# cboin1996/avddpg

Measured on AMD Instinct MI355X. Metric: env-steps/sec + DDPG updates/sec, 4096x5-vehicle platoons, higher is better.
Workload: dtype f32-class (fp16 hi+lo operand pairs on the 16-bit matrix cores, f32 accumulate)

## Files before the change

### avddpg_amd/_hip.py

```python
import ctypes as C
import os

_HERE = os.path.dirname(os.path.abspath(__file__))
LIB_PATH = os.path.join(_HERE, "lib", "libavddpg_hip.so")
if os.environ.get("AVDDPG_HIP_LIB"):
    LIB_PATH = os.path.abspath(os.environ["AVDDPG_HIP_LIB"])
HEADER_PATH = os.path.join(os.path.dirname(_HERE), "include", "avddpg_hip.h")
AVD_MAX_L = 16


class AvdError(RuntimeError):
    pass


class EnvConsts(C.Structure):
    _fields_ = [("L", C.c_int32), ("model_a", C.c_int32), ("can_terminate", C.c_int32), ("uniform_reset", C.c_int32),
                ("max_ep", C.c_float), ("max_ev", C.c_float), ("abs_action_high", C.c_float),
                ("two_max_a", C.c_float), ("T", C.c_float),
                ("ca", C.c_float), ("cb", C.c_float), ("cc", C.c_float), ("cd", C.c_float),
                ("re_scalar", C.c_float), ("terminal_reward", C.c_float),
                ("stand_still", C.c_float), ("timegap", C.c_float),
                ("reset_ep_max", C.c_float), ("reset_max_ev", C.c_float), ("reset_max_a", C.c_float),
                ("reset_ep_eval", C.c_float), ("reset_ev_eval", C.c_float), ("reset_a_eval", C.c_float),
                ("leader_reset_a", C.c_float),
                ("A", (C.c_float * 16) * AVD_MAX_L), ("B", (C.c_float * 4) * AVD_MAX_L),
                ("C", (C.c_float * 4) * AVD_MAX_L)]


_LAYOUT_FIELDS = ["S", "A", "H1", "H2", "Ha", "B",
                  "aW1", "ab1", "ag1", "abe1", "aW2", "ab2", "ag2", "abe2", "aW3", "ab3", "actor_size",
                  "cWs", "cbs", "cgs", "cbes", "cWa", "cba", "cga", "cbea", "cW2", "cb2", "cg3", "cbe3", "cW3", "cb3",
                  "theta_size",
                  "amm1", "amv1", "amm2", "amv2", "cmms", "cmvs", "cmma", "cmva", "cmm3", "cmv3", "stats_size"]


class MlpLayout(C.Structure):
    _fields_ = [(n, C.c_int32) for n in _LAYOUT_FIELDS]


_P = C.c_void_p
_i, _f, _d, _u64, _i64 = C.c_int, C.c_float, C.c_double, C.c_uint64, C.c_int64
_LP = C.POINTER(MlpLayout)

_PROTOS = {
    "avd_mlp_layout_init": [_LP, _i, _i, _i, _i, _i, _i],
    "avd_env_step_f32": [_P, _i, _i, _P, _P, _P, _P, _P, _P, _P, _P, _P, _P, _P, _P],
    "avd_env_reset_f32": [_P, _i, _i, _P, _P, _P, _P, _P, _i, _u64, _u64, _P, _P],
    "avd_episode_end_f32": [_P, _i, _i, _i, _P, _P, _P, _P, _P, _P, _i, _P, _P, _P, _P, _i, _u64, _u64, _P],
    "avd_ou_step_f32": [_i, _P, _P, _f, _f, _f, _f, _u64, _u64, _P],
    "avd_policy_f32": [_i, _P, _P, _f, _f, _P, _P],
    "avd_normal_f32": [_i, _P, _f, _u64, _u64, _P],
    "avd_uniform_f32": [_i, _P, _f, _u64, _u64, _P],
    "avd_step_fused_f32": [_P, _i, _i, _i, _P, _P, _P, _P, _P, _P, _P, _P, _P, _P, _P, _P, _P, _f, _f, _f, _f, _f, _f, _f, _i, _u64, _u64,
                           _u64, _P, _i, _i64, _P, _P],
    "avd_replay_sample_f32": [_i, _i, _i, _i, _i, _P, _i, _u64, _u64, _P, _P, _P, _P, _P, _P],
    "avd_actor_forward_set_f32": [_LP, _i, _i, _P, _P, _P, _i, _f, _P, _P, _P],
    "avd_replay_add_f32": [_i, _i, _i, _i, _P, _i64, _P, _P, _i, _P, _P, _P],
    "avd_replay_indices": [_i, _i, _i, _u64, _u64, _P, _P],
    "avd_replay_gather_f32": [_i, _i, _i, _i, _i, _P, _P, _P, _P, _P, _P, _P],
    "avd_actor_forward_f32": [_LP, _i, _i, _P, _P, _P, _i, _f, _P, _P],
    "avd_actor_forward_cond_f32": [_LP, _i, _i, _P, _P, _P, _i, _f, _P, _P, _P],
    "avd_critic_forward_f32": [_LP, _i, _i, _P, _P, _P, _i, _P, _P, _P],
    "avd_learn_f32": [_LP, _i, _i, _P, _P, _P, _P, _P, _P, _P, _P, _f, _f, _P, _P, _P],
    "avd_learn_update_f32": [_LP, _i, _P, _P, _P, _P, _P, _P, _P, _P, _P, _P, _P, _P, _f, _f, _f, _f, _d, _P, _P, _P],
    "avd_learn_update_act_f32": [_LP, _i, _P, _P, _P, _P, _P, _P, _P, _P, _P, _P, _P, _P, _f, _f, _f, _f, _d, _P, _P, _P, _i, _P, _P],
    "avd_learn_update_plan": [_LP, _i, C.POINTER(C.c_int), C.POINTER(C.c_int), C.POINTER(C.c_int)],
    "avd_adam_polyak_f32": [_LP, _i, _P, _P, _P, _P, _P, _P, _P, _P, _f, _f, _d, _P],
    "avd_adam_polyak_guarded_f32": [_LP, _i, _P, _P, _P, _P, _P, _P, _P, _P, _f, _f, _d, _P, _P],
    "avd_polyak_f32": [_i64, _P, _P, _d, _P],
    "avd_fed_sum_f32": [_i, _i, _i, _i, _i, _P, _P, _P, _P, _P],
    "avd_fed_finalize_f32": [_i, _i, _P, _f, _P, _P],
    "avd_fed_scatter_f32": [_i, _i, _i, _i, _i, _i, _P, _P, _P],
    "avd_adam_polyak_intra_f32": [_LP, _i, _i, _i, _P, _P, _P, _P, _P, _P, _P, _P, _P, _f, _f, _d, _P],
    "avd_fed_history_push_f32": [_i, _i, _i, _P, _P, _P, _i, _P, _i, _i, _P, _P, _P],
    "avd_fed_weights_f32": [_i, _i, _i, _P, _P, _i, _P, _P, _P, _P],
    "avd_learn_shared_workspace": [_LP, _i, _i, C.POINTER(C.c_size_t)],
    "avd_learn_shared_bf16": [_LP, _i, _i, _P, _P, _P, _P, _P, _P, _P, _P, _P, _f, _f, _P, _P, _P, C.c_size_t, _P],
    "avd_learn_set_fused_workspace": [_LP, _i, _i, C.POINTER(C.c_size_t)],
    "avd_learn_set_fused_bf16": [_LP, _i, _i, _P, _P, _P, _P, _P, _P, _P, _P, _P, _f, _f, _P, _P, _P, C.c_size_t, _P],
    "avd_learn_set_split_workspace": [_LP, _i, _i, C.POINTER(C.c_size_t)],
    "avd_learn_set_split_mfma_count": [_LP, _i, _i, C.POINTER(C.c_ulonglong)],
    "avd_learn_set_split_critic": [_LP, _i, _i, _P, _P, _P, _P, _P, _P, _P, _P, _P, _f, _f, _P, _P, _P, C.c_size_t, _P],
    "avd_learn_set_split_actor": [_LP, _i, _i, _P, _P, _P, _f, _P, _P, C.c_size_t, _P],
    "avd_learn_set_split_bf16x3": [_LP, _i, _i, _P, _P, _P, _P, _P, _P, _P, _P, _P, _f, _f, _P, _P, _P, C.c_size_t, _P],
    "avd_learn_set_split_f16x3": [_LP, _i, _i, _P, _P, _P, _P, _P, _P, _P, _P, _P, _f, _f, _P, _P, _P, C.c_size_t, _P],
    "avd_actor_forward_shared_workspace": [_LP, _i, _i, C.POINTER(C.c_size_t)],
    "avd_actor_forward_shared_bf16": [_LP, _i, _i, _P, _P, _P, _f, _P, _P, C.c_size_t, _P],
    "avd_gemm_bt_bf16": [_i, _i, _i, _P, C.c_long, _P, C.c_long, _P, C.c_long, _P],
}

_lib = None
DIAG_LIB_PATH = os.path.join(_HERE, "lib", "libavddpg_hip_diag.so")


def _load(path):
    if not os.path.exists(path):
        raise AvdError(f"{path} not found: build the HIP extension first (__graft_entry__.build()); "
                       "avddpg_amd has no CPU fallback")
    l = C.CDLL(path)
    missing = []
    for name, args in _PROTOS.items():
        fn = getattr(l, name, None)
        if fn is None:
            missing.append(name)
            continue
        fn.argtypes = args
        fn.restype = C.c_int
    if missing and not os.environ.get("AVDDPG_HIP_LIB"):
        raise AvdError(f"{path} does not export {', '.join(missing)}: rebuild it (make -C avddpg_amd/csrc)")
    l.avd_last_error.restype = C.c_char_p
    l.avd_last_error.argtypes = []
    l.avd_version.restype, l.avd_version.argtypes = C.c_int, []
    if getattr(l, "avd_diagnostics_enabled", None) is None:
        l.avd_diagnostics_enabled = lambda: 0
    else:
        l.avd_diagnostics_enabled.restype, l.avd_diagnostics_enabled.argtypes = C.c_int, []
    return l


def lib():
    global _lib
    if _lib is None:
        _lib = _load(LIB_PATH)
    return _lib


class diag_library:
    _cached = None
    _stack = []

    def __enter__(self):
        global _lib, LIB_PATH
        if diag_library._cached is None:
            diag_library._cached = _load(DIAG_LIB_PATH)
            if not diag_library._cached.avd_diagnostics_enabled():
                raise AvdError(f"{DIAG_LIB_PATH} is not a diagnostic build")
        diag_library._stack.append((lib(), LIB_PATH))
        _lib, LIB_PATH = diag_library._cached, DIAG_LIB_PATH
        return _lib

    def __exit__(self, *exc):
        global _lib, LIB_PATH
        _lib, LIB_PATH = diag_library._stack.pop()
        return False


def call(name, *args):
    fn = getattr(lib(), name, None)
    if fn is None:
        raise AvdError(f"{name} is not exported by the loaded library (an older build?)")
    rc = fn(*args)
    if rc != 0:
        raise AvdError(f"{name} failed ({rc}): {lib().avd_last_error().decode()}")


def ptr(t):
    if t is None:
        return None
    if not t.is_contiguous():
        raise AvdError("non-contiguous tensor passed to the C ABI")
    return C.c_void_p(t.data_ptr())


def stream_handle():
    import torch
    return C.c_void_p(torch.cuda.current_stream().cuda_stream)


def make_layout(S, A, H1, H2, Ha, B):
    lay = MlpLayout()
    call("avd_mlp_layout_init", C.byref(lay), S, A, H1, H2, Ha, B)
    return lay
```

### avddpg_amd/csrc/fset.hip

```cpp
#include "fset_common.h"

namespace avd {
namespace fset {

__device__ __forceinline__ bf16x8 make_xf(float x0, float x1, float x2, float x3, int h) {
    const bf16 a0 = (bf16)x0, a1 = (bf16)x1, a2 = (bf16)x2, a3 = (bf16)x3;
    const bf16 l0 = (bf16)(x0 - (float)a0), l1 = (bf16)(x1 - (float)a1), l2 = (bf16)(x2 - (float)a2), l3 = (bf16)(x3 - (float)a3);
    const bf16 one = (bf16)1.f, zero = (bf16)0.f;
    bf16x8 v;
    v[0] = a0, v[1] = a1, v[2] = a2, v[3] = a3;
    v[4] = h ? one : l0, v[5] = h ? one : l1, v[6] = h ? zero : l2, v[7] = h ? zero : l3;
    return v;
}
__device__ __forceinline__ bf16x8 make_wf(float w0, float w1, float w2, float w3, float b, int h) {
    const bf16 a0 = (bf16)w0, a1 = (bf16)w1, a2 = (bf16)w2, a3 = (bf16)w3, bh = (bf16)b;
    const bf16 l0 = (bf16)(w0 - (float)a0), l1 = (bf16)(w1 - (float)a1), l2 = (bf16)(w2 - (float)a2), l3 = (bf16)(w3 - (float)a3);
    const bf16 bl = (bf16)(b - (float)bh), zero = (bf16)0.f;
    bf16x8 v;
    v[0] = h ? l0 : a0, v[1] = h ? l1 : a1, v[2] = h ? l2 : a2, v[3] = h ? l3 : a3;
    v[4] = h ? bh : a0, v[5] = h ? bl : a1, v[6] = h ? zero : a2, v[7] = h ? zero : a3;
    return v;
}

struct NetP {
// ... 382 lines not shown
    NetP net;
    int n_agents, n_sets;
    const bf16* xf;
    const float* act;
    const bf16* dz;
    float* partG;
};
template <int S, class NET>
__global__ __launch_bounds__(NT) void dw_kernel(const DwArgs p) {
    constexpr int KG = NET::KG, NGT = NET::NGT, NFW = (NGT + 1) / 2, LDZ = 160;
    __shared__ __attribute__((aligned(16))) bf16 dzimg[2][TILE * LDZ];
    const int tid = threadIdx.x, w = tid >> 6, lane = tid & 63, r = lane & 31, h = lane >> 5, wn = w & 3, fg = w >> 2;
    const int set = blockIdx.x % p.n_sets, j0 = blockIdx.x / p.n_sets, J = gridDim.x / p.n_sets, P = p.n_agents / p.n_sets;
    const float* th = p.net.th + (long)set * p.net.th_stride;
    bf16x8 wf[NFW];
    f32x16 G[NFW];
    const f32x16 zero16 = {};
#pragma unroll
    for (int i = 0; i < NFW; ++i) wf[i] = layer1_wf<S, NET>(p.net, th, fg * NFW + i, r, h, true), G[i] = zero16;
    const bool act_tiles = NET::critic && fg == 1;

    const int srow = tid >> 3, sch = tid & 7;
    uint4 d0 = {}, d1 = {};
    auto fetch = [&](int agent) {
        const uint4* src = (const uint4*)(p.dz + ((long)agent * TILE + srow) * H2 + 16 * sch);
        d0 = src[0], d1 = src[1];
    };
    auto stage = [&](int buf) {
        uint4* dst = (uint4*)(dzimg[buf] + srow * LDZ + 16 * sch);
        dst[0] = d0, dst[1] = d1;
    };
    bf16x8 nx0 = {}, nx1 = {};
    float na0 = 0.f, na1 = 0.f;
    auto fetch_x = [&](int agent) {
        const bf16x8* xa = (const bf16x8*)p.xf + (long)agent * TILE * 2;
        nx0 = xa[2 * r + h], nx1 = xa[2 * (32 + r) + h];
        if (act_tiles) na0 = p.act[(long)agent * TILE + r], na1 = p.act[(long)agent * TILE + 32 + r];
    };
    if (j0 < P) fetch(j0 * p.n_sets + set), fetch_x(j0 * p.n_sets + set), stage(0);
    __syncthreads();
    const int g4 = lane >> 4, q = (lane & 15) >> 2, pp = lane & 3;
    int buf = 0;
    for (int pi = j0; pi < P; pi += J, buf ^= 1) {
        const bool more = pi + J < P;
        const bf16x8 xs0 = nx0, xs1 = nx1;
        const bf16x8 xa0 = make_xf(na0, 0.f, 0.f, 0.f, h), xa1 = make_xf(na1, 0.f, 0.f, 0.f, h);
        if (more) fetch((pi + J) * p.n_sets + set), fetch_x((pi + J) * p.n_sets + set);
        bf16x8 bfr[2][2];
#pragma unroll
        for (int rh = 0; rh < 2; ++rh)
#pragma unroll
            for (int s = 0; s < 2; ++s)
#pragma unroll
                for (int hf = 0; hf < 2; ++hf) {
                    const int R0 = 32 * rh + 16 * s + 8 * hf + 4 * (g4 >> 1);
                    const bf16x4 t = __builtin_amdgcn_ds_read_tr16_b64_v4bf16(
                        (__attribute__((address_space(3))) bf16x4*)(dzimg[buf] + (R0 + q) * LDZ + 32 * wn + 16 * (g4 & 1) + 4 * pp));
#pragma unroll
                    for (int j = 0; j < 4; ++j) bfr[rh][s][4 * hf + j] = t[j];
                }
#pragma unroll
        for (int i = 0; i < NFW; ++i) {
            if (fg * NFW + i >= NGT) continue;
            const bool at = act_tiles && i >= 3;
#pragma unroll
            for (int rh = 0; rh < 2; ++rh) {
                const bf16x8 xf = rh ? (at ? xa1 : xs1) : (at ? xa0 : xs0);
                const f32x16 p1 = mfma(xf, wf[i], zero16);
#pragma unroll
                for (int s = 0; s < 2; ++s) {
                    uint4 xu;
                    xu.x = relu_bf16x2(p1[8 * s], p1[8 * s + 1]), xu.y = relu_bf16x2(p1[8 * s + 2], p1[8 * s + 3]);
                    xu.z = relu_bf16x2(p1[8 * s + 4], p1[8 * s + 5]), xu.w = relu_bf16x2(p1[8 * s + 6], p1[8 * s + 7]);
                    G[i] = mfma(__builtin_bit_cast(bf16x8, xu), bfr[rh][s], G[i]);
                }
            }
        }
        if (more) stage(buf ^ 1);
        __syncthreads();
    }
#pragma unroll
    for (int i = 0; i < NFW; ++i) {
        if (fg * NFW + i >= NGT) continue;
        float* dst = p.partG + ((long)blockIdx.x * KG + 32 * (fg * NFW + i)) * H2 + 32 * wn + r;
#pragma unroll
        for (int k = 0; k < 16; ++k) dst[(long)acc_row(k, h) * H2] = G[i][k];
    }
}

struct DxArgs {
    NetP net;
    int n_agents, n_sets;
    const bf16* xf;
    const float* x;
    const bf16* dz;
    float* partU;
    float* partV;
};
template <int S, class NET>
__global__ __launch_bounds__(NT) void dx_kernel(const DxArgs p) {
    constexpr int KP = NET::KP, NF = 2, LDZ = 136;
    __shared__ __attribute__((aligned(16))) bf16 dzimg[2][TILE * LDZ];
    __shared__ __attribute__((aligned(16))) bf16 xt[8][2][32 * 32];
    const int tid = threadIdx.x, w = tid >> 6, lane = tid & 63, r = lane & 31, h = lane >> 5, rh = w & 1, fg = w >> 1;
    const int set = blockIdx.x % p.n_sets, j0 = blockIdx.x / p.n_sets, J = gridDim.x / p.n_sets, P = p.n_agents / p.n_sets;
    const float* th = p.net.th + (long)set * p.net.th_stride;
    const f32x16 zero16 = {};
    bf16x8 w2[NF][8], wf[NF];
    f32x16 V[NF];
    float U0[NF], U1[NF];
#pragma unroll
    for (int i = 0; i < NF; ++i) {
        const int ft = fg + 4 * i;
        const bf16* src = p.net.W2R + ((long)set * KP + 32 * ft + r) * H2 + 8 * h;
#pragma unroll
        for (int s = 0; s < 8; ++s) w2[i][s] = *(const bf16x8*)(src + 16 * s);
        wf[i] = layer1_wf<S, NET>(p.net, th, ft, r, h);
        V[i] = zero16, U0[i] = 0.f, U1[i] = 0.f;
    }
    for (int i = lane; i < 2 * 32 * 32; i += 64) {
        const int k = (i >> 5) & 31;
        xt[w][0][i] = (bf16)(k == 8 ? 1.f : 0.f);
    }
    const int srow = tid >> 3, sch = tid & 7;
    uint4 d0 = {}, d1 = {};
    auto fetch = [&](int agent) {
        const uint4* src = (const uint4*)(p.dz + ((long)agent * TILE + srow) * H2 + 16 * sch);
        d0 = src[0], d1 = src[1];
    };
    auto stage = [&](int buf) {
        uint4* dst = (uint4*)(dzimg[buf] + srow * LDZ + 16 * sch);
        dst[0] = d0, dst[1] = d1;
    };
    bf16x8 xfn = {};
    auto fetch_x = [&](int agent) { xfn = ((const bf16x8*)p.xf)[((long)agent * TILE + 32 * rh + r) * 2 + h]; };
    auto stage_x = [&](int buf) {
        if (h == 0) {
#pragma unroll
            for (int k = 0; k < 8; ++k) xt[w][buf][k * 32 + r] = xfn[k];
        }
    };
    __syncthreads();
    if (j0 < P) fetch(j0 * p.n_sets + set), fetch_x(j0 * p.n_sets + set), stage(0), stage_x(0);
    __syncthreads();
    int buf = 0;
    for (int pi = j0; pi < P; pi += J, buf ^= 1) {
        const bool more = pi + J < P;
        const bf16x8 xf = xfn;
        if (more) fetch((pi + J) * p.n_sets + set), fetch_x((pi + J) * p.n_sets + set);
        bf16x8 dzf[8];
        const bf16* arow = dzimg[buf] + (32 * rh + r) * LDZ + 8 * h;
#pragma unroll
        for (int s = 0; s < 8; ++s) dzf[s] = *(const bf16x8*)(arow + 16 * s);
        bf16x8 xb[2];
#pragma unroll
        for (int s = 0; s < 2; ++s) {
            const bf16x4 lo = *(const bf16x4*)(&xt[w][buf][r * 32 + 16 * s + 4 * h]);
            const bf16x4 hi = *(const bf16x4*)(&xt[w][buf][r * 32 + 16 * s + 8 + 4 * h]);
#pragma unroll
            for (int j = 0; j < 4; ++j) xb[s][j] = lo[j], xb[s][4 + j] = hi[j];
        }
#pragma unroll
        for (int i = 0; i < NF; ++i) {
            f32x16 dc = zero16;
#pragma unroll
            for (int s = 0; s < 8; ++s) dc = mfma(dzf[s], w2[i][s], dc);
            const f32x16 p1 = mfma(xf, wf[i], zero16);
            float u0 = 0.f, u1 = 0.f;
            bf16x8 va[2];
#pragma unroll
            for (int k = 0; k < 16; ++k) {
                const float pr = relu(p1[k]);
                u0 += dc[k];
                u1 = fmaf(dc[k], pr, u1);
                va[k >> 3][k & 7] = (bf16)(pr > 0.f ? dc[k] : 0.f);
            }
            U0[i] += u0, U1[i] += u1;
            V[i] = mfma(va[0], xb[0], V[i]);
            V[i] = mfma(va[1], xb[1], V[i]);
        }
        if (more) stage(buf ^ 1), stage_x(buf ^ 1);
        __syncthreads();
    }
#pragma unroll
    for (int i = 0; i < NF; ++i) {
        const int ft = fg + 4 * i;
        float* pu = p.partU + ((((long)blockIdx.x * 2 + rh) * 2 + h) * KP + 32 * ft + r) * 2;
        pu[0] = U0[i], pu[1] = U1[i];
        if (r < 16) {
            float* pv = p.partV + (((long)blockIdx.x * 2 + rh) * KP + 32 * ft) * 16 + r;
#pragma unroll
            for (int k = 0; k < 16; ++k) pv[(long)acc_row(k, h) * 16] = V[i][k];
        }
    }
}

template <int S>
__global__ __launch_bounds__(NT) void dxa_kernel(const DxArgs p) {
    typedef Critic NET;
    constexpr int KP = NET::KP;
    __shared__ __attribute__((aligned(16))) bf16 xt[8][2][32 * 32];
    __shared__ float comb[4][64][2 + 16];
    const int tid = threadIdx.x, w = tid >> 6, lane = tid & 63, r = lane & 31, h = lane >> 5, rh = w & 1, ftl = (w >> 1) & 1, par = w >> 2;
    const int set = blockIdx.x % p.n_sets, j0 = blockIdx.x / p.n_sets, J = gridDim.x / p.n_sets, P = p.n_agents / p.n_sets;
    const float* th = p.net.th + (long)set * p.net.th_stride;
    const f32x16 zero16 = {};
    const int ft = 8 + ftl;
    bf16x8 w2[8];
    {
        const bf16* src = p.net.W2R + ((long)set * KP + 32 * ft + r) * H2 + 8 * h;
#pragma unroll
        for (int s = 0; s < 8; ++s) w2[s] = *(const bf16x8*)(src + 16 * s);
    }
    const bf16x8 wf = layer1_wf<S, NET>(p.net, th, ft, r, h);
    f32x16 V = zero16;
    float U0 = 0.f, U1 = 0.f;
    for (int i = lane; i < 2 * 32 * 32; i += 64) {
        const int k = (i >> 5) & 31;
        xt[w][0][i] = (bf16)(k == 8 ? 1.f : 0.f);
    }
    __syncthreads();
    const int ntile = j0 < P ? (P - j0 + J - 1) / J : 0;
    bf16x8 dzn[8];
    float an = 0.f;
    auto fetch = [&](int k) {
        const long ri = (long)((j0 + k * J) * p.n_sets + set) * TILE + 32 * rh + r;
        const bf16* src = p.dz + ri * H2 + 8 * h;
#pragma unroll
        for (int s = 0; s < 8; ++s) dzn[s] = *(const bf16x8*)(src + 16 * s);
        an = p.x[ri];
    };
    if (par < ntile) fetch(par);
    int buf = 0;
    for (int k = par; k < ntile; k += 2, buf ^= 1) {
        bf16x8 dzf[8];
#pragma unroll
        for (int s = 0; s < 8; ++s) dzf[s] = dzn[s];
        const bf16x8 xf = make_xf(an, 0.f, 0.f, 0.f, h);
        if (k + 2 < ntile) fetch(k + 2);
        if (h == 0) {
            xt[w][buf][r] = xf[0];
            xt[w][buf][4 * 32 + r] = xf[4];
        }
        __builtin_amdgcn_fence(__ATOMIC_RELEASE, "wavefront");
        __builtin_amdgcn_wave_barrier();
        bf16x8 xb[2];
#pragma unroll
        for (int s = 0; s < 2; ++s) {
            const bf16x4 lo = *(const bf16x4*)(&xt[w][buf][r * 32 + 16 * s + 4 * h]);
            const bf16x4 hi = *(const bf16x4*)(&xt[w][buf][r * 32 + 16 * s + 8 + 4 * h]);
#pragma unroll
            for (int j = 0; j < 4; ++j) xb[s][j] = lo[j], xb[s][4 + j] = hi[j];
        }
        f32x16 dc = zero16;
#pragma unroll
        for (int s = 0; s < 8; ++s) dc = mfma(dzf[s], w2[s], dc);
        const f32x16 p1 = mfma(xf, wf, zero16);
        float u0 = 0.f, u1 = 0.f;
        bf16x8 va[2];
#pragma unroll
        for (int i = 0; i < 16; ++i) {
            const float pr = relu(p1[i]);
            u0 += dc[i];
            u1 = fmaf(dc[i], pr, u1);
            va[i >> 3][i & 7] = (bf16)(pr > 0.f ? dc[i] : 0.f);
        }
        U0 += u0, U1 += u1;
        V = mfma(va[0], xb[0], V);
        V = mfma(va[1], xb[1], V);
    }
    const int pw = w & 3;
    if (par == 1) {
        comb[pw][lane][0] = U0, comb[pw][lane][1] = U1;
#pragma unroll
        for (int i = 0; i < 16; ++i) comb[pw][lane][2 + i] = V[i];
    }
    __syncthreads();
    if (par == 0) {
        U0 += comb[pw][lane][0], U1 += comb[pw][lane][1];
        float* pu = p.partU + ((((long)blockIdx.x * 2 + rh) * 2 + h) * KP + 32 * ft + r) * 2;
        pu[0] = U0, pu[1] = U1;
        if (r < 16) {
            float* pv = p.partV + (((long)blockIdx.x * 2 + rh) * KP + 32 * ft) * 16 + r;
#pragma unroll
            for (int i = 0; i < 16; ++i) pv[(long)acc_row(i, h) * 16] = V[i] + comb[pw][lane][2 + i];
        }
    }
}

__global__ __launch_bounds__(512) void finalize_small_kernel(const FinArgs a) {
    const int set = blockIdx.x, net = a.net_lo + blockIdx.y, tid = threadIdx.x, jl = tid & 31;
    const int item = a.item_base + blockIdx.z * 16 + (tid >> 5);
    const bool critic = net;
    const avd_mlp_layout& L = a.L;
    const float* th = a.theta + (long)set * L.theta_size + (critic ? L.actor_size : 0);
    const float* st = a.stats + (long)set * L.stats_size;
    float* g = a.grads + (long)set * L.theta_size + (critic ? L.actor_size : 0);
    const int K = critic ? Critic::K : Actor::K, KP = critic ? Critic::KP : Actor::KP;
    auto allsum = [&](float v) {
#pragma unroll
        for (int o = 1; o < 32; o <<= 1) v += __shfl_xor(v, o);
        return v;
    };
    if (item < H2) {
        const int n = item;
        const int og2 = critic ? L.cg3 : L.ag2, obe2 = critic ? L.cbe3 : L.abe2, omm2 = critic ? L.cmm3 : L.amm2, omv2 = critic ? L.cmv3 : L.amv2;
        const int oW3 = critic ? L.cW3 : L.aW3, ob3 = critic ? L.cb3 : L.ab3, ob2 = critic ? L.cb2 : L.ab2;
        const int KG = critic ? Critic::KG : Actor::KG;
        float T1 = 0.f, S2 = 0.f, D = 0.f, Lc = 0.f, La = 0.f;
        const bool t1g = a.t1_from_g[net] != 0;
        for (int j = jl; j < a.J; j += 32) {
            const long wg = (long)j * a.n_sets + set;
            for (int w = 0; w < 8; ++w) {
                if (!t1g) T1 += a.partH[net][(wg * 8 + w) * H2 + n];
                D += a.partHs[net][(wg * 8 + w) * 2];
                if (critic && n == 0) Lc += a.partHs[1][(wg * 8 + w) * 2 + 1], La += a.partLa[(wg * 8 + w) * 2 + 1];
            }
            S2 += a.partG[net][(wg * KG + K) * H2 + n];
        }
        T1 = allsum(T1), S2 = allsum(S2), D = allsum(D);
        if (t1g && jl == 0) a.s2raw[((long)net * a.n_sets + set) * H2 + n] = S2;
        if (a.c3[net]) S2 *= a.c3[net][(long)set * VEC + H2 + n];
        if (critic && n == 0) Lc = allsum(Lc), La = allsum(La);
        if (a.bad && *a.bad) T1 = S2 = D = Lc = La = __uint_as_float(0x7fc00000u);
        if (jl == 0) {
            const float rs2 = 1.0f / sqrtf(st[omv2 + n] + BN_EPS), inv2 = rs2 * th[og2 + n], mm2 = st[omm2 + n];
            const float sh2 = th[obe2 + n] - mm2 * inv2, w3 = th[oW3 + n];
            if (!t1g) {
                g[oW3 + n] = inv2 * T1 + sh2 * D;
                g[og2 + n] = w3 * rs2 * (T1 - mm2 * D);
            }
            g[obe2 + n] = w3 * D;
            g[ob2 + n] = S2;
            if (n == 0) g[ob3] = D;
            if (critic && n == 0 && a.losses) a.losses[2 * set] = Lc * a.inv_n, a.losses[2 * set + 1] = -La * a.inv_n;
        }
        return;
    }
    const int f = item - H2;
    if (f >= K) return;
    float U0 = 0.f, U1 = 0.f, V[9];
#pragma unroll
    for (int k = 0; k < 9; ++k) V[k] = 0.f;
    const bool have_u = a.partU[net] != nullptr;
    for (int j = jl; j < a.J; j += 32) {
        const long wg = (long)j * a.n_sets + set;
        for (int rh = 0; rh < a.nrh; ++rh) {
            if (have_u)
                for (int h = 0; h < 2; ++h) {
                    const float* pu = a.partU[net] + ((((wg * a.nrh + rh) * 2 + h) * KP) + f) * 2;
                    U0 += pu[0], U1 += pu[1];
                }
            const float* pv = a.partV[net] + ((wg * a.nrh + rh) * KP + f) * 16;
#pragma unroll
            for (int k = 0; k < 9; ++k) V[k] += pv[k];
        }
    }
    U0 = allsum(U0), U1 = allsum(U1);
#pragma unroll
    for (int k = 0; k < 9; ++k) V[k] = allsum(V[k]);
    if (!have_u) {
        const int oW2 = critic ? L.cW2 : L.aW2, ob2 = critic ? L.cb2 : L.ab2;
        float u0 = 0.f;
        for (int n = jl; n < H2; n += 32) u0 = fmaf(th[oW2 + (long)f * H2 + n], g[ob2 + n], u0);
        U0 = allsum(u0);
        int oW, ob, ff = f, ld = H1, sin = a.S;
        if (!critic) oW = L.aW1, ob = L.ab1;
        else if (f < H1) oW = L.cWs, ob = L.cbs;
        else oW = L.cWa, ob = L.cba, ff = f - H1, ld = HA, sin = 1;
        U1 = th[ob + ff] * V[8];
        for (int k = 0; k < sin; ++k) U1 = fmaf(th[oW + k * ld + ff], V[k] + V[4 + k], U1);
    }
    if (a.bad && *a.bad) U0 = U1 = V[0] = V[4] = V[8] = __uint_as_float(0x7fc00000u);
    if (jl == 0) {
        int og, obe, omm, omv, oW, ob, ff = f, ld = H1, sin = a.S;
        if (!critic) og = L.ag1, obe = L.abe1, omm = L.amm1, omv = L.amv1, oW = L.aW1, ob = L.ab1;
        else if (f < H1) og = L.cgs, obe = L.cbes, omm = L.cmms, omv = L.cmvs, oW = L.cWs, ob = L.cbs;
        else og = L.cga, obe = L.cbea, omm = L.cmma, omv = L.cmva, oW = L.cWa, ob = L.cba, ff = f - H1, ld = HA, sin = 1;
        const float rs1 = 1.0f / sqrtf(st[omv + ff] + BN_EPS), inv1 = rs1 * th[og + ff], mm1 = st[omm + ff];
        g[obe + ff] = U0;
        g[og + ff] = rs1 * (U1 - mm1 * U0);
        g[ob + ff] = inv1 * V[8];
        for (int k = 0; k < sin; ++k) g[oW + k * ld + ff] = inv1 * (V[k] + V[4 + k]);
    }
}
__global__ __launch_bounds__(128) void finalize_w2_kernel(const FinArgs a) {
    const int f = blockIdx.x, set = blockIdx.y, net = a.net_lo + blockIdx.z, n = threadIdx.x;
    const bool critic = net;
    const int K = critic ? Critic::K : Actor::K, KG = critic ? Critic::KG : Actor::KG;
    if (f >= K) return;
    const avd_mlp_layout& L = a.L;
    const float* th = a.theta + (long)set * L.theta_size + (critic ? L.actor_size : 0);
    const float* st = a.stats + (long)set * L.stats_size;
    float* g = a.grads + (long)set * L.theta_size + (critic ? L.actor_size : 0);
    int og, obe, omm, omv, ff = f;
    if (!critic) og = L.ag1, obe = L.abe1, omm = L.amm1, omv = L.amv1;
    else if (f < H1) og = L.cgs, obe = L.cbes, omm = L.cmms, omv = L.cmvs;
    else og = L.cga, obe = L.cbea, omm = L.cmma, omv = L.cmva, ff = f - H1;
    const float inv1 = (1.0f / sqrtf(st[omv + ff] + BN_EPS)) * th[og + ff], sh1 = th[obe + ff] - st[omm + ff] * inv1;
    float G = 0.f;
    const float* pg = a.partG[net] + ((long)set * KG + f) * H2 + n;
    const long stride = (long)a.n_sets * KG * H2;
    int j = 0;
    for (; j + 8 <= a.J; j += 8) {
        float v[8];
#pragma unroll
        for (int u = 0; u < 8; ++u) v[u] = pg[(j + u) * stride];
#pragma unroll
        for (int u = 0; u < 8; ++u) G += v[u];
    }
    for (; j < a.J; ++j) G += pg[j * stride];
    const int oW2 = critic ? L.cW2 : L.aW2, ob2 = critic ? L.cb2 : L.ab2;
    if (a.t1_from_g[net]) a.t1p[(((long)net * a.n_sets + set) * Critic::K + f) * H2 + n] = inv1 * th[oW2 + (long)f * H2 + n] * G;
    if (a.c3[net]) G *= a.c3[net][(long)set * VEC + H2 + n];
    if (a.bad && *a.bad) G = __uint_as_float(0x7fc00000u);
    g[oW2 + (long)f * H2 + n] = inv1 * G + sh1 * g[ob2 + n];
}
__global__ __launch_bounds__(128) void finalize_t1_kernel(const FinArgs a) {
    const int set = blockIdx.x, net = a.net_lo + blockIdx.y, n = threadIdx.x;
    if (!a.t1_from_g[net]) return;
    const bool critic = net;
    const avd_mlp_layout& L = a.L;
    const float* th = a.theta + (long)set * L.theta_size + (critic ? L.actor_size : 0);
    const float* st = a.stats + (long)set * L.stats_size;
    float* g = a.grads + (long)set * L.theta_size + (critic ? L.actor_size : 0);
    const int K = critic ? Critic::K : Actor::K;
    const int og2 = critic ? L.cg3 : L.ag2, obe2 = critic ? L.cbe3 : L.abe2, omm2 = critic ? L.cmm3 : L.amm2, omv2 = critic ? L.cmv3 : L.amv2;
    const int oW3 = critic ? L.cW3 : L.aW3, ob3 = critic ? L.cb3 : L.ab3;
    const float* tp = a.t1p + ((long)net * a.n_sets + set) * Critic::K * H2 + n;
    float T1 = 0.f;
    int f = 0;
    for (; f + 8 <= K; f += 8) {
        float v[8];
#pragma unroll
        for (int u = 0; u < 8; ++u) v[u] = tp[(long)(f + u) * H2];
#pragma unroll
        for (int u = 0; u < 8; ++u) T1 += v[u];
    }
    for (; f < K; ++f) T1 += tp[(long)f * H2];
    T1 = fmaf(a.c3[net][(long)set * VEC + n], a.s2raw[((long)net * a.n_sets + set) * H2 + n], T1);
    const float D = g[ob3];
    if (a.bad && *a.bad) T1 = __uint_as_float(0x7fc00000u);
    const float rs2 = 1.0f / sqrtf(st[omv2 + n] + BN_EPS), inv2 = rs2 * th[og2 + n], mm2 = st[omm2 + n];
    const float sh2 = th[obe2 + n] - mm2 * inv2, w3 = th[oW3 + n];
    g[oW3 + n] = inv2 * T1 + sh2 * D;
    g[og2 + n] = w3 * rs2 * (T1 - mm2 * D);
}

void launch_finalize(const FinArgs& fa0, hipStream_t st, int net_lo, int n_nets) {
    FinArgs fa = fa0;
    fa.net_lo = net_lo, fa.item_base = 0;
    const int K = (net_lo + n_nets > 1) ? Critic::K : Actor::K;
    if (fa.partU[net_lo]) {
        hipLaunchKernelGGL(finalize_small_kernel, dim3(fa.n_sets, n_nets, (H2 + K + 15) / 16), dim3(512), 0, st, fa);
    } else {
        hipLaunchKernelGGL(finalize_small_kernel, dim3(fa.n_sets, n_nets, H2 / 16), dim3(512), 0, st, fa);
        fa.item_base = H2;
        hipLaunchKernelGGL(finalize_small_kernel, dim3(fa.n_sets, n_nets, (K + 15) / 16), dim3(512), 0, st, fa);
    }
    hipLaunchKernelGGL(finalize_w2_kernel, dim3(K, fa.n_sets, n_nets), dim3(H2), 0, st, fa);
    bool any = false;
    for (int net = net_lo; net < net_lo + n_nets; ++net) any = any || fa.t1_from_g[net];
    if (any) hipLaunchKernelGGL(finalize_t1_kernel, dim3(fa.n_sets, n_nets), dim3(H2), 0, st, fa);
}

struct Plan {
    int grid, J;
    size_t W2T[4], W2R[2], vec[4], a2, y, mu, dmu, dz, xfs, xfs2, partH[2], partHs[3], partU[2], partV[2], partG[2], bad, total;
};
int cu_count() {
    static int cache[64] = {0};
    int dev = 0;
    if (hipGetDevice(&dev) != hipSuccess || dev < 0) return 256;
    if (dev < 64 && cache[dev]) return cache[dev];
    hipDeviceProp_t prop;
    if (hipGetDeviceProperties(&prop, dev) != hipSuccess) return 256;
    const int n = prop.multiProcessorCount > 0 ? prop.multiProcessorCount : 256;
    if (dev < 64) cache[dev] = n;
    return n;
}
static Plan make_plan(int n_agents, int n_sets) {
    Plan pl;
    const int P = n_agents / n_sets;
    int J = cu_count() / n_sets;
    if (J < 1) J = 1;
    if (J > P) J = P;
    pl.J = J, pl.grid = J * n_sets;
    size_t o = 0;
    auto take = [&](size_t bytes) {
        const size_t at = o;
        o += (bytes + 255) / 256 * 256;
        return at;
    };
    for (int i = 0; i < 4; ++i) {
        const int KP = (i & 1) ? Critic::KP : Actor::KP, KW = (i & 1) ? Critic::KW : Actor::KW;
        pl.W2T[i] = take(sizeof(bf16) * (size_t)n_sets * H2 * KW);
        pl.vec[i] = take(sizeof(float) * (size_t)n_sets * VEC);
        if (i < 2) pl.W2R[i] = take(sizeof(bf16) * (size_t)n_sets * KP * H2);
    }
    const size_t rows = (size_t)n_agents * TILE;
    pl.a2 = take(4 * rows), pl.y = take(4 * rows), pl.mu = take(4 * rows), pl.dmu = take(4 * rows);
    pl.dz = take(sizeof(bf16) * rows * H2);
    pl.xfs = take(sizeof(bf16) * rows * 16), pl.xfs2 = take(sizeof(bf16) * rows * 16);
    for (int i = 0; i < 2; ++i) {
        const int KP = i ? Critic::KP : Actor::KP, KG = i ? Critic::KG : Actor::KG;
        pl.partH[i] = take(4 * (size_t)pl.grid * 8 * H2);
        pl.partU[i] = take(4 * (size_t)pl.grid * 2 * 2 * KP * 2);
        pl.partV[i] = take(4 * (size_t)pl.grid * 2 * KP * 16);
        pl.partG[i] = take(4 * (size_t)pl.grid * KG * H2);
    }
    for (int i = 0; i < 3; ++i) pl.partHs[i] = take(4 * (size_t)pl.grid * 8 * 2);
    pl.bad = take(sizeof(int));
    pl.total = o;
    return pl;
}
static int check_fset(const avd_mlp_layout* L, int n_agents, int n_sets, const char* who) {
    AVD_REQUIRE(L, "%s: null layout", who);
    if (L->H1 != H1 || L->H2 != H2 || L->Ha != HA || L->A != 1 || (L->S != 3 && L->S != 4) || L->B != TILE) {
        set_error("%s: serves the reference widths only (layer1 256, layer2 128, action layer 48, A = 1, S in {3, 4}, B = 64); "
                  "got H1=%d H2=%d Ha=%d A=%d S=%d B=%d (avd_learn_shared_bf16 takes other widths)",
                  who, L->H1, L->H2, L->Ha, L->A, L->S, L->B);
        return AVD_E_UNSUPPORTED;
    }
    AVD_REQUIRE(n_sets > 0 && n_sets <= 64 && n_agents > 0 && n_agents % n_sets == 0, "%s: n_agents=%d n_sets=%d", who, n_agents,
                n_sets);
    return AVD_OK;
}

template <int S>
static int run(const avd_mlp_layout& L, int n_agents, int n_sets, const float* theta, const float* stats, const float* theta_t,
               const float* stats_t, const float* s, const float* a, const float* r, const float* s2, const float* aw, float gamma,
               float high, float* grads, float* losses, unsigned char* ws, const Plan& pl, hipStream_t st) {
    PrepArgs pa;
    pa.L = L, pa.theta = theta, pa.stats = stats, pa.theta_t = theta_t, pa.stats_t = stats_t;
    NetP net[4];
    for (int i = 0; i < 4; ++i) {
        const bool critic = i & 1, target = i >= 2;
        pa.W2T[i] = (bf16*)(ws + pl.W2T[i]), pa.vec[i] = (float*)(ws + pl.vec[i]);
        pa.W2R[i] = i < 2 ? (bf16*)(ws + pl.W2R[i]) : nullptr;
        NetP& n = net[i];
        n.th = (target ? theta_t : theta) + (critic ? L.actor_size : 0), n.st = target ? stats_t : stats;
        n.th_stride = L.theta_size, n.st_stride = L.stats_size;
        n.oW1 = critic ? L.cWs : L.aW1, n.ob1 = critic ? L.cbs : L.ab1;
        n.oWa = critic ? L.cWa : 0, n.oba = critic ? L.cba : 0, n.oga = critic ? L.cga : 0, n.omva = critic ? L.cmva : 0;
        n.W2T = pa.W2T[i], n.W2R = pa.W2R[i], n.vec = pa.vec[i];
    }
    pa.bad = (int*)(ws + pl.bad);
    (void)hipMemsetAsync(ws + pl.bad, 0, sizeof(int), st);
    hipLaunchKernelGGL(prep_kernel, dim3(H2, 4, n_sets), dim3(320), 0, st, pa);
    const long nrows = (long)n_agents * TILE;
    bf16 *xfs = (bf16*)(ws + pl.xfs), *xfs2 = (bf16*)(ws + pl.xfs2);
    int* bad = (int*)(ws + pl.bad);
    hipLaunchKernelGGL(pack_x_kernel<S>, dim3((unsigned)((2 * nrows + 255) / 256)), dim3(256), 0, st, s, a, nrows, xfs, bad);
    hipLaunchKernelGGL(pack_x_kernel<S>, dim3((unsigned)((2 * nrows + 255) / 256)), dim3(256), 0, st, s2, r, nrows, xfs2, bad);
    const int P = n_agents / n_sets;
    const float inv_n = 1.0f / ((float)P * TILE);
    float *a2 = (float*)(ws + pl.a2), *y = (float*)(ws + pl.y), *mu = (float*)(ws + pl.mu), *dmu = (float*)(ws + pl.dmu);
    bf16* dz = (bf16*)(ws + pl.dz);
    auto F = [&](size_t off) { return (float*)(ws + off); };
    const dim3 grid(pl.grid), block(NT);
    HeadArgs h;
    h.n_agents = n_agents, h.n_sets = n_sets, h.gamma = gamma, h.high = high, h.inv_n = inv_n, h.aw = aw, h.dz = dz, h.dmu = dmu;
    auto head = [&](auto kern, int mode, int ni, const bf16* x, const float* act, const float* rr, const float* yin, float* out,
                    float* part, float* part_s) {
        h.net = net[ni], h.xf = x, h.act = act, h.r = rr, h.yin = yin, h.out = out, h.part = part, h.part_s = part_s;
        hipLaunchKernelGGL(kern, grid, dim3(64 * head_waves(mode)), 0, st, h);
    };
    DwArgs dw;
    dw.n_agents = n_agents, dw.n_sets = n_sets, dw.dz = dz;
    DxArgs dx;
    dx.n_agents = n_agents, dx.n_sets = n_sets, dx.dz = dz;
    head(head_kernel<S, Actor, OUT_TANH>, OUT_TANH, 2, xfs2, nullptr, nullptr, nullptr, a2, nullptr, nullptr);
    head(head_kernel<S, Critic, OUT_TD>, OUT_TD, 3, xfs2, a2, r, nullptr, y, nullptr, nullptr);
    head(head_kernel<S, Actor, OUT_TANH>, OUT_TANH, 0, xfs, nullptr, nullptr, nullptr, mu, nullptr, nullptr);
    head(head_kernel<S, Critic, HEAD_CRITIC>, HEAD_CRITIC, 1, xfs, a, nullptr, y, nullptr, F(pl.partH[1]), F(pl.partHs[1]));
    dw.net = net[1], dw.xf = xfs, dw.act = a, dw.partG = F(pl.partG[1]);
    hipLaunchKernelGGL((dw_kernel<S, Critic>), grid, block, 0, st, dw);
    dx.net = net[1], dx.partU = F(pl.partU[1]), dx.partV = F(pl.partV[1]);
    dx.xf = xfs, dx.x = nullptr;
    hipLaunchKernelGGL((dx_kernel<S, Critic>), grid, block, 0, st, dx);
    dx.x = a;
    hipLaunchKernelGGL((dxa_kernel<S>), grid, block, 0, st, dx);
    head(head_kernel<S, Critic, HEAD_CONST>, HEAD_CONST, 1, xfs, mu, nullptr, nullptr, nullptr, nullptr, F(pl.partHs[2]));
    head(head_kernel<S, Actor, HEAD_ACTOR>, HEAD_ACTOR, 0, xfs, nullptr, nullptr, dmu, nullptr, F(pl.partH[0]), F(pl.partHs[0]));
    dw.net = net[0], dw.xf = xfs, dw.act = nullptr, dw.partG = F(pl.partG[0]);
    hipLaunchKernelGGL((dw_kernel<S, Actor>), grid, block, 0, st, dw);
    dx.net = net[0], dx.partU = F(pl.partU[0]), dx.partV = F(pl.partV[0]), dx.x = nullptr;
    hipLaunchKernelGGL((dx_kernel<S, Actor>), grid, block, 0, st, dx);
    FinArgs fa;
    fa.L = L, fa.n_sets = n_sets, fa.J = pl.J, fa.S = S, fa.theta = theta, fa.stats = stats, fa.grads = grads, fa.losses = losses;
    fa.inv_n = inv_n, fa.partLa = F(pl.partHs[2]);
    for (int i = 0; i < 2; ++i)
        fa.partH[i] = F(pl.partH[i]), fa.partHs[i] = F(pl.partHs[i]), fa.partU[i] = F(pl.partU[i]), fa.partV[i] = F(pl.partV[i]),
        fa.partG[i] = F(pl.partG[i]);
    fa.nrh = 2, fa.c3[0] = fa.c3[1] = nullptr, fa.bad = (const int*)(ws + pl.bad);
    fa.t1_from_g[0] = fa.t1_from_g[1] = 0, fa.t1p = nullptr, fa.s2raw = nullptr;
    launch_finalize(fa, st);
    return check_launch("avd_learn_set_fused_bf16");
}

}
}

using namespace avd;

extern "C" int avd_learn_set_fused_workspace(const avd_mlp_layout* lay, int n_agents, int n_sets, size_t* bytes) {
    int rc = fset::check_fset(lay, n_agents, n_sets, "avd_learn_set_fused_workspace");
    if (rc) return rc;
    AVD_REQUIRE(bytes, "avd_learn_set_fused_workspace: null pointer");
    *bytes = fset::make_plan(n_agents, n_sets).total;
    return AVD_OK;
}

extern "C" int avd_learn_set_fused_bf16(const avd_mlp_layout* lay, int n_agents, int n_sets, const float* theta, const float* stats,
                                        const float* theta_t, const float* stats_t, const float* s, const float* a, const float* r,
                                        const float* s2, const float* agent_weight, float gamma, float high, float* grads,
                                        float* losses, void* workspace, size_t workspace_bytes, void* stream) {
    int rc = fset::check_fset(lay, n_agents, n_sets, "avd_learn_set_fused_bf16");
    if (rc) return rc;
    AVD_REQUIRE(theta && stats && theta_t && stats_t && s && a && r && s2 && grads && workspace,
                "avd_learn_set_fused_bf16: null pointer");
    const fset::Plan pl = fset::make_plan(n_agents, n_sets);
    AVD_REQUIRE(workspace_bytes >= pl.total, "avd_learn_set_fused_bf16: workspace %zu B < %zu B", workspace_bytes, pl.total);
    if (hipMemsetAsync(grads, 0, sizeof(float) * (size_t)n_sets * lay->theta_size, (hipStream_t)stream) != hipSuccess)
        return check_launch("avd_learn_set_fused_bf16: hipMemsetAsync(grads)");
    if (lay->S == 4)
        return fset::run<4>(*lay, n_agents, n_sets, theta, stats, theta_t, stats_t, s, a, r, s2, agent_weight, gamma, high, grads,
                            losses, (unsigned char*)workspace, pl, (hipStream_t)stream);
    return fset::run<3>(*lay, n_agents, n_sets, theta, stats, theta_t, stats_t, s, a, r, s2, agent_weight, gamma, high, grads, losses,
                        (unsigned char*)workspace, pl, (hipStream_t)stream);
}
```

### avddpg_amd/csrc/fsplit.hip

```cpp
#include <type_traits>

#include "fset_common.h"

namespace avd {
namespace fsplit {
using namespace fset;

struct ActorS {
    static constexpr int K = 256, KP = 256, NFT = 8, NKS = 16, LD = 264, NGT = 9, KG = 288;
    static constexpr bool critic = false;
};
struct CriticS {
    static constexpr int K = 304, KP = 320, NFT = 10, NKS = 19, LD = 312, NGT = 10, KG = 320;
    static constexpr bool critic = true;
};
constexpr int NGT_MAX = 10;

template <int I, int N, class F>
__device__ __forceinline__ void static_for(F&& f) {
    if constexpr (I < N) {
        f(std::integral_constant<int, I>{});
        static_for<I + 1, N>(f);
    }
}

typedef _Float16 f16;
typedef _Float16 f16x2 __attribute__((ext_vector_type(2)));
typedef _Float16 f16x8 __attribute__((ext_vector_type(8)));
constexpr float S1 = 64.f;
constexpr float F16_OVERFLOW = 65520.f;
#if defined(FSPLIT_ABL_CONST)
#define FSPLIT_ABL(x) FSPLIT_ABL_CONST
#elif defined(AVD_DIAG)
#define FSPLIT_ABL(x) (x)
#else
#define FSPLIT_ABL(x) 0
#endif
__device__ __forceinline__ void split2h(float a, float b, unsigned& hi, unsigned& lo) {
    const f32x2 f = {a, b};
    const f16x2 h = __builtin_convertvector(f, f16x2);
    hi = __builtin_bit_cast(unsigned, h);
    f32x2 l;
#ifdef __HIP_DEVICE_COMPILE__
    asm("v_fma_mix_f32 %0, -%1, 1.0, %2 op_sel:[0,0,0] op_sel_hi:[1,0,0]" : "=v"(l[0]) : "v"(hi), "v"(a));
    asm("v_fma_mix_f32 %0, -%1, 1.0, %2 op_sel:[1,0,0] op_sel_hi:[1,0,0]" : "=v"(l[1]) : "v"(hi), "v"(b));
#else
    l[0] = a - (float)h[0], l[1] = b - (float)h[1];
#endif
    lo = __builtin_bit_cast(unsigned, __builtin_convertvector(l, f16x2));
}
__device__ __forceinline__ void split1h(float x, f16& hi, f16& lo) {
    hi = (f16)x;
    lo = (f16)(x - (float)hi);
}
template <class V>
__device__ __forceinline__ void pin16(V& x) {
#pragma unroll
    for (int q = 0; q < 2; ++q) {
        float a = x[8 * q], b = x[8 * q + 1], c = x[8 * q + 2], d = x[8 * q + 3], e = x[8 * q + 4], f = x[8 * q + 5], g = x[8 * q + 6], h = x[8 * q + 7];
        asm volatile("" : "+v"(a), "+v"(b), "+v"(c), "+v"(d), "+v"(e), "+v"(f), "+v"(g), "+v"(h));
        x[8 * q] = a, x[8 * q + 1] = b, x[8 * q + 2] = c, x[8 * q + 3] = d, x[8 * q + 4] = e, x[8 * q + 5] = f, x[8 * q + 6] = g, x[8 * q + 7] = h;
    }
}
__device__ __forceinline__ f16x8 fragh(unsigned a, unsigned b, unsigned c, unsigned d) {
    uint4 o;
    o.x = a, o.y = b, o.z = c, o.w = d;
    return __builtin_bit_cast(f16x8, o);
}
__device__ __forceinline__ f32x16 mfmah(f16x8 a, f16x8 b, f32x16 c) {
    return __builtin_amdgcn_mfma_f32_32x32x16_f16(a, b, c, 0, 0, 0);
}
__device__ __forceinline__ f16x8 make_xh(float x0, float x1, float x2, float x3, int h) {
    f16 a0, a1, a2, a3, l0, l1, l2, l3;
    split1h(x0, a0, l0), split1h(x1, a1, l1), split1h(x2, a2, l2), split1h(x3, a3, l3);
    const f16 one = (f16)1.f, zero = (f16)0.f;
    f16x8 v;
    v[0] = a0, v[1] = a1, v[2] = a2, v[3] = a3;
    v[4] = h ? one : l0, v[5] = h ? one : l1, v[6] = h ? zero : l2, v[7] = h ? zero : l3;
    return v;
}
__device__ __forceinline__ f16x8 make_wh(float w0, float w1, float w2, float w3, float b, float sc, int h) {
    f16 a0, a1, a2, a3, l0, l1, l2, l3, bh, bl;
    split1h(sc * w0, a0, l0), split1h(sc * w1, a1, l1), split1h(sc * w2, a2, l2), split1h(sc * w3, a3, l3), split1h(sc * b, bh, bl);
    const f16 zero = (f16)0.f;
    f16x8 v;
    v[0] = h ? l0 : a0, v[1] = h ? l1 : a1, v[2] = h ? l2 : a2, v[3] = h ? l3 : a3;
    v[4] = h ? bh : a0, v[5] = h ? bl : a1, v[6] = h ? bh : a2, v[7] = h ? zero : a3;
    return v;
}
__device__ __forceinline__ f16x8 make_xg(float x0, float x1, float x2, float x3, float g, int h) {
    f16 a0, a1, a2, a3, l0, l1, l2, l3, gh, gl;
    split1h(x0, a0, l0), split1h(x1, a1, l1), split1h(x2, a2, l2), split1h(x3, a3, l3), split1h(g, gh, gl);
    const f16 zero = (f16)0.f;
    f16x8 v;
    v[0] = a0, v[1] = a1, v[2] = a2, v[3] = a3;
    v[4] = h ? gh : l0, v[5] = h ? gh : l1, v[6] = h ? gl : l2, v[7] = h ? zero : l3;
    return v;
}

template <int S>
__device__ __forceinline__ void load_x(const float* xa, long row, float (&x)[4]) {
    if (S == 4) {
        const float4 v = *(const float4*)(xa + 4 * row);
        x[0] = v.x, x[1] = v.y, x[2] = v.z, x[3] = v.w;
    } else {
#pragma unroll
        for (int k = 0; k < 4; ++k) x[k] = k < S ? xa[S * row + k] : 0.f;
    }
}

__host__ __device__ constexpr int wpos(int f) { return (f & ~12) | ((f & 4) << 1) | ((f & 8) >> 1); }

struct NetP {
    const float* th;
    long th_stride;
    const f16* Whi;
    const f16* Wlo;
    const f16* Wchi;
    const f16* Wclo;
    const f16x8* wf1h;
    const float* vec;
    const unsigned* wap;
};

struct PackArgs {
    const float* x[2];
    const float* extra[2];
    f16x8* outh[2];
    long rows;
    int* bad;
};
template <int S>
__global__ __launch_bounds__(256) void pack_x_kernel(const PackArgs a) {
    const int which = blockIdx.y;
    const float* x = a.x[which];
    const float* extra = a.extra[which];
    const bool extra_is_action = which == 0;
    const long i = (long)blockIdx.x * 256 + threadIdx.x;
    if (i >= 2 * a.rows) return;
    float v[4];
    load_x<S>(x, i >> 1, v);
    bool nf = not_finite(v[0]) || not_finite(v[1]) || not_finite(v[2]) || not_finite(v[3]);
    nf = nf || fmaxf(fmaxf(fabsf(v[0]), fabsf(v[1])), fmaxf(fabsf(v[2]), fabsf(v[3]))) >= F16_OVERFLOW;
    if (!(i & 1)) {
        const float e = extra[i >> 1];
        nf = nf || not_finite(e) || (extra_is_action && fabsf(e) >= F16_OVERFLOW);
    }
    if (nf) atomicOr(a.bad, 1);
    a.outh[which][i] = make_xh(v[0], v[1], v[2], v[3], (int)(i & 1));
}

struct PrepArgs {
    avd_mlp_layout L;
    int S;
    const float *theta, *stats, *theta_t, *stats_t;
    f16 *Whi[4], *Wlo[4];
    f16 *Wchi[4], *Wclo[4];
    f16x8* wf1h[4];
    float* vec[4];
    unsigned* wap;
    unsigned* smax;
    int* bad;
};
constexpr int SCALE_SLICES = 16;
__device__ __forceinline__ float pow2_for(float mx) {
    int e = 0;
    if (mx > 0.f && !not_finite(mx)) (void)frexpf(mx, &e);
    int k = 13 - e;
    k = k < -14 ? -14 : (k > 30 ? 30 : k);
    return ldexpf(1.f, k);
}
__global__ __launch_bounds__(256) void scale_kernel(const PrepArgs a) {
    __shared__ float red[256], red2[256], c3a[H2], inva[CriticS::K];
    const int net = blockIdx.x, set = blockIdx.y, slice = blockIdx.z, tid = threadIdx.x;
    const bool critic = net & 1, target = net >= 2;
    const avd_mlp_layout& L = a.L;
    const float* th = (target ? a.theta_t : a.theta) + (long)set * L.theta_size + (critic ? L.actor_size : 0);
    const float* st = (target ? a.stats_t : a.stats) + (long)set * L.stats_size;
    const int K = critic ? CriticS::K : ActorS::K, oW2 = critic ? L.cW2 : L.aW2;
    const int og2 = critic ? L.cg3 : L.ag2, omv2 = critic ? L.cmv3 : L.amv2, oW3 = critic ? L.cW3 : L.aW3;
    if (tid < H2) c3a[tid] = fabsf((1.0f / sqrtf(st[omv2 + tid] + BN_EPS)) * th[og2 + tid] * th[oW3 + tid]);
    for (int f = tid; f < K; f += 256) {
        int og, omv, ff = f;
        if (!critic) og = L.ag1, omv = L.amv1;
        else if (f < H1) og = L.cgs, omv = L.cmvs;
        else og = L.cga, omv = L.cmva, ff = f - H1;
        inva[f] = fabsf((1.0f / sqrtf(st[omv + ff] + BN_EPS)) * th[og + ff]);
    }
    __syncthreads();
    const int total = K * H2, per = (total + SCALE_SLICES - 1) / SCALE_SLICES, lo = slice * per, hi = min(total, lo + per);
    float m = 0.f, m2 = 0.f;
    for (int i = lo + tid; i < hi; i += 256) {
        const float w = fabsf(th[oW2 + i]);
        m = fmaxf(m, inva[i / H2] * w);
        m2 = fmaxf(m2, c3a[i % H2] * w);
    }
    red[tid] = m, red2[tid] = m2;
    __syncthreads();
    for (int o = 128; o > 0; o >>= 1) {
        if (tid < o) red[tid] = fmaxf(red[tid], red[tid + o]), red2[tid] = fmaxf(red2[tid], red2[tid + o]);
        __syncthreads();
    }
    if (tid == 0) {
        unsigned* dst = a.smax + ((long)net * gridDim.y + set) * 2;
        atomicMax(dst, __float_as_uint(red[0]));
        atomicMax(dst + 1, __float_as_uint(red2[0]));
    }
}
__global__ __launch_bounds__(320) void prep_kernel(const PrepArgs a) {
    __shared__ float red[320];
    const int n = blockIdx.x, net = blockIdx.y, set = blockIdx.z, f = threadIdx.x;
    const bool critic = net & 1, target = net >= 2;
    const avd_mlp_layout& L = a.L;
    const float* th = (target ? a.theta_t : a.theta) + (long)set * L.theta_size + (critic ? L.actor_size : 0);
    const float* st = (target ? a.stats_t : a.stats) + (long)set * L.stats_size;
    const int K = critic ? CriticS::K : ActorS::K, KP = critic ? CriticS::KP : ActorS::KP;
    const int oW2 = critic ? L.cW2 : L.aW2, ob2 = critic ? L.cb2 : L.ab2, oW3 = critic ? L.cW3 : L.aW3, ob3 = critic ? L.cb3 : L.ab3;
    const int og2 = critic ? L.cg3 : L.ag2, obe2 = critic ? L.cbe3 : L.abe2, omm2 = critic ? L.cmm3 : L.amm2, omv2 = critic ? L.cmv3 : L.amv2;
    const float inv2n = (1.0f / sqrtf(st[omv2 + n] + BN_EPS)) * th[og2 + n], c3n = inv2n * th[oW3 + n];
    const unsigned* smax = a.smax + ((long)net * gridDim.z + set) * 2;
    const float SW = pow2_for(__uint_as_float(smax[0])), SWC = pow2_for(__uint_as_float(smax[1]));
    float shw = 0.f;
    if (f < KP) {
        float w = 0.f, inv = 0.f;
        if (f < K) {
            int og, obe, omm, omv, ff = f;
            if (!critic) og = L.ag1, obe = L.abe1, omm = L.amm1, omv = L.amv1;
            else if (f < H1) og = L.cgs, obe = L.cbes, omm = L.cmms, omv = L.cmvs;
            else og = L.cga, obe = L.cbea, omm = L.cmma, omv = L.cmva, ff = f - H1;
            inv = (1.0f / sqrtf(st[omv + ff] + BN_EPS)) * th[og + ff];
            const float sh = th[obe + ff] - st[omm + ff] * inv;
            w = th[oW2 + (long)f * H2 + n];
            shw = sh * w;
            if (not_finite(w) || not_finite(inv) || not_finite(sh)) atomicOr(a.bad, 1);
            f16 hi, lo;
            const float ws = SW * (inv * w);
            if (fabsf(ws) >= F16_OVERFLOW) atomicOr(a.bad, 1);
            split1h(ws, hi, lo);
            const long at = ((long)set * H2 + n) * K + wpos(f);
            a.Whi[net][at] = hi, a.Wlo[net][at] = lo;
        }
        if (!target) {
            f16 hi, lo;
            const float wc = SWC * (c3n * w);
            if (fabsf(wc) >= F16_OVERFLOW) atomicOr(a.bad, 1);
            split1h(wc, hi, lo);
            const long at = ((long)set * KP + f) * H2 + n;
            a.Wchi[net][at] = hi, a.Wclo[net][at] = lo;
        }
    }
    red[f] = shw;
    __syncthreads();
    if (f < 64) red[f] += red[f + 256];
    __syncthreads();
    for (int o = 128; o > 0; o >>= 1) {
        if (f < o) red[f] += red[f + o];
        __syncthreads();
    }
    float* vec = a.vec[net] + (long)set * VEC;
    if (f == 0) {
        if (n == 0) vec[2 * H2 + 1] = SW, vec[2 * H2 + 2] = SWC;
        vec[n] = th[ob2 + n] + red[0];
        vec[H2 + n] = c3n;
        if (not_finite(vec[n]) || not_finite(c3n) || not_finite(th[ob3])) atomicOr(a.bad, 1);
    }
    if (n == 0) {
        __syncthreads();
        float v = 0.f;
        if (f < H2) {
            const float inv2 = (1.0f / sqrtf(st[omv2 + f] + BN_EPS)) * th[og2 + f];
            v = (th[obe2 + f] - st[omm2 + f] * inv2) * th[oW3 + f];
        }
        red[f] = v;
        __syncthreads();
        for (int o = 64; o > 0; o >>= 1) {
            if (f < o) red[f] += red[f + o];
            __syncthreads();
        }
        if (f == 0) vec[2 * H2] = th[ob3] + red[0];
    }
}
__global__ __launch_bounds__(64) void prep1_kernel(const PrepArgs a) {
    const int ft = blockIdx.x, net = blockIdx.y, set = blockIdx.z, lane = threadIdx.x, r = lane & 31, h = lane >> 5;
    const bool critic = net & 1, target = net >= 2;
    const avd_mlp_layout& L = a.L;
    const float* th = (target ? a.theta_t : a.theta) + (long)set * L.theta_size + (critic ? L.actor_size : 0);
    const int K = critic ? CriticS::K : ActorS::K;
    const int f = 32 * ft + r;
    float w[4] = {0.f, 0.f, 0.f, 0.f}, b = 0.f;
    if (f == K) {
        b = 1.f;
    } else if (f < K) {
        if (critic && ft >= 8) {
            w[0] = th[L.cWa + (f - H1)], b = th[L.cba + (f - H1)];
        } else {
            const float* W = th + (critic ? L.cWs : L.aW1);
#pragma unroll
            for (int k = 0; k < 4; ++k) w[k] = k < a.S ? W[k * H1 + f] : 0.f;
            b = th[(critic ? L.cbs : L.ab1) + f];
        }
        if (not_finite(w[0]) || not_finite(w[1]) || not_finite(w[2]) || not_finite(w[3]) || not_finite(b)) atomicOr(a.bad, 1);
        if (S1 * fmaxf(fmaxf(fabsf(w[0]), fabsf(w[1])), fmaxf(fmaxf(fabsf(w[2]), fabsf(w[3])), fabsf(b))) >= F16_OVERFLOW) atomicOr(a.bad, 1);
    }
    a.wf1h[net][((long)set * NGT_MAX + ft) * 64 + lane] = make_wh(w[0], w[1], w[2], w[3], b, S1, h);
    if (net == 1 && ft == 0 && lane < 48) {
        const int hl = lane / 24, hh = (lane / 12) & 1, ks = (lane / 4) % 3, m = lane & 3;
        unsigned v = 0;
#pragma unroll
        for (int e = 0; e < 2; ++e) {
            const int jj = 2 * m + e, fa = 16 * ks + 8 * (jj >> 2) + 4 * hh + (jj & 3);
            f16 hi, lo;
            split1h(S1 * th[L.cWa + fa], hi, lo);
            v |= (unsigned)__builtin_bit_cast(unsigned short, hl ? lo : hi) << (16 * e);
        }
        a.wap[(long)set * 48 + lane] = v;
    }
}

enum HeadMode { OUT_TANH = 0, OUT_TD = 1, HEAD_BOTH = 5, OUT_TANH_SAVE = 6 };
struct HeadArgs {
    unsigned long long* stamp;
    NetP net;
    int n_agents, n_sets;
    const f16x8* xf;
    const float* act;
    const float* act2;
    const float* r;
    const float* yin;
    const float* aw;
    float* out;
    f16* sm;
    float* g3;
    float* dmu;
    float* part_s;
    float* part_s2;
    float* part_m;
    float* tz;
    float gamma, high, inv_n;
    int* bad;
    int abl;
};
#ifndef HEAD_FAST
#define HEAD_FAST 5
#define HEAD_SLOW 3
#endif

template <int S, class NET, int MODE>
__global__ __launch_bounds__(NT) void head_kernel(const HeadArgs p) {
    constexpr int K = NET::K, NKS = NET::NKS, NFT = NET::NFT, LD = NET::LD;
    constexpr int NTH = NT;
    constexpr bool BOTH = (MODE == HEAD_BOTH);
    static_assert(!BOTH || NET::critic, "HEAD_BOTH is a critic mode");
    __shared__ __attribute__((aligned(16))) f16 wimg[2][H2 * LD];
    __shared__ __attribute__((aligned(16))) float b2s[H2];
    __shared__ __attribute__((aligned(16))) float c3s[H2];
    __shared__ __attribute__((aligned(16))) unsigned waps[BOTH ? 48 : 4];
    const int tid = threadIdx.x, w = tid >> 6, lane = tid & 63, r = lane & 31, h = lane >> 5, q = w >> 1, rh = w & 1;
    const int set = blockIdx.x % p.n_sets, j0 = blockIdx.x / p.n_sets, J = gridDim.x / p.n_sets, P = p.n_agents / p.n_sets;
    for (int i = tid; i < 2 * H2 * (K / 8); i += NTH) {
        const int hl = i / (H2 * (K / 8)), rem = i - hl * (H2 * (K / 8)), n = rem / (K / 8), c = rem - n * (K / 8);
        const f16* src = (hl ? p.net.Wlo : p.net.Whi) + ((long)set * H2 + n) * K + 8 * c;
        *(uint4*)(&wimg[hl][n * LD + 8 * c]) = *(const uint4*)src;
    }
    const float* vec = p.net.vec + (long)set * VEC;
    const float SW = vec[2 * H2 + 1], sc = SW * S1, isc = 1.f / sc;
    if (tid < H2) b2s[tid] = vec[tid] * sc, c3s[tid] = vec[H2 + tid] * isc;
    if (BOTH && tid < 48) waps[tid] = p.net.wap[(long)set * 48 + tid];
    const float d3 = vec[2 * H2];
    const f16x8* wf1 = p.net.wf1h + (long)set * NGT_MAX * 64 + lane;
    const f32x16 zero16 = {};
#ifdef AVD_STAMP
    unsigned long long hacc[4] = {0, 0, 0, 0}, hlast = __builtin_amdgcn_s_memtime();
    const unsigned long long hstart = hlast;
#define HSTAMP(i) { const unsigned long long t_ = __builtin_amdgcn_s_memtime(); hacc[i] += t_ - hlast; hlast = t_; }
#else
#define HSTAMP(i)
#endif
    float Dacc = 0.f, Lacc = 0.f, Dacc2 = 0.f, Lacc2 = 0.f, gmax = 0.f;
    unsigned watch = 0;
    auto look = [&](float x) {
        unsigned u = __float_as_uint(x);
        asm volatile("" : "+v"(u));
        u &= 0x7fffffffu;
        watch = watch > u ? watch : u;
    };
    __syncthreads();

    const int ntile = j0 < P ? (P - j0 + J - 1) / J : 0;
    const int row = 32 * rh + r;
    f16x8 nx = {};
    float na = 0.f, nb = 0.f, ny = 0.f, nw = 1.f;
    auto fetch_in = [&](int k) {
        const int agent = (j0 + k * J) * p.n_sets + set;
        const long ri = (long)agent * TILE + row;
        nx = p.xf[2 * ri + h];
        if (NET::critic) na = p.act[ri];
        if (BOTH) nb = p.act2[ri];
        if (MODE == OUT_TD) ny = p.r[ri];
        if (BOTH) ny = p.yin[ri];
        if (BOTH && p.aw) nw = p.aw[agent];
    };
    const f16* whi0 = &wimg[0][r * LD + 8 * h];
    const f16* wlo0 = &wimg[1][r * LD + 8 * h];
    constexpr int NSEQ = BOTH ? 8 : NFT;
    HSTAMP(3);
    constexpr int FAST = HEAD_FAST, SLOW = HEAD_SLOW, PERIOD = 2 * (FAST + SLOW);
    const int qs = __builtin_amdgcn_readfirstlane(q);
    const int cnt = qs < 2 ? FAST : SLOW, start = qs < 2 ? qs * FAST : 2 * FAST + (qs - 2) * SLOW;
    int k = start, pos = 0;
    auto next_tile = [&](int kk, int pp) { return pp + 1 == cnt ? kk + PERIOD - cnt + 1 : kk + 1; };
    if (k < ntile) fetch_in(k);
    for (int ui = 0; k < ntile; ++ui, k = next_tile(k, pos), pos = pos + 1 == cnt ? 0 : pos + 1) {
        const int agent = (j0 + k * J) * p.n_sets + set;
        const long ri = (long)agent * TILE + row;
        const f16x8 xs = nx, xa = make_xh(na, 0.f, 0.f, 0.f, h), xb = BOTH ? make_xh(nb, 0.f, 0.f, 0.f, h) : xa;
        const float ty = ny, tw = nw;
        if (next_tile(k, pos) < ntile) fetch_in(next_tile(k, pos));
        f32x16 acc[4];
#pragma unroll
        for (int t = 0; t < 4; ++t)
#pragma unroll
            for (int g = 0; g < 4; ++g) {
                const float4 b = *(const float4*)(b2s + 32 * t + 8 * g + 4 * h);
                acc[t][4 * g] = b.x, acc[t][4 * g + 1] = b.y, acc[t][4 * g + 2] = b.z, acc[t][4 * g + 3] = b.w;
            }
        unsigned ph[8], pl[8];
        auto split16 = [&](const f32x16& p1) {
            if (FSPLIT_ABL(p.abl) & 4) {
#pragma unroll
                for (int m = 0; m < 8; ++m) ph[m] = __float_as_uint(p1[2 * m]), pl[m] = __float_as_uint(p1[2 * m + 1]);
                return;
            }
#pragma unroll
            for (int m = 0; m < 8; ++m) split2h(relu(p1[2 * m]), relu(p1[2 * m + 1]), ph[m], pl[m]);
        };
        auto zdot_t = [&](f32x16& a, int t) {
            float zp = 0.f;
#pragma unroll
            for (int g = 0; g < 4; ++g) {
                const float4 c = *(const float4*)(c3s + 32 * t + 8 * g + 4 * h);
                const float cc[4] = {c.x, c.y, c.z, c.w};
#pragma unroll
                for (int j = 0; j < 4; ++j) {
                    a[4 * g + j] = relu(a[4 * g + j]);
                    zp = fmaf(a[4 * g + j], cc[j], zp);
                }
            }
            return zp;
        };
        auto zdot_nd = [&](const f32x16& a, int t) {
            float zp = 0.f;
#pragma unroll
            for (int g = 0; g < 4; ++g) {
                const float4 c = *(const float4*)(c3s + 32 * t + 8 * g + 4 * h);
                const float cc[4] = {c.x, c.y, c.z, c.w};
#pragma unroll
                for (int j = 0; j < 4; ++j) zp = fmaf(relu(a[4 * g + j]), cc[j], zp);
            }
            return zp;
        };
        auto mask_t = [&](const f32x16& a, int t, unsigned s16, f16* dst) {
            unsigned pk[4][2];
#pragma unroll
            for (int g = 0; g < 4; ++g)
#pragma unroll
                for (int e = 0; e < 2; ++e) {
                    const int i = 4 * g + 2 * e;
                    pk[g][e] = (a[i] > 0.f ? s16 : 0u) | (a[i + 1] > 0.f ? s16 << 16 : 0u);
                }
#pragma unroll
            for (int gg = 0; gg < 2; ++gg) {
                const auto s0 = __builtin_amdgcn_permlane32_swap(pk[2 * gg][0], pk[2 * gg + 1][0], false, false);
                const auto s1 = __builtin_amdgcn_permlane32_swap(pk[2 * gg][1], pk[2 * gg + 1][1], false, false);
                uint4 o;
                o.x = s0[0], o.y = s1[0], o.z = s0[1], o.w = s1[1];
                *(uint4*)(dst + 32 * t + 16 * gg) = o;
            }
        };
        auto out_z = [&](f32x16 (&ac)[4]) {
            float zp = 0.f;
#pragma unroll
            for (int t = 0; t < 4; ++t) zp += zdot_t(ac[t], t);
            zp += __shfl_xor(zp, 32);
            return d3 + zp;
        };
        split16(mfmah(wf1[0], xs, zero16));
        f16x8 wfn = wf1[64];
        f16x8 wg[2][2][2];
        auto read_group = [&](int g, f16x8 (&dst)[2][2]) {
            const int ks = g >> 1, th = g & 1;
#pragma unroll
            for (int tt = 0; tt < 2; ++tt) {
                dst[tt][0] = *(const f16x8*)(whi0 + 32 * (2 * th + tt) * LD + 16 * ks);
                dst[tt][1] = *(const f16x8*)(wlo0 + 32 * (2 * th + tt) * LD + 16 * ks);
            }
        };
        read_group(0, wg[0]);
        auto tile = [&](auto si_c, f32x16 (&ac)[4]) {
            constexpr int si = decltype(si_c)::value;
            constexpr int ft = si;
            f32x16 p1n = zero16;
            if constexpr (si + 1 < NSEQ) {
                p1n = mfmah(wfn, (NET::critic && si + 1 >= 8) ? xa : xs, zero16);
                if constexpr (si + 2 < NSEQ) wfn = wf1[64 * (si + 2)];
            }
#pragma unroll
            for (int s = 0; s < 2; ++s) {
                const int ks = 2 * ft + s;
                if (ks >= NKS) continue;
                const f16x8 bhi = fragh(ph[4 * s], ph[4 * s + 1], ph[4 * s + 2], ph[4 * s + 3]);
                const f16x8 blo = fragh(pl[4 * s], pl[4 * s + 1], pl[4 * s + 2], pl[4 * s + 3]);
#pragma unroll
                for (int th = 0; th < 2; ++th) {
                    const int g = 2 * ks + th;
                    if (g + 1 < 2 * (BOTH ? 16 : NKS)) read_group(g + 1, wg[(g + 1) & 1]);
#pragma unroll
                    for (int tt = 0; tt < 2; ++tt) {
                        const int t = 2 * th + tt;
                        const f16x8 whi = wg[g & 1][tt][0], wlo = wg[g & 1][tt][1];
                        ac[t] = mfmah(whi, bhi, ac[t]);
                        ac[t] = mfmah(wlo, bhi, ac[t]);
                        ac[t] = mfmah(whi, blo, ac[t]);
                    }
                }
            }
            if constexpr (si + 1 < NSEQ) split16(p1n);
            __builtin_amdgcn_sched_group_barrier(0x008, 1, 0);
#pragma unroll
            for (int gi = 0; gi < 4; ++gi) {
                __builtin_amdgcn_sched_group_barrier(0x100, 4, 0);
#pragma unroll
                for (int i = 0; i < 6; ++i) {
                    __builtin_amdgcn_sched_group_barrier(0x008, 1, 0);
                    __builtin_amdgcn_sched_group_barrier(0x002, 3, 0);
                }
            }
            __builtin_amdgcn_sched_barrier(0);
        };
        HSTAMP(0);
        static_for<0, NSEQ>([&](auto si_c) { tile(si_c, acc); });
        HSTAMP(1);
        if constexpr (BOTH) {
            f16x8 fh[3], fl[3];
            auto act_sweep = [&](f32x16 (&c)[4]) {
                f16x8 wq[2][2][2];
                read_group(2 * 16, wq[0]);
#pragma unroll
                for (int g = 0; g < 6; ++g) {
                    if (g + 1 < 6) read_group(2 * 16 + g + 1, wq[(g + 1) & 1]);
#pragma unroll
                    for (int tt = 0; tt < 2; ++tt) {
                        const int t = 2 * (g & 1) + tt;
                        const f16x8 whi = wq[g & 1][tt][0], wlo = wq[g & 1][tt][1];
                        c[t] = mfmah(whi, fh[g >> 1], c[t]);
                        c[t] = mfmah(wlo, fh[g >> 1], c[t]);
                        c[t] = mfmah(whi, fl[g >> 1], c[t]);
                    }
                }
            };
#pragma unroll
            for (int tl = 0; tl < 2; ++tl) {
                const f32x16 p1 = mfmah(wf1[64 * (8 + tl)], xa, zero16);
                split16(p1);
#pragma unroll
                for (int ss = 0; ss < 2 - tl; ++ss) {
                    fh[2 * tl + ss] = fragh(ph[4 * ss], ph[4 * ss + 1], ph[4 * ss + 2], ph[4 * ss + 3]);
                    fl[2 * tl + ss] = fragh(pl[4 * ss], pl[4 * ss + 1], pl[4 * ss + 2], pl[4 * ss + 3]);
                }
            }
            act_sweep(acc);
            look(acc[0][0]);
            {
                float zp = 0.f;
#pragma unroll
                for (int t = 0; t < 4; ++t) zp += zdot_nd(acc[t], t);
                zp += __shfl_xor(zp, 32);
                const float diff = d3 + zp - ty, g3a = 2.f * diff * p.inv_n * tw;
                if (h == 0) p.g3[ri] = g3a, Dacc += g3a, Lacc += diff * diff;
                gmax = fmaxf(gmax, fabsf(g3a));
#pragma unroll
                for (int t = 0; t < 4; ++t) {
                    mask_t(acc[t], t, g3a < 0.f ? 0xbc00u : 0x3c00u, p.sm + ri * H2 + 8 * h);
                }
            }
            __builtin_amdgcn_sched_barrier(0);
            f16x8 mh[3], ml[3];
#pragma unroll
            for (int tl = 0; tl < 2; ++tl) {
                const f32x16 pa = mfmah(wf1[64 * (8 + tl)], xa, zero16), pm = mfmah(wf1[64 * (8 + tl)], xb, zero16);
                unsigned dh[8], dl[8], mk[8];
#pragma unroll
                for (int m = 0; m < 4 * (2 - tl); ++m) {
                    split2h(relu(pm[2 * m]) - relu(pa[2 * m]), relu(pm[2 * m + 1]) - relu(pa[2 * m + 1]), dh[m], dl[m]);
                    mk[m] = (pm[2 * m] > 0.f ? 0xffffu : 0u) | (pm[2 * m + 1] > 0.f ? 0xffff0000u : 0u);
                }
#pragma unroll
                for (int ss = 0; ss < 2 - tl; ++ss) {
                    const int kk = 2 * tl + ss;
                    fh[kk] = fragh(dh[4 * ss], dh[4 * ss + 1], dh[4 * ss + 2], dh[4 * ss + 3]);
                    fl[kk] = fragh(dl[4 * ss], dl[4 * ss + 1], dl[4 * ss + 2], dl[4 * ss + 3]);
                    const uint4 ch = *(const uint4*)(waps + (0 * 2 + h) * 12 + 4 * kk), cl = *(const uint4*)(waps + (1 * 2 + h) * 12 + 4 * kk);
                    mh[kk] = fragh(ch.x & mk[4 * ss], ch.y & mk[4 * ss + 1], ch.z & mk[4 * ss + 2], ch.w & mk[4 * ss + 3]);
                    ml[kk] = fragh(cl.x & mk[4 * ss], cl.y & mk[4 * ss + 1], cl.z & mk[4 * ss + 2], cl.w & mk[4 * ss + 3]);
                }
            }
            act_sweep(acc);
            look(acc[0][0]);
            float zq = 0.f;
            unsigned pos[2] = {0u, 0u};
#pragma unroll
            for (int t = 0; t < 4; ++t) {
                zq += zdot_nd(acc[t], t);
#pragma unroll
                for (int i = 0; i < 16; ++i) pos[t >> 1] |= acc[t][i] > 0.f ? 1u << (16 * (t & 1) + i) : 0u;
            }
            zq += __shfl_xor(zq, 32);
            asm volatile("" : "+v"(pos[0]), "+v"(pos[1]));
#pragma unroll
            for (int kk = 0; kk < 3; ++kk) fh[kk] = mh[kk], fl[kk] = ml[kk];
#pragma unroll
            for (int t = 0; t < 4; ++t) acc[t] = zero16;
// ... 292 lines not shown
    if (p.stamp && blockIdx.x == 16 && lane == 0)
        for (int i = 0; i < 4; ++i) p.stamp[w * 8 + i] = tacc[i];
#endif
    const float dsc = 1.f / (gsc * S1);
    float* comb = (float*)&smimg[0][0];
    const int cidx = NET::critic ? 2 * (w >> 2) + (w & 1) : (w & 3);
    if (xrh == 1) {
#pragma unroll
        for (int c = 0; c < XC; ++c)
#pragma unroll
            for (int k = 0; k < 16; ++k) comb[((cidx * XC + c) * 16 + k) * 64 + lane] = G1[c][k];
    }
    __syncthreads();
#pragma unroll
    for (int c = 0; c < 4; ++c) {
        float* dst = p.partG + ((long)blockIdx.x * KG + 32 * w) * H2 + 32 * c + r;
#pragma unroll
        for (int k = 0; k < 16; ++k) dst[(long)acc_row(k, h) * H2] = G0[c][k] * dsc;
    }
    if (xrh == 0) {
#pragma unroll
        for (int c = 0; c < XC; ++c) {
            float* dst = p.partG + ((long)blockIdx.x * KG + 32 * xt) * H2 + 32 * (xc0 + c) + r;
#pragma unroll
            for (int k = 0; k < 16; ++k) dst[(long)acc_row(k, h) * H2] = (G1[c][k] + comb[((cidx * XC + c) * 16 + k) * 64 + lane]) * dsc;
        }
    }
}

struct DxArgs {
    NetP net;
    int n_agents, n_sets;
    const f16x8* xfh;
    const float* act;
    int L_cWa, L_cba;
    const float* g3;
    const float* part_m;
    const f16* sm;
    int unsigned_mask;
    float* partV;
    int abl;
    unsigned long long* stamp;
};
template <int S, class NET>
__global__ __launch_bounds__(NT) void dx_kernel(const DxArgs p) {
    constexpr int KP = NET::KP, LDZ = 136;
    constexpr float VSH = 1.f / 32.f;
    __shared__ __attribute__((aligned(16))) f16 smimg[2][TILE * LDZ];
    __shared__ __attribute__((aligned(16))) f16 xt[2][2][32 * 32];
    __shared__ __attribute__((aligned(16))) float g3s[2][TILE];
    __shared__ float gred[8];
    const int tid = threadIdx.x, w = __builtin_amdgcn_readfirstlane(tid >> 6), lane = tid & 63, r = lane & 31, h = lane >> 5, ft = w;
    const int set = blockIdx.x % p.n_sets, j0 = blockIdx.x / p.n_sets, J = gridDim.x / p.n_sets, P = p.n_agents / p.n_sets;
    const f32x16 zero16 = {};
    const float gsc = set_gscale(p.part_m, set, p.n_sets, J, gred);
    f16x8 wch[8], wcl[8];
    {
        const long at = ((long)set * KP + 32 * ft + r) * H2 + 8 * h;
#pragma unroll
        for (int s = 0; s < 8; ++s) wch[s] = *(const f16x8*)(p.net.Wchi + at + 16 * s), wcl[s] = *(const f16x8*)(p.net.Wclo + at + 16 * s);
    }
    const float swc = __uint_as_float(__builtin_amdgcn_readfirstlane(__float_as_uint(p.net.vec[(long)set * VEC + 2 * H2 + 2])));
    const float gv = gsc * VSH, vs = gsc * swc * VSH;
    const f16x8 wf = p.net.wf1h[((long)set * NGT_MAX + ft) * 64 + lane];
    f32x16 V = zero16;
    for (int i = tid; i < 2 * 2 * 32 * 32; i += NT) {
        const int k = (i >> 5) & 31;
        (&xt[0][0][0])[i] = (f16)(k == 8 ? 1.f : 0.f);
    }
    const int srow = tid >> 3, sch = tid & 7;
    uint4 d0 = {}, d1 = {};
    float gn = 0.f;
    auto fetch = [&](int agent) {
        if (FSPLIT_ABL(p.abl) & 1) agent = j0 * p.n_sets + set;
        const uint4* src = (const uint4*)(p.sm + ((long)agent * TILE + srow) * H2 + 16 * sch);
        d0 = src[0], d1 = src[1];
        if (tid < TILE) gn = p.g3[(long)agent * TILE + tid];
    };
    auto stage = [&](int buf) {
        uint4* dst = (uint4*)(smimg[buf] + srow * LDZ + 16 * sch);
        dst[0] = d0, dst[1] = d1;
        if (tid < TILE) g3s[buf][tid] = (p.unsigned_mask ? gn : fabsf(gn)) * gv;
    };
    f16x8 xfn0 = {}, xfn1 = {};
    auto fetch_x = [&](int agent) {
        xfn0 = p.xfh[((long)agent * TILE + r) * 2 + h];
        xfn1 = p.xfh[((long)agent * TILE + 32 + r) * 2 + h];
    };
    auto stage_x = [&](int buf) {
        if (w < 2 && h == 0) {
            f16x8 src = xfn0;
            if (w == 1) src = xfn1;
            asm volatile("" : "+v"(src));
#pragma unroll
            for (int k = 0; k < 8; ++k) xt[buf][w][k * 32 + r] = src[k];
        }
    };
    __syncthreads();
    if (j0 < P) fetch(j0 * p.n_sets + set), fetch_x(j0 * p.n_sets + set), stage(0), stage_x(0);
    __syncthreads();
#ifdef AVD_STAMP
    unsigned long long dacc[4] = {0, 0, 0, 0}, dlast = __builtin_amdgcn_s_memtime();
#define DXSTAMP(i) { const unsigned long long t_ = __builtin_amdgcn_s_memtime(); dacc[i] += t_ - dlast; dlast = t_; }
#else
#define DXSTAMP(i)
#endif
    int buf = 0;
    for (int pi = j0; pi < P; pi += J, buf ^= 1) {
        const bool more = pi + J < P;
        const f16x8 xf[2] = {xfn0, xfn1};
        if (more) fetch((pi + J) * p.n_sets + set), fetch_x((pi + J) * p.n_sets + set);
        DXSTAMP(0);
        auto read_a = [&](int e, f16x8 (&smf)[8]) {
            const f16* arow = smimg[buf] + (32 * e + r) * LDZ + 8 * h;
#pragma unroll
            for (int s = 0; s < 8; ++s) smf[s] = *(const f16x8*)(arow + 16 * s);
        };
        typedef _Float16 f16x4 __attribute__((ext_vector_type(4)));
        auto read_img = [&](const f16* img, f16x8 (&xb)[2]) {
#pragma unroll
            for (int s = 0; s < 2; ++s) {
                const f16x4 lo = *(const f16x4*)(img + r * 32 + 16 * s + 4 * h);
                const f16x4 hi = *(const f16x4*)(img + r * 32 + 16 * s + 8 + 4 * h);
#pragma unroll
                for (int j = 0; j < 4; ++j) xb[s][j] = lo[j], xb[s][4 + j] = hi[j];
            }
        };
        auto backward = [&](int e, const f32x16& dc, const f32x16& p1, unsigned (&vh)[8], unsigned (&vl)[8]) {
            if (FSPLIT_ABL(p.abl) & 4) {
#pragma unroll
                for (int m = 0; m < 8; ++m) vh[m] = __float_as_uint(dc[2 * m]) ^ __float_as_uint(p1[2 * m]), vl[m] = __float_as_uint(dc[2 * m + 1]);
                return;
            }
#pragma unroll
            for (int g = 0; g < 4; ++g) {
                const float4 gq = *(const float4*)(&g3s[buf][32 * e + 8 * g + 4 * h]);
                const float gg[4] = {gq.x, gq.y, gq.z, gq.w};
                float dm[4];
#pragma unroll
                for (int j = 0; j < 4; ++j) {
                    const int k = 4 * g + j;
                    dm[j] = p1[k] > 0.f ? dc[k] * gg[j] : 0.f;
                }
                split2h(dm[0], dm[1], vh[2 * g], vl[2 * g]);
                split2h(dm[2], dm[3], vh[2 * g + 1], vl[2 * g + 1]);
            }
        };
        f16x8 smf[8], xb0[2], xb1[2];
        unsigned vh0[8], vl0[8], vh1[8], vl1[8];
        read_a(0, smf);
        f32x16 dc0 = zero16;
#pragma unroll
        for (int s = 0; s < 8; ++s) dc0 = mfmah(smf[s], wch[s], dc0), dc0 = mfmah(smf[s], wcl[s], dc0);
        const f32x16 p10 = mfmah(xf[0], wf, zero16);
        __builtin_amdgcn_sched_barrier(0);
        read_a(1, smf);
        read_img(xt[buf][0], xb0);
        f32x16 dc1 = zero16;
#pragma unroll
        for (int s = 0; s < 8; ++s) dc1 = mfmah(smf[s], wch[s], dc1), dc1 = mfmah(smf[s], wcl[s], dc1);
        const f32x16 p11 = mfmah(xf[1], wf, zero16);
        backward(0, dc0, p10, vh0, vl0);
        __builtin_amdgcn_sched_group_barrier(0x100, 12, 0);
#pragma unroll
        for (int i = 0; i < 17; ++i) {
            __builtin_amdgcn_sched_group_barrier(0x008, 1, 0);
            __builtin_amdgcn_sched_group_barrier(0x002, 5, 0);
            __builtin_amdgcn_sched_group_barrier(0x100, 1, 0);
        }
        __builtin_amdgcn_sched_barrier(0);
        read_img(xt[buf][1], xb1);
#pragma unroll
        for (int s = 0; s < 2; ++s) {
            V = mfmah(fragh(vh0[4 * s], vh0[4 * s + 1], vh0[4 * s + 2], vh0[4 * s + 3]), xb0[s], V);
            V = mfmah(fragh(vl0[4 * s], vl0[4 * s + 1], vl0[4 * s + 2], vl0[4 * s + 3]), xb0[s], V);
        }
        backward(1, dc1, p11, vh1, vl1);
#pragma unroll
        for (int s = 0; s < 2; ++s) {
            V = mfmah(fragh(vh1[4 * s], vh1[4 * s + 1], vh1[4 * s + 2], vh1[4 * s + 3]), xb1[s], V);
            V = mfmah(fragh(vl1[4 * s], vl1[4 * s + 1], vl1[4 * s + 2], vl1[4 * s + 3]), xb1[s], V);
        }
        DXSTAMP(1);
        if (more) stage(buf ^ 1), stage_x(buf ^ 1);
        DXSTAMP(2);
        if (!(FSPLIT_ABL(p.abl) & 2)) __syncthreads();
        DXSTAMP(3);
    }
#ifdef AVD_STAMP
    if (p.stamp && blockIdx.x == 16 && lane == 0)
        for (int i = 0; i < 4; ++i) p.stamp[w * 8 + i] = dacc[i];
#endif
    const float ivs = 1.f / vs;
    if (r < 16) {
        float* pv = p.partV + ((long)blockIdx.x * KP + 32 * ft) * 16 + r;
#pragma unroll
        for (int k = 0; k < 16; ++k) pv[(long)acc_row(k, h) * 16] = V[k] * ivs;
    }
}

template <int S>
__global__ __launch_bounds__(NT) void dxa_kernel(const DxArgs p) {
    typedef CriticS NET;
    constexpr int KP = NET::KP;
    constexpr float VSH = 1.f / 32.f;
    constexpr int LDZ = 136;
    __shared__ __attribute__((aligned(16))) f16 simg[8][32 * LDZ];
    __shared__ __attribute__((aligned(16))) float ga[8][2][2][32];
    __shared__ float comb[8][64][2];
    __shared__ float gred[8];
    const int tid = threadIdx.x, w = __builtin_amdgcn_readfirstlane(tid >> 6), lane = tid & 63, r = lane & 31, h = lane >> 5;
    const int rh = w & 1, ftl = (w >> 1) & 1, par = w >> 2;
    const int set = blockIdx.x % p.n_sets, j0 = blockIdx.x / p.n_sets, J = gridDim.x / p.n_sets, P = p.n_agents / p.n_sets;
    const f32x16 zero16 = {};
    const int ft = 8 + ftl, f = 32 * ftl + r;
    const float gsc = set_gscale(p.part_m, set, p.n_sets, J, gred);
    f16x8 wch[8], wcl[8];
    {
        const long at = ((long)set * KP + 32 * ft + r) * H2 + 8 * h;
#pragma unroll
        for (int s = 0; s < 8; ++s) wch[s] = *(const f16x8*)(p.net.Wchi + at + 16 * s), wcl[s] = *(const f16x8*)(p.net.Wclo + at + 16 * s);
    }
    const float swc = __uint_as_float(__builtin_amdgcn_readfirstlane(__float_as_uint(p.net.vec[(long)set * VEC + 2 * H2 + 2])));
    const float gv = gsc * VSH, vs = gsc * swc * VSH;
    const float* th = p.net.th + (long)set * p.net.th_stride;
    const float wa = f < HA ? th[p.L_cWa + f] : 0.f, ba = f < HA ? th[p.L_cba + f] : 0.f;
    float Sa = 0.f, Sb = 0.f;
    const int ntile = j0 < P ? (P - j0 + J - 1) / J : 0;
    uint4 A0 = {}, A1 = {}, A2 = {}, A3 = {}, A4 = {}, A5 = {}, A6 = {}, A7 = {}, B0 = {}, B1 = {}, B2 = {}, B3 = {}, B4 = {}, B5 = {}, B6 = {}, B7 = {};
    float gA = 0.f, aA = 0.f, gB = 0.f, aB = 0.f;
#define DXA_FETCH(k_, X, g_, a_)                                                                                    \
    {                                                                                                               \
        const long r0_ = (long)((j0 + (k_) * J) * p.n_sets + set) * TILE + 32 * rh;                                 \
        const uint4* src_ = (const uint4*)(p.sm + r0_ * H2) + lane;  \
        X##0 = src_[0], X##1 = src_[64], X##2 = src_[128], X##3 = src_[192], X##4 = src_[256], X##5 = src_[320], X##6 = src_[384], X##7 = src_[448]; \
        g_ = p.g3[r0_ + r], a_ = p.act[r0_ + r];                                                                    \
    }
#define DXA_PUT(buf_, X, g_, a_)                                                                                    \
    {                                                                                                               \
        if (h == 0) ga[w][buf_][0][r] = fabsf(g_) * gv, ga[w][buf_][1][r] = a_;                                     \
        f16* dst_ = simg[w] + (lane >> 4) * LDZ + 8 * (lane & 15);                                                   \
        *(uint4*)(dst_) = X##0, *(uint4*)(dst_ + 4 * LDZ) = X##1, *(uint4*)(dst_ + 8 * LDZ) = X##2, *(uint4*)(dst_ + 12 * LDZ) = X##3; \
        *(uint4*)(dst_ + 16 * LDZ) = X##4, *(uint4*)(dst_ + 20 * LDZ) = X##5, *(uint4*)(dst_ + 24 * LDZ) = X##6, *(uint4*)(dst_ + 28 * LDZ) = X##7; \
        __builtin_amdgcn_fence(__ATOMIC_RELEASE, "wavefront");                                                      \
        __builtin_amdgcn_wave_barrier();                                                                            \
    }
    auto unit = [&](int buf) {
        f32x16 dc = zero16;
        const f16* arow = simg[w] + r * LDZ + 8 * h;
#pragma unroll
        for (int s = 0; s < 8; ++s) {
            const f16x8 af = *(const f16x8*)(arow + 16 * s);
            dc = mfmah(af, wch[s], dc), dc = mfmah(af, wcl[s], dc);
        }
        float sa = 0.f, sb = 0.f;
#pragma unroll
        for (int q = 0; q < 4; ++q) {
            const float4 gq = *(const float4*)(&ga[w][buf][0][8 * q + 4 * h]), aq = *(const float4*)(&ga[w][buf][1][8 * q + 4 * h]);
            const float gg[4] = {gq.x, gq.y, gq.z, gq.w}, av[4] = {aq.x, aq.y, aq.z, aq.w};
#pragma unroll
            for (int j = 0; j < 4; ++j) {
                const float m = fmaf(av[j], wa, ba) > 0.f ? dc[4 * q + j] * gg[j] : 0.f;
                sa = fmaf(m, av[j], sa);
                sb += m;
            }
        }
        Sa += sa, Sb += sb;
        __builtin_amdgcn_fence(__ATOMIC_ACQ_REL, "wavefront");
        __builtin_amdgcn_wave_barrier();
    };
    if (par < ntile) DXA_FETCH(par, A, gA, aA);
    if (par + 2 < ntile) DXA_FETCH(par + 2, B, gB, aB);
    for (int k = par; k < ntile; k += 4) {
        DXA_PUT(0, A, gA, aA);
        if (k + 4 < ntile) DXA_FETCH(k + 4, A, gA, aA);
        unit(0);
        if (k + 2 < ntile) {
            DXA_PUT(1, B, gB, aB);
            if (k + 6 < ntile) DXA_FETCH(k + 6, B, gB, aB);
            unit(1);
        }
    }
#undef DXA_FETCH
#undef DXA_PUT
    comb[w][lane][0] = Sa, comb[w][lane][1] = Sb;
    __syncthreads();
    if (rh == 0 && par == 0 && h == 0) {
        const int ws[4] = {w, w + 1, w + 4, w + 5};
        float t[2] = {0.f, 0.f};
#pragma unroll
        for (int i = 0; i < 4; ++i)
#pragma unroll
            for (int c = 0; c < 2; ++c) t[c] += comb[ws[i]][r][c] + comb[ws[i]][32 + r][c];
        const float ivs = 1.f / vs;
        float* pv = p.partV + ((long)blockIdx.x * KP + 32 * ft + r) * 16;
#pragma unroll
        for (int c = 0; c < 9; ++c) pv[c] = c == 0 ? t[0] * ivs : (c == 8 ? t[1] * ivs : 0.f);
    }
}

struct Plan {
    int grid, J;
    size_t Whi[4], Wlo[4], Wchi[2], Wclo[2], wf1h[4], vec[4], wap, a2, y, mu, dmu, g3, sm, sma, tz, t1p, s2raw, xfs, xfs2, partHs[3], partM[2],
        partV[2], partG[2], bad, total;
};
static Plan make_plan(int n_agents, int n_sets) {
    Plan pl;
    const int P = n_agents / n_sets;
    int J = cu_count() / n_sets;
    if (const char* e = AVD_DIAG_ENV("FSPLIT_J")) J = atoi(e);
    if (J < 1) J = 1;
    if (J > P) J = P;
    pl.J = J, pl.grid = J * n_sets;
    size_t o = 0;
    auto take = [&](size_t bytes) {
        const size_t at = o;
        o += (bytes + 255) / 256 * 256;
        return at;
    };
    for (int i = 0; i < 4; ++i) {
        const int K = (i & 1) ? CriticS::K : ActorS::K, KP = (i & 1) ? CriticS::KP : ActorS::KP;
        pl.Whi[i] = take(sizeof(f16) * (size_t)n_sets * H2 * K), pl.Wlo[i] = take(sizeof(f16) * (size_t)n_sets * H2 * K);
        pl.vec[i] = take(sizeof(float) * (size_t)n_sets * VEC);
        pl.wf1h[i] = take(16 * (size_t)n_sets * NGT_MAX * 64);
        if (i < 2) pl.Wchi[i] = take(sizeof(f16) * (size_t)n_sets * KP * H2), pl.Wclo[i] = take(sizeof(f16) * (size_t)n_sets * KP * H2);
    }
    pl.wap = take(4 * (size_t)n_sets * 48);
    const size_t rows = (size_t)n_agents * TILE;
    pl.a2 = take(4 * rows), pl.y = take(4 * rows), pl.mu = take(4 * rows), pl.dmu = take(4 * rows), pl.g3 = take(4 * rows);
    pl.sm = take(sizeof(f16) * rows * H2);
    pl.sma = take(sizeof(f16) * rows * H2);
    pl.tz = take(4 * rows);
    pl.t1p = take(2 * 4 * (size_t)n_sets * CriticS::K * H2), pl.s2raw = take(2 * 4 * (size_t)n_sets * H2);
    pl.xfs = take(32 * rows), pl.xfs2 = take(32 * rows);
    for (int i = 0; i < 2; ++i) {
        const int KP = i ? CriticS::KP : ActorS::KP, KG = i ? CriticS::KG : ActorS::KG;
        pl.partM[i] = take(4 * (size_t)pl.grid * 8);
        pl.partV[i] = take(4 * (size_t)pl.grid * KP * 16);
        pl.partG[i] = take(4 * (size_t)pl.grid * KG * H2);
    }
    for (int i = 0; i < 3; ++i) pl.partHs[i] = take(4 * (size_t)pl.grid * 8 * 2);
    pl.bad = take(sizeof(int) + sizeof(unsigned) * 4 * (size_t)n_sets * 2);
    pl.total = o;
    return pl;
}
static int check_shape(const avd_mlp_layout* L, int n_agents, int n_sets, const char* who) {
    AVD_REQUIRE(L, "%s: null layout", who);
    if (L->H1 != H1 || L->H2 != H2 || L->Ha != HA || L->A != 1 || (L->S != 3 && L->S != 4) || L->B != TILE) {
        set_error("%s: serves the reference widths only (layer1 256, layer2 128, action layer 48, A = 1, S in {3, 4}, B = 64); "
                  "got H1=%d H2=%d Ha=%d A=%d S=%d B=%d (avd_learn_shared_bf16 takes other widths)",
                  who, L->H1, L->H2, L->Ha, L->A, L->S, L->B);
        return AVD_E_UNSUPPORTED;
    }
    AVD_REQUIRE(n_sets > 0 && n_sets <= 64 && n_agents > 0 && n_agents % n_sets == 0, "%s: n_agents=%d n_sets=%d", who, n_agents,
                n_sets);
    return AVD_OK;
}

enum Phase { PH_CRITIC = 1, PH_ACTOR = 2, PH_BOTH = 3 };
template <int S>
static int run(int phases, const avd_mlp_layout& L, int n_agents, int n_sets, const float* theta, const float* stats, const float* theta_t,
               const float* stats_t, const float* s, const float* a, const float* r, const float* s2, const float* aw, float gamma,
               float high, float* grads, float* losses, unsigned char* ws, const Plan& pl, hipStream_t st) {
    PrepArgs pa;
    pa.L = L, pa.S = S, pa.theta = theta, pa.stats = stats, pa.theta_t = theta_t, pa.stats_t = stats_t;
    pa.wap = (unsigned*)(ws + pl.wap), pa.bad = (int*)(ws + pl.bad), pa.smax = (unsigned*)(ws + pl.bad + sizeof(int));
    NetP net[4];
    for (int i = 0; i < 4; ++i) {
        const bool critic = i & 1, target = i >= 2;
        pa.Whi[i] = (f16*)(ws + pl.Whi[i]), pa.Wlo[i] = (f16*)(ws + pl.Wlo[i]), pa.vec[i] = (float*)(ws + pl.vec[i]);
        pa.wf1h[i] = (f16x8*)(ws + pl.wf1h[i]);
        pa.Wchi[i] = i < 2 ? (f16*)(ws + pl.Wchi[i]) : nullptr, pa.Wclo[i] = i < 2 ? (f16*)(ws + pl.Wclo[i]) : nullptr;
        NetP& n = net[i];
        n.th = (target ? theta_t : theta) + (critic ? L.actor_size : 0), n.th_stride = L.theta_size;
        n.Whi = pa.Whi[i], n.Wlo = pa.Wlo[i], n.Wchi = pa.Wchi[i], n.Wclo = pa.Wclo[i], n.wf1h = pa.wf1h[i], n.vec = pa.vec[i];
        n.wap = pa.wap;
    }
    const int P = n_agents / n_sets;
    const float inv_n = 1.0f / ((float)P * TILE);
    const long nrows = (long)n_agents * TILE;
    f16x8 *xfs = (f16x8*)(ws + pl.xfs), *xfs2 = (f16x8*)(ws + pl.xfs2);
    int* bad = (int*)(ws + pl.bad);
    float *a2 = (float*)(ws + pl.a2), *y = (float*)(ws + pl.y), *mu = (float*)(ws + pl.mu), *dmu = (float*)(ws + pl.dmu);
    float* g3 = (float*)(ws + pl.g3);
    f16 *sm = (f16*)(ws + pl.sm), *sma = (f16*)(ws + pl.sma);
    auto F = [&](size_t off) { return (float*)(ws + off); };
    const dim3 grid(pl.grid), block(NT);
    HeadArgs h;
    h.n_agents = n_agents, h.n_sets = n_sets, h.gamma = gamma, h.high = high, h.inv_n = inv_n, h.aw = aw, h.sm = sm, h.g3 = g3, h.dmu = dmu;
    h.act2 = nullptr, h.part_s2 = nullptr, h.stamp = nullptr, h.bad = bad, h.part_m = nullptr, h.tz = F(pl.tz), h.abl = 0;
    if (const char* e = AVD_DIAG_ENV("FSPLIT_ABL")) h.abl = atoi(e);
    auto head = [&](auto kern, int ni, const f16x8* x, const float* act, const float* rr, const float* yin, float* out, float* part_s) {
        h.net = net[ni], h.xf = x, h.act = act, h.r = rr, h.yin = yin, h.out = out, h.part_s = part_s;
        hipLaunchKernelGGL(kern, grid, block, 0, st, h);
    };
    DwArgs dw;
    dw.n_agents = n_agents, dw.n_sets = n_sets, dw.sm = sm, dw.g3 = g3, dw.x = s, dw.stamp = nullptr, dw.abl = 0;
    if (const char* e = AVD_DIAG_ENV("FSPLIT_ABL")) dw.abl = atoi(e);
#ifdef AVD_STAMP
    static unsigned long long* d_stamp = nullptr;
    if (!d_stamp) (void)hipMalloc(&d_stamp, 128 * 8);
    dw.stamp = d_stamp;
#endif
    DxArgs dx;
    dx.n_agents = n_agents, dx.n_sets = n_sets, dx.sm = sm, dx.g3 = g3, dx.xfh = xfs, dx.stamp = nullptr, dx.L_cWa = dx.L_cba = 0, dx.unsigned_mask = 0;
    dx.abl = dw.abl;
#ifdef AVD_STAMP
    dx.stamp = d_stamp;
#endif
    FinArgs fa;
    fa.L = L, fa.n_sets = n_sets, fa.J = pl.J, fa.S = S, fa.nrh = 1, fa.theta = theta, fa.stats = stats, fa.grads = grads, fa.losses = losses;
    fa.inv_n = inv_n, fa.partLa = F(pl.partHs[2]), fa.bad = bad;
    for (int i = 0; i < 2; ++i)
        fa.partH[i] = nullptr, fa.partHs[i] = F(pl.partHs[i]), fa.partU[i] = nullptr, fa.partV[i] = F(pl.partV[i]),
        fa.partG[i] = F(pl.partG[i]), fa.c3[i] = F(pl.vec[i]);
    fa.t1_from_g[0] = fa.t1_from_g[1] = 1, fa.t1p = F(pl.t1p), fa.s2raw = F(pl.s2raw);
    if (phases & PH_CRITIC) {
        if (hipMemsetAsync(ws + pl.bad, 0, sizeof(int) + sizeof(unsigned) * 4 * (size_t)n_sets * 2, st) != hipSuccess)
            return check_launch("avd_learn_set_split: memset");
        hipLaunchKernelGGL(scale_kernel, dim3(4, n_sets, SCALE_SLICES), dim3(256), 0, st, pa);
        hipLaunchKernelGGL(prep_kernel, dim3(H2, 4, n_sets), dim3(320), 0, st, pa);
        hipLaunchKernelGGL(prep1_kernel, dim3(NGT_MAX, 4, n_sets), dim3(64), 0, st, pa);
        PackArgs pk;
        pk.x[0] = s, pk.extra[0] = a, pk.outh[0] = xfs, pk.x[1] = s2, pk.extra[1] = r, pk.outh[1] = xfs2, pk.rows = nrows, pk.bad = bad;
        hipLaunchKernelGGL(pack_x_kernel<S>, dim3((unsigned)((2 * nrows + 255) / 256), 2), dim3(256), 0, st, pk);
        head(head_kernel<S, ActorS, OUT_TANH>, 2, xfs2, nullptr, nullptr, nullptr, a2, nullptr);
        head(head_kernel<S, CriticS, OUT_TD>, 3, xfs2, a2, r, nullptr, y, nullptr);
        h.sm = sma;
        head(head_kernel<S, ActorS, OUT_TANH_SAVE>, 0, xfs, nullptr, nullptr, nullptr, mu, nullptr);
        h.sm = sm;
        h.act2 = mu, h.part_s2 = F(pl.partHs[2]), h.part_m = F(pl.partM[1]);
        head(head_kernel<S, CriticS, HEAD_BOTH>, 1, xfs, a, nullptr, y, nullptr, F(pl.partHs[1]));
        dw.net = net[1], dw.act = a, dw.partG = F(pl.partG[1]), dw.part_m = F(pl.partM[1]);
        hipLaunchKernelGGL((dw_kernel<S, CriticS>), grid, block, 0, st, dw);
        dx.net = net[1], dx.partV = F(pl.partV[1]), dx.act = a, dx.part_m = F(pl.partM[1]);
        hipLaunchKernelGGL((dx_kernel<S, CriticS>), grid, block, 0, st, dx);
        dx.L_cWa = L.cWa, dx.L_cba = L.cba;
        hipLaunchKernelGGL((dxa_kernel<S>), grid, block, 0, st, dx);
        if (phases == PH_CRITIC) launch_finalize(fa, st, 1, 1);
    }
    if (phases & PH_ACTOR) {
        SeedArgs sd;
        sd.n_agents = n_agents, sd.n_sets = n_sets, sd.dmu = dmu, sd.tz = F(pl.tz), sd.high = high, sd.g3 = g3, sd.part_m = F(pl.partM[0]),
        sd.part_s = F(pl.partHs[0]);
        hipLaunchKernelGGL(actor_seed_kernel, grid, block, 0, st, sd);
        dw.sm = sma, dx.sm = sma;
        dw.net = net[0], dw.act = nullptr, dw.partG = F(pl.partG[0]), dw.part_m = F(pl.partM[0]);
        hipLaunchKernelGGL((dw_kernel<S, ActorS>), grid, block, 0, st, dw);
        dx.net = net[0], dx.partV = F(pl.partV[0]), dx.act = nullptr, dx.part_m = F(pl.partM[0]), dx.L_cWa = dx.L_cba = 0, dx.unsigned_mask = 1;
        hipLaunchKernelGGL((dx_kernel<S, ActorS>), grid, block, 0, st, dx);
        if (phases == PH_ACTOR) launch_finalize(fa, st, 0, 1);
        else launch_finalize(fa, st, 0, 2);
    }
    return check_launch("avd_learn_set_split");
}

}
}

using namespace avd;

namespace avd { namespace fsplit {
constexpr long MFMA_PER_TILE = 2 * (200 + 238 + 200 + 314)
                               + 8 * (2 + 32 + 1 + 2 * 2 * 2)
                               + 8 * (2 + 32 + 1 + 2 * 1 * 2)
                               + 2 * 8 * (32 + 2 + 8)
                               + 4 * 16;
static_assert(MFMA_PER_TILE == 3296, "update DESIGN.md 3.4 and the count above together");
}}
extern "C" int avd_learn_set_split_mfma_count(const avd_mlp_layout* lay, int n_agents, int n_sets, unsigned long long* mfma_32x32x16) {
    int rc = fsplit::check_shape(lay, n_agents, n_sets, "avd_learn_set_split_mfma_count");
    if (rc) return rc;
    AVD_REQUIRE(mfma_32x32x16, "avd_learn_set_split_mfma_count: null pointer");
    *mfma_32x32x16 = (unsigned long long)fsplit::MFMA_PER_TILE * (unsigned long long)n_agents;
    return AVD_OK;
}

extern "C" int avd_learn_set_split_workspace(const avd_mlp_layout* lay, int n_agents, int n_sets, size_t* bytes) {
    int rc = fsplit::check_shape(lay, n_agents, n_sets, "avd_learn_set_split_workspace");
    if (rc) return rc;
    AVD_REQUIRE(bytes, "avd_learn_set_split_workspace: null pointer");
    *bytes = fsplit::make_plan(n_agents, n_sets).total;
    return AVD_OK;
}

static int split_entry(int phases, const char* who, const avd_mlp_layout* lay, int n_agents, int n_sets, const float* theta, const float* stats,
                       const float* theta_t, const float* stats_t, const float* s, const float* a, const float* r, const float* s2,
                       const float* agent_weight, float gamma, float high, float* grads, float* losses, void* workspace,
                       size_t workspace_bytes, void* stream) {
    int rc = fsplit::check_shape(lay, n_agents, n_sets, who);
    if (rc) return rc;
    const bool cr = phases & fsplit::PH_CRITIC;
    AVD_REQUIRE(theta && stats && s && grads && workspace && (!cr || (theta_t && stats_t && a && r && s2)), "%s: null pointer", who);
    const fsplit::Plan pl = fsplit::make_plan(n_agents, n_sets);
    AVD_REQUIRE(workspace_bytes >= pl.total, "%s: workspace %zu B < %zu B", who, workspace_bytes, pl.total);
    if (cr && hipMemsetAsync(grads, 0, sizeof(float) * (size_t)n_sets * lay->theta_size, (hipStream_t)stream) != hipSuccess)
        return check_launch("avd_learn_set_split: hipMemsetAsync(grads)");
    if (lay->S == 4)
        return fsplit::run<4>(phases, *lay, n_agents, n_sets, theta, stats, theta_t, stats_t, s, a, r, s2, agent_weight, gamma, high, grads,
                              losses, (unsigned char*)workspace, pl, (hipStream_t)stream);
    return fsplit::run<3>(phases, *lay, n_agents, n_sets, theta, stats, theta_t, stats_t, s, a, r, s2, agent_weight, gamma, high, grads, losses,
                          (unsigned char*)workspace, pl, (hipStream_t)stream);
}

extern "C" int avd_learn_set_split_f16x3(const avd_mlp_layout* lay, int n_agents, int n_sets, const float* theta, const float* stats,
                                          const float* theta_t, const float* stats_t, const float* s, const float* a, const float* r,
                                          const float* s2, const float* agent_weight, float gamma, float high, float* grads,
                                          float* losses, void* workspace, size_t workspace_bytes, void* stream) {
    return split_entry(fsplit::PH_BOTH, "avd_learn_set_split_f16x3", lay, n_agents, n_sets, theta, stats, theta_t, stats_t, s, a, r, s2,
                       agent_weight, gamma, high, grads, losses, workspace, workspace_bytes, stream);
}

extern "C" int avd_learn_set_split_bf16x3(const avd_mlp_layout* lay, int n_agents, int n_sets, const float* theta, const float* stats,
                                          const float* theta_t, const float* stats_t, const float* s, const float* a, const float* r,
                                          const float* s2, const float* agent_weight, float gamma, float high, float* grads,
                                          float* losses, void* workspace, size_t workspace_bytes, void* stream) {
    return avd_learn_set_split_f16x3(lay, n_agents, n_sets, theta, stats, theta_t, stats_t, s, a, r, s2, agent_weight, gamma, high, grads,
                                     losses, workspace, workspace_bytes, stream);
}

extern "C" int avd_learn_set_split_critic(const avd_mlp_layout* lay, int n_agents, int n_sets, const float* theta, const float* stats,
                                          const float* theta_t, const float* stats_t, const float* s, const float* a, const float* r,
                                          const float* s2, const float* agent_weight, float gamma, float high, float* grads,
                                          float* losses, void* workspace, size_t workspace_bytes, void* stream) {
    return split_entry(fsplit::PH_CRITIC, "avd_learn_set_split_critic", lay, n_agents, n_sets, theta, stats, theta_t, stats_t, s, a, r, s2,
                       agent_weight, gamma, high, grads, losses, workspace, workspace_bytes, stream);
}

extern "C" int avd_learn_set_split_actor(const avd_mlp_layout* lay, int n_agents, int n_sets, const float* theta, const float* stats,
                                         const float* s, float high, float* grads, void* workspace, size_t workspace_bytes, void* stream) {
    return split_entry(fsplit::PH_ACTOR, "avd_learn_set_split_actor", lay, n_agents, n_sets, theta, stats, nullptr, nullptr, s, nullptr, nullptr,
                       nullptr, nullptr, 0.f, high, grads, nullptr, workspace, workspace_bytes, stream);
}
```

### avddpg_amd/csrc/optim.hip

```cpp
#include <stdlib.h>

#include "common.h"

namespace avd {

constexpr float ADAM_B1 = 0.9f, ADAM_B2 = 0.999f, ADAM_EPS = 1e-7f;

__device__ __forceinline__ bool slab_is_nan(const float* g, int actor_size) {
    const unsigned a = __float_as_uint(g[0]) & 0x7fffffffu, c = __float_as_uint(g[actor_size]) & 0x7fffffffu;
    return a >= 0x7f800000u || c >= 0x7f800000u;
}

template <bool GUARD>
__global__ __launch_bounds__(256) void adam_polyak_kernel(int theta_size, int actor_size, float4* __restrict__ theta,
                                                          float4* __restrict__ theta_t, float4* __restrict__ m,
                                                          float4* __restrict__ v, const float4* __restrict__ grads,
                                                          int32_t* __restrict__ step, float actor_lr,
                                                          float critic_lr, float tau, float omt, int32_t* __restrict__ skipped) {
#pragma clang fp contract(off)
    const int set = blockIdx.y;
    const int t = step[set];
    if (GUARD && slab_is_nan((const float*)grads + (long)set * theta_size, actor_size)) {
        if (blockIdx.x == 0 && threadIdx.x == 0) {
            step[set] = t - 1;
            if (skipped) atomicAdd(skipped, 1);
        }
        return;
    }
    const float b1p = (float)pow((double)ADAM_B1, (double)t);
    const float b2p = (float)pow((double)ADAM_B2, (double)t);
    const float root = sqrtf(1.0f - b2p);
    const float alpha_a = (actor_lr * root) / (1.0f - b1p);
    const float alpha_c = (critic_lr * root) / (1.0f - b1p);
    const int n4 = theta_size / 4;
    const long base = (long)set * n4;
    for (int i = blockIdx.x * blockDim.x + threadIdx.x; i < n4; i += gridDim.x * blockDim.x) {
        const float alpha = (i * 4 < actor_size) ? alpha_a : alpha_c;
        float4 w = theta[base + i], wt = theta_t[base + i], mm = m[base + i], vv = v[base + i];
        const float4 g = grads[base + i];
        float* wp = &w.x;
        float* tp = &wt.x;
        float* mp = &mm.x;
        float* vp = &vv.x;
        const float* gp = &g.x;
#pragma unroll
        for (int k = 0; k < 4; ++k) {
            mp[k] = mp[k] + (gp[k] - mp[k]) * (1.0f - ADAM_B1);
            vp[k] = vp[k] + (gp[k] * gp[k] - vp[k]) * (1.0f - ADAM_B2);
            wp[k] = wp[k] - (mp[k] * alpha) / (sqrtf(vp[k]) + ADAM_EPS);
            tp[k] = wp[k] * tau + tp[k] * omt;
        }
        theta[base + i] = w;
        theta_t[base + i] = wt;
        m[base + i] = mm;
        v[base + i] = vv;
    }
}

__global__ __launch_bounds__(256) void adam_polyak_ranges_kernel(int theta_size, int actor_size,
                                                                 const float4* __restrict__ theta_in,
                                                                 float4* __restrict__ theta_out,
                                                                 float4* __restrict__ theta_t, float4* __restrict__ m,
                                                                 float4* __restrict__ v,
                                                                 const float4* __restrict__ grads,
                                                                 const int32_t* __restrict__ step, float actor_lr,
                                                                 float critic_lr, float tau, float omt, int a0, int a1,
                                                                 int c0, int c1) {
#pragma clang fp contract(off)
    const int set = blockIdx.y;
    const int t = step[set];
    const float b1p = (float)pow((double)ADAM_B1, (double)t);
    const float b2p = (float)pow((double)ADAM_B2, (double)t);
    const float root = sqrtf(1.0f - b2p);
    const float alpha_a = (actor_lr * root) / (1.0f - b1p);
    const float alpha_c = (critic_lr * root) / (1.0f - b1p);
    const int n0 = a0 / 4, n1 = (c0 - a1) / 4, n2 = (theta_size - c1) / 4;
    const long base = (long)set * (theta_size / 4);
    for (int j = blockIdx.x * blockDim.x + threadIdx.x; j < n0 + n1 + n2; j += gridDim.x * blockDim.x) {
        const int i = j < n0 ? j : (j < n0 + n1 ? a1 / 4 + (j - n0) : c1 / 4 + (j - n0 - n1));
        const float alpha = (i * 4 < actor_size) ? alpha_a : alpha_c;
        float4 w = theta_in[base + i], wt = theta_t[base + i], mm = m[base + i], vv = v[base + i];
        const float4 g = grads[base + i];
        float* wp = &w.x;
        float* tp = &wt.x;
        float* mp = &mm.x;
        float* vp = &vv.x;
        const float* gp = &g.x;
#pragma unroll
        for (int k = 0; k < 4; ++k) {
            mp[k] = mp[k] + (gp[k] - mp[k]) * (1.0f - ADAM_B1);
            vp[k] = vp[k] + (gp[k] * gp[k] - vp[k]) * (1.0f - ADAM_B2);
            wp[k] = wp[k] - (mp[k] * alpha) / (sqrtf(vp[k]) + ADAM_EPS);
            tp[k] = wp[k] * tau + tp[k] * omt;
        }
        theta_out[base + i] = w;
        theta_t[base + i] = wt;
        m[base + i] = mm;
        v[base + i] = vv;
    }
}

#ifndef AR_UNR_N
#define AR_UNR_N 4
#endif
constexpr int AR_UNR = AR_UNR_N;
typedef float v4f __attribute__((ext_vector_type(4)));
#define NTL(p) ({ const v4f t_ = __builtin_nontemporal_load((const v4f*)(p)); make_float4(t_[0], t_[1], t_[2], t_[3]); })
#define NTS(val_, p) __builtin_nontemporal_store((v4f){(val_).x, (val_).y, (val_).z, (val_).w}, (v4f*)(p))
__global__ __launch_bounds__(256) void adam_polyak_rows_kernel(int theta_size, int actor_size, int n_sets,
                                                               const float4* __restrict__ theta_in, float4* __restrict__ theta_out,
                                                               float4* __restrict__ theta_t, float4* __restrict__ m,
                                                               float4* __restrict__ v, const float4* __restrict__ grads,
                                                               const int32_t* __restrict__ step, float actor_lr, float critic_lr,
                                                               float tau, float omt) {
#pragma clang fp contract(off)
    const int n4 = theta_size / 4;
    for (int set = blockIdx.x; set < n_sets; set += gridDim.x) {
        const int t = step[set];
        const float b1p = (float)pow((double)ADAM_B1, (double)t);
        const float b2p = (float)pow((double)ADAM_B2, (double)t);
        const float root = sqrtf(1.0f - b2p);
        const float alpha_a = (actor_lr * root) / (1.0f - b1p);
        const float alpha_c = (critic_lr * root) / (1.0f - b1p);
        const long base = (long)set * n4;
        for (int i0 = threadIdx.x; i0 < n4; i0 += 256 * AR_UNR) {
            float4 w[AR_UNR], wt[AR_UNR], mm[AR_UNR], vv[AR_UNR], g[AR_UNR];
#pragma unroll
            for (int u = 0; u < AR_UNR; ++u) {
                const int i = min(i0 + 256 * u, n4 - 1);
                w[u] = NTL(theta_in + base + i), wt[u] = NTL(theta_t + base + i), mm[u] = NTL(m + base + i), vv[u] = NTL(v + base + i);
                g[u] = NTL(grads + base + i);
            }
#pragma unroll
            for (int u = 0; u < AR_UNR; ++u) {
                const int i = i0 + 256 * u;
                if (i >= n4) break;
                const float alpha = (i * 4 < actor_size) ? alpha_a : alpha_c;
                float* wp = &w[u].x;
                float* tp = &wt[u].x;
                float* mp = &mm[u].x;
                float* vp = &vv[u].x;
                const float* gp = &g[u].x;
#pragma unroll
                for (int k = 0; k < 4; ++k) {
                    mp[k] = mp[k] + (gp[k] - mp[k]) * (1.0f - ADAM_B1);
                    vp[k] = vp[k] + (gp[k] * gp[k] - vp[k]) * (1.0f - ADAM_B2);
                    wp[k] = wp[k] - (mp[k] * alpha) / (sqrtf(vp[k]) + ADAM_EPS);
                    tp[k] = wp[k] * tau + tp[k] * omt;
                }
                NTS(w[u], theta_out + base + i), NTS(wt[u], theta_t + base + i), NTS(mm[u], m + base + i), NTS(vv[u], v + base + i);
            }
        }
    }
}

#undef NTL
#undef NTS

constexpr int INTRA_MAX_M = 16;
__global__ __launch_bounds__(256) void adam_polyak_intra_kernel(int theta_size, int actor_size, int M, int lead_skip,
                                                                float4* __restrict__ theta, float4* __restrict__ theta_t,
                                                                float4* __restrict__ m, float4* __restrict__ v,
                                                                const float4* __restrict__ grads, const int32_t* __restrict__ step,
                                                                const float* __restrict__ weights, float actor_lr, float critic_lr,
                                                                float tau, float omt) {
#pragma clang fp contract(off)
    __shared__ float s_aa[INTRA_MAX_M], s_ac[INTRA_MAX_M], s_w[INTRA_MAX_M], s_scale;
    const int p = blockIdx.y, n4 = theta_size / 4;
    const long set0 = (long)p * M;
    if (threadIdx.x < M) {
        const int t = step[set0 + threadIdx.x];
        const float b1p = (float)pow((double)ADAM_B1, (double)t), b2p = (float)pow((double)ADAM_B2, (double)t);
        const float root = sqrtf(1.0f - b2p);
        s_aa[threadIdx.x] = (actor_lr * root) / (1.0f - b1p);
        s_ac[threadIdx.x] = (critic_lr * root) / (1.0f - b1p);
        s_w[threadIdx.x] = weights ? weights[set0 + threadIdx.x] : 1.0f;
    }
    __syncthreads();
    if (threadIdx.x == 0) {
        float ws = 0.f;
        for (int i = 0; i < M; ++i) ws += s_w[i];
        s_scale = 1.0f / ws;
    }
    __syncthreads();
    for (int i4 = blockIdx.x * blockDim.x + threadIdx.x; i4 < n4; i4 += gridDim.x * blockDim.x) {
        float4 acc[4];
#pragma unroll
        for (int k = 0; k < 4; ++k) acc[k] = make_float4(0.f, 0.f, 0.f, 0.f);
        for (int i = 0; i < M; ++i) {
            const float4 g = grads[(set0 + i) * n4 + i4];
            const float w = s_w[i];
            float4& a = acc[i & 3];
            a.x = __builtin_fmaf(w, g.x, a.x), a.y = __builtin_fmaf(w, g.y, a.y), a.z = __builtin_fmaf(w, g.z, a.z), a.w = __builtin_fmaf(w, g.w, a.w);
        }
        float4 r = acc[0];
#pragma unroll
        for (int k = 1; k < 4; ++k) r.x += acc[k].x, r.y += acc[k].y, r.z += acc[k].z, r.w += acc[k].w;
        float gm[4];
        if (weights)
            gm[0] = s_scale * r.x, gm[1] = s_scale * r.y, gm[2] = s_scale * r.z, gm[3] = s_scale * r.w;
        else
            gm[0] = r.x / (float)M, gm[1] = r.y / (float)M, gm[2] = r.z / (float)M, gm[3] = r.w / (float)M;
        const bool actor = i4 * 4 < actor_size;
        for (int i = lead_skip ? 1 : 0; i < M; ++i) {
            const long o = (set0 + i) * n4 + i4;
            const float alpha = actor ? s_aa[i] : s_ac[i];
            float4 w = theta[o], wt = theta_t[o], mm = m[o], vv = v[o];
            float* wp = &w.x;
            float* tp = &wt.x;
            float* mp = &mm.x;
            float* vp = &vv.x;
#pragma unroll
            for (int k = 0; k < 4; ++k) {
                mp[k] = mp[k] + (gm[k] - mp[k]) * (1.0f - ADAM_B1);
                vp[k] = vp[k] + (gm[k] * gm[k] - vp[k]) * (1.0f - ADAM_B2);
                wp[k] = wp[k] - (mp[k] * alpha) / (sqrtf(vp[k]) + ADAM_EPS);
                tp[k] = wp[k] * tau + tp[k] * omt;
            }
            theta[o] = w, theta_t[o] = wt, m[o] = mm, v[o] = vv;
        }
    }
}
__global__ void polyak_intra_kernel(int stats_size, int M, int lead_skip, const float* __restrict__ w, float* __restrict__ t, float tau,
                                    float omt) {
#pragma clang fp contract(off)
    const int set = blockIdx.y;
    if (lead_skip && set % M == 0) return;
    const long base = (long)set * stats_size;
    for (int i = blockIdx.x * blockDim.x + threadIdx.x; i < stats_size; i += gridDim.x * blockDim.x)
        t[base + i] = w[base + i] * tau + t[base + i] * omt;
}

__global__ void polyak_kernel(long n, const float* __restrict__ w, float* __restrict__ t, float tau, float omt) {
#pragma clang fp contract(off)
    for (long i = (long)blockIdx.x * blockDim.x + threadIdx.x; i < n; i += (long)gridDim.x * blockDim.x)
        t[i] = w[i] * tau + t[i] * omt;
}
__global__ void polyak_guarded_kernel(int stats_size, const float* __restrict__ w, float* __restrict__ t, float tau, float omt,
                                      const float* __restrict__ grads, int theta_size, int actor_size) {
#pragma clang fp contract(off)
    const int set = blockIdx.y;
    if (slab_is_nan(grads + (long)set * theta_size, actor_size)) return;
    const long base = (long)set * stats_size;
    for (int i = blockIdx.x * blockDim.x + threadIdx.x; i < stats_size; i += gridDim.x * blockDim.x)
        t[base + i] = w[base + i] * tau + t[base + i] * omt;
}

constexpr int FS_COLS = 64, FS_PH = 4, FS_UNR = 8;
__global__ __launch_bounds__(256) void fed_sum_kernel(int n_in, int so, int si, int n, const float4* __restrict__ g,
                                                      const float* __restrict__ weights, float4* __restrict__ out,
                                                      float* __restrict__ wsum) {
    __shared__ float4 part[FS_PH][FS_COLS];
    const int n4 = n / 4;
    const int o = blockIdx.y;
    if (wsum && blockIdx.x == 0 && threadIdx.x == 0) {
        float s = 0.f;
        for (int i = 0; i < n_in; ++i) s += weights[(long)o * so + (long)i * si];
        wsum[o] = s;
    }
    const int col = threadIdx.x % FS_COLS, ph = threadIdx.x / FS_COLS;
    const int j = blockIdx.x * FS_COLS + col;
    float4 acc = make_float4(0.f, 0.f, 0.f, 0.f);
    if (j < n4) {
        for (int i0 = ph; i0 < n_in; i0 += FS_PH * FS_UNR) {
            float4 x[FS_UNR];
            float w[FS_UNR];
#pragma unroll
            for (int u = 0; u < FS_UNR; ++u) {
                const int i = i0 + FS_PH * u;
                const long row = (long)o * so + (long)(i < n_in ? i : ph) * si;
                x[u] = g[row * n4 + j];
                w[u] = i < n_in ? (weights ? weights[row] : 1.0f) : 0.0f;
            }
#pragma unroll
            for (int u = 0; u < FS_UNR; ++u)
                if (i0 + FS_PH * u < n_in) acc.x += w[u] * x[u].x, acc.y += w[u] * x[u].y, acc.z += w[u] * x[u].z, acc.w += w[u] * x[u].w;
        }
    }
    part[ph][col] = acc;
    __syncthreads();
    if (ph == 0 && j < n4) {
        float4 r = part[0][col];
#pragma unroll
        for (int p = 1; p < FS_PH; ++p) r.x += part[p][col].x, r.y += part[p][col].y, r.z += part[p][col].z, r.w += part[p][col].w;
        out[(long)o * n4 + j] = r;
    }
}

__global__ void fed_finalize_kernel(int n_out, int n, float* __restrict__ out, float count,
                                    const float* __restrict__ wsum) {
#pragma clang fp contract(off)
    const long total = (long)n_out * n;
    for (long i = (long)blockIdx.x * blockDim.x + threadIdx.x; i < total; i += (long)gridDim.x * blockDim.x) {
        if (wsum)
            out[i] = (1.0f / wsum[i / n]) * out[i];
        else
            out[i] = out[i] / count;
    }
}

__global__ void fed_scatter_kernel(int so, int si, int i_begin, int n, const float4* __restrict__ src,
                                   float4* __restrict__ dst) {
    const int n4 = n / 4;
    const int o = blockIdx.z, i = blockIdx.y + i_begin;
    const long row = (long)o * so + (long)i * si;
    for (int j = blockIdx.x * blockDim.x + threadIdx.x; j < n4; j += gridDim.x * blockDim.x)
        dst[row * n4 + j] = src[(long)o * n4 + j];
}

}

using namespace avd;

static int adam_polyak_launch(const char* who, bool guard, const avd_mlp_layout* lay, int n_sets, float* theta, float* stats, float* theta_t,
                              float* stats_t, float* m, float* v, const float* grads, int32_t* step, float actor_lr, float critic_lr,
                              double tau, int32_t* skipped, void* stream) {
    AVD_REQUIRE(lay && n_sets > 0, "%s: n_sets=%d", who, n_sets);
    AVD_REQUIRE(theta && stats && theta_t && stats_t && m && v && grads && step, "%s: null pointer", who);
    AVD_REQUIRE(lay->theta_size % 4 == 0 && lay->actor_size % 4 == 0 && lay->stats_size % 4 == 0, "%s: layout not 4-float aligned", who);
    const float tauf = (float)tau, omt = (float)(1.0 - tau);
    const int n4 = lay->theta_size / 4;
    int gx = (n4 + 255) / 256;
    if (n_sets >= 256 && gx > 8) gx = 8;
    if (const char* e = AVD_DIAG_ENV("ADAM_GX")) gx = atoi(e);
    if (guard)
        hipLaunchKernelGGL(adam_polyak_kernel<true>, dim3(gx, n_sets), dim3(256), 0, (hipStream_t)stream, lay->theta_size, lay->actor_size,
                           (float4*)theta, (float4*)theta_t, (float4*)m, (float4*)v, (const float4*)grads, step, actor_lr, critic_lr, tauf,
                           omt, skipped);
    else
        hipLaunchKernelGGL(adam_polyak_kernel<false>, dim3(gx, n_sets), dim3(256), 0, (hipStream_t)stream, lay->theta_size, lay->actor_size,
                           (float4*)theta, (float4*)theta_t, (float4*)m, (float4*)v, (const float4*)grads, step, actor_lr, critic_lr, tauf,
                           omt, (int32_t*)nullptr);
    int rc = check_launch(who);
    if (rc) return rc;
    if (guard) {
        hipLaunchKernelGGL(polyak_guarded_kernel, dim3((unsigned)((lay->stats_size + 255) / 256), n_sets), dim3(256), 0, (hipStream_t)stream,
                           lay->stats_size, stats, stats_t, tauf, omt, grads, lay->theta_size, lay->actor_size);
        return check_launch(who);
    }
    const long ns = (long)n_sets * lay->stats_size;
    long blocks = (ns + 255) / 256;
    if (blocks > 2048) blocks = 2048;
    hipLaunchKernelGGL(polyak_kernel, dim3((unsigned)blocks), dim3(256), 0, (hipStream_t)stream, ns, stats, stats_t,
                       tauf, omt);
    return check_launch(who);
}

__global__ void fed_history_push_kernel(int P, int M, int W, float* __restrict__ ep_reward, const uint8_t* __restrict__ done,
                                        const int32_t* __restrict__ ep_len, int limit, const int32_t* __restrict__ cond, int force,
                                        int zero_after, float* __restrict__ ring, int32_t* __restrict__ hist_cnt) {
    const int p = blockIdx.x * blockDim.x + threadIdx.x;
    if (p >= P) return;
    bool end = force != 0 || (cond && *cond != 0);
    if (!end && done) end = done[p] != 0 || (ep_len && ep_len[p] + 1 >= limit);
    if (!end) return;
    const int c = hist_cnt[p], slot = c % W;
    for (int m = 0; m < M; ++m) {
        const long v = (long)p * M + m;
        ring[v * W + slot] = ep_reward[v];
        if (zero_after) ep_reward[v] = 0.f;
    }
    hist_cnt[p] = c + 1;
}

__global__ void fed_weights_w_kernel(long n, int W, const float* __restrict__ ring, float* __restrict__ w_cand) {
    const long v = (long)blockIdx.x * blockDim.x + threadIdx.x;
    if (v >= n) return;
    float acc = 0.f;
    for (int k = 0; k < W; ++k) acc += ring[v * W + k];
    w_cand[v] = fabsf(1.0f / (acc / (float)W));
}
__global__ __launch_bounds__(1024) void fed_weights_kernel(int P, int M, int W, const int32_t* __restrict__ hist_cnt, int host_enabled,
                                                           float* __restrict__ w_raw, float* __restrict__ aw, float* __restrict__ wsum) {
    __shared__ float part[1024];
    __shared__ int cmin[1024];
    const int m = blockIdx.x, tid = threadIdx.x;
    int enabled = host_enabled;
    if (host_enabled < 0) {
        int c = 0x7fffffff;
        for (int p = tid; p < P; p += 1024) c = min(c, hist_cnt[p]);
        cmin[tid] = c;
        __syncthreads();
        for (int o = 512; o > 0; o >>= 1) {
            if (tid < o) cmin[tid] = min(cmin[tid], cmin[tid + o]);
            __syncthreads();
        }
        enabled = cmin[0] >= W ? 1 : 0;
    }
    float s = 0.f;
    for (int p = tid; p < P; p += 1024) {
        const long v = (long)p * M + m;
        const float w = enabled ? w_raw[v] : 1.0f;
        w_raw[v] = w;
        s += w;
    }
    part[tid] = s;
    __syncthreads();
    for (int o = 512; o > 0; o >>= 1) {
        if (tid < o) part[tid] += part[tid + o];
        __syncthreads();
    }
    const float total = part[0];
    if (tid == 0) wsum[m] = total;
    const float f = (float)P / total;
    for (int p = tid; p < P; p += 1024) {
        const long v = (long)p * M + m;
        aw[v] = enabled ? w_raw[v] * f : 1.0f;
    }
}

extern "C" int avd_adam_polyak_f32(const avd_mlp_layout* lay, int n_sets, float* theta, float* stats, float* theta_t,
                                   float* stats_t, float* m, float* v, const float* grads, const int32_t* step,
                                   float actor_lr, float critic_lr, double tau, void* stream) {
    return adam_polyak_launch("avd_adam_polyak_f32", false, lay, n_sets, theta, stats, theta_t, stats_t, m, v, grads, (int32_t*)step, actor_lr,
                              critic_lr, tau, nullptr, stream);
}

extern "C" int avd_adam_polyak_guarded_f32(const avd_mlp_layout* lay, int n_sets, float* theta, float* stats, float* theta_t,
                                           float* stats_t, float* m, float* v, const float* grads, int32_t* step, float actor_lr,
                                           float critic_lr, double tau, int32_t* skipped, void* stream) {
    return adam_polyak_launch("avd_adam_polyak_guarded_f32", true, lay, n_sets, theta, stats, theta_t, stats_t, m, v, grads, step, actor_lr,
                              critic_lr, tau, skipped, stream);
}

int launch_adam_polyak_ranges(const avd_mlp_layout* lay, int n_sets, const float* theta_in, float* theta_out,
                              float* theta_t, float* m, float* v, const float* grads, const int32_t* step,
                              float actor_lr, float critic_lr, double tau, int skip_a0, int skip_a1, int skip_c0,
                              int skip_c1, void* stream) {
    AVD_REQUIRE(skip_a0 % 4 == 0 && skip_a1 % 4 == 0 && skip_c0 % 4 == 0 && skip_c1 % 4 == 0 && skip_a1 <= skip_c0,
                "launch_adam_polyak_ranges: skip ranges must be 4-float aligned and ordered");
    const int kept4 = (lay->theta_size - (skip_a1 - skip_a0) - (skip_c1 - skip_c0)) / 4;
    int gx = (kept4 + 255) / 256;
    hipLaunchKernelGGL(adam_polyak_ranges_kernel, dim3(gx, n_sets), dim3(256), 0, (hipStream_t)stream, lay->theta_size,
                       lay->actor_size, (const float4*)theta_in, (float4*)theta_out, (float4*)theta_t, (float4*)m,
                       (float4*)v, (const float4*)grads, step, actor_lr, critic_lr, (float)tau, (float)(1.0 - tau),
                       skip_a0, skip_a1, skip_c0, skip_c1);
    return check_launch("avd_learn_update_f32(small tensors)");
}

int launch_adam_polyak_rows(const avd_mlp_layout* lay, int n_sets, int n_groups, const float* theta_in, float* theta_out, float* theta_t,
                            float* m, float* v, const float* grads, const int32_t* step, float actor_lr, float critic_lr, double tau,
                            void* stream) {
    AVD_REQUIRE(lay->theta_size % 4 == 0 && lay->actor_size % 4 == 0 && n_groups > 0, "launch_adam_polyak_rows: layout not 4-float aligned");
    hipLaunchKernelGGL(adam_polyak_rows_kernel, dim3(n_groups < n_sets ? n_groups : n_sets), dim3(256), 0, (hipStream_t)stream,
                       lay->theta_size, lay->actor_size, n_sets, (const float4*)theta_in, (float4*)theta_out, (float4*)theta_t, (float4*)m,
                       (float4*)v, (const float4*)grads, step, actor_lr, critic_lr, (float)tau, (float)(1.0 - tau));
    return check_launch("avd_learn_update_f32(update pass)");
}

extern "C" int avd_polyak_f32(int64_t n, const float* w, float* t, double tau, void* stream) {
    AVD_REQUIRE(n > 0 && w && t, "avd_polyak_f32: n=%ld", (long)n);
    long blocks = (n + 255) / 256;
    if (blocks > 2048) blocks = 2048;
    hipLaunchKernelGGL(polyak_kernel, dim3((unsigned)blocks), dim3(256), 0, (hipStream_t)stream, (long)n, w, t,
                       (float)tau, (float)(1.0 - tau));
    return check_launch("avd_polyak_f32");
}

extern "C" int avd_fed_sum_f32(int n_out, int n_in, int stride_out, int stride_in, int n, const float* g,
                               const float* weights, float* out, float* wsum, void* stream) {
    AVD_REQUIRE(n_out > 0 && n_in > 0 && n > 0 && n % 4 == 0 && g && out, "avd_fed_sum_f32: n_out=%d n_in=%d n=%d",
                n_out, n_in, n);
    AVD_REQUIRE(n_out <= 65535, "avd_fed_sum_f32: n_out=%d exceeds the grid limit", n_out);
    AVD_REQUIRE(!wsum || weights, "avd_fed_sum_f32: wsum requested without weights");
    const int gx = (n / 4 + FS_COLS - 1) / FS_COLS;
    hipLaunchKernelGGL(fed_sum_kernel, dim3(gx, n_out), dim3(256), 0, (hipStream_t)stream, n_in, stride_out,
                       stride_in, n, (const float4*)g, weights, (float4*)out, wsum);
    return check_launch("avd_fed_sum_f32");
}

extern "C" int avd_fed_finalize_f32(int n_out, int n, float* out, float count, const float* wsum, void* stream) {
    AVD_REQUIRE(n_out > 0 && n > 0 && out && (wsum || count > 0.f), "avd_fed_finalize_f32: n_out=%d n=%d", n_out, n);
    long blocks = ((long)n_out * n + 255) / 256;
    if (blocks > 2048) blocks = 2048;
    hipLaunchKernelGGL(fed_finalize_kernel, dim3((unsigned)blocks), dim3(256), 0, (hipStream_t)stream, n_out, n, out,
                       count, wsum);
    return check_launch("avd_fed_finalize_f32");
}

extern "C" int avd_fed_scatter_f32(int n_out, int n_in, int stride_out, int stride_in, int i_begin, int n,
                                   const float* src, float* dst, void* stream) {
    AVD_REQUIRE(n_out > 0 && n_in > 0 && i_begin >= 0 && i_begin < n_in && n > 0 && n % 4 == 0 && src && dst,
                "avd_fed_scatter_f32: n_out=%d n_in=%d i_begin=%d n=%d", n_out, n_in, i_begin, n);
    AVD_REQUIRE(n_out <= 65535 && n_in <= 65535, "avd_fed_scatter_f32: group counts exceed the grid limit");
    int gx = (n / 4 + 255) / 256;
    if (gx > 16) gx = 16;
    hipLaunchKernelGGL(fed_scatter_kernel, dim3(gx, n_in - i_begin, n_out), dim3(256), 0, (hipStream_t)stream,
                       stride_out, stride_in, i_begin, n, (const float4*)src, (float4*)dst);
    return check_launch("avd_fed_scatter_f32");
}

extern "C" int avd_fed_history_push_f32(int P, int M, int W, float* ep_reward, const uint8_t* done, const int32_t* ep_len, int limit,
                                        const int32_t* cond, int force, int zero_after, float* ring, int32_t* hist_cnt, void* stream) {
    AVD_REQUIRE(P > 0 && M > 0 && W > 0 && ep_reward && ring && hist_cnt, "avd_fed_history_push_f32: P=%d M=%d W=%d", P, M, W);
    AVD_REQUIRE(force || cond || (done && (!ep_len || limit >= 1)), "avd_fed_history_push_f32: no closing condition given");
    hipLaunchKernelGGL(fed_history_push_kernel, dim3((P + 255) / 256), dim3(256), 0, (hipStream_t)stream, P, M, W, ep_reward, done,
                       ep_len, limit, cond, force, zero_after, ring, hist_cnt);
    return check_launch("avd_fed_history_push_f32");
}

extern "C" int avd_fed_weights_f32(int P, int M, int W, const float* ring, const int32_t* hist_cnt, int host_enabled, float* w_raw,
                                   float* agent_weight, float* wsum, void* stream) {
    AVD_REQUIRE(P > 0 && M > 0 && M <= 65535 && W > 0 && ring && hist_cnt && w_raw && agent_weight && wsum,
                "avd_fed_weights_f32: P=%d M=%d W=%d", P, M, W);
    const long n = (long)P * M;
    hipLaunchKernelGGL(fed_weights_w_kernel, dim3((unsigned)((n + 255) / 256)), dim3(256), 0, (hipStream_t)stream, n, W, ring, w_raw);
    hipLaunchKernelGGL(fed_weights_kernel, dim3(M), dim3(1024), 0, (hipStream_t)stream, P, M, W, hist_cnt, host_enabled, w_raw,
                       agent_weight, wsum);
    return check_launch("avd_fed_weights_f32");
}

extern "C" int avd_adam_polyak_intra_f32(const avd_mlp_layout* lay, int P, int M, int lead_skip, float* theta, float* stats, float* theta_t,
                                         float* stats_t, float* m, float* v, const float* grads, const int32_t* step, const float* weights,
                                         float actor_lr, float critic_lr, double tau, void* stream) {
    AVD_REQUIRE(lay && P > 0 && M > 0 && M <= INTRA_MAX_M && P <= 65535, "avd_adam_polyak_intra_f32: P=%d M=%d (M <= %d)", P, M, INTRA_MAX_M);
    AVD_REQUIRE(theta && stats && theta_t && stats_t && m && v && grads && step, "avd_adam_polyak_intra_f32: null pointer");
    AVD_REQUIRE(lay->theta_size % 4 == 0 && lay->actor_size % 4 == 0, "avd_adam_polyak_intra_f32: layout not 4-float aligned");
    const float tauf = (float)tau, omt = (float)(1.0 - tau);
    const int n4 = lay->theta_size / 4;
    int gx = (n4 + 255) / 256;
    if (P >= 64 && gx > 8) gx = 8;
    hipLaunchKernelGGL(adam_polyak_intra_kernel, dim3(gx, P), dim3(256), 0, (hipStream_t)stream, lay->theta_size, lay->actor_size, M,
                       lead_skip ? 1 : 0, (float4*)theta, (float4*)theta_t, (float4*)m, (float4*)v, (const float4*)grads, step, weights,
                       actor_lr, critic_lr, tauf, omt);
    int rc = check_launch("avd_adam_polyak_intra_f32");
    if (rc) return rc;
    hipLaunchKernelGGL(polyak_intra_kernel, dim3((unsigned)((lay->stats_size + 255) / 256), (unsigned)(P * M)), dim3(256), 0,
                       (hipStream_t)stream, lay->stats_size, M, lead_skip ? 1 : 0, stats, stats_t, tauf, omt);
    return check_launch("avd_adam_polyak_intra_f32");
}
```

### avddpg_amd/vec.py

```python
import ctypes as C

import numpy as np
import torch

from . import _hip, dynamics, params
from ._hip import call, ptr, stream_handle


def _dev(device):
    return torch.device(device if device is not None else "cuda")


class VecPlatoon:

    def __init__(self, num_platoons, length, config, device=None, rand_states=True, evaluator_states_enabled=False,
                 rng="host", seed=1, track_aux=False):
        self.P, self.L, self.config = int(num_platoons), int(length), config
        self.length = self.L
        self.device = _dev(device)
        self.rng, self.seed = rng, int(seed)
        self.rand_states, self.evaluator_states_enabled = rand_states, evaluator_states_enabled
        centralized = config.framework == config.cntrl
        self.multiplier = self.L if centralized else 1
        self.hidden_multiplier = config.centrl_hidd_mult if centralized else 1
# ... 52 lines not shown
                    draws[p, i, 0] = self._rand(c.reset_ep_max)
                    draws[p, i, 1] = self._rand(c.reset_max_ev)
                    draws[p, i, 2] = self._rand(c.reset_max_a)
        self._upload_reset(draws, self.front_accel)

    def _upload_reset(self, draws, fa, cond=None):
        d = torch.from_numpy(draws.astype(np.float32)).to(self.device) if draws is not None else None
        f = torch.from_numpy(np.asarray(fa, dtype=np.float32)).to(self.device) if fa is not None else None
        call("avd_env_reset_f32", ptr(self.d_consts), self.P, self.L, ptr(self.x), ptr(self.prev_a),
             ptr(self.cum_accel), ptr(d), ptr(f), self._mode(), self.seed, self.reset_count, ptr(cond),
             stream_handle())

    def _host_reset_draws(self):
        c, P, L = self.config, self.P, self.L
        draws = np.zeros((P, L, 3), dtype=np.float64)
        fa = np.zeros(P, dtype=np.float64)
        train = self._mode() == 0
        for p in range(P):
            fa[p] = self._rand(c.pl_leader_reset_a)
            for i in range(L):
                self.front_u[p] = self._rand(c.reset_max_u)
                if train:
                    draws[p, i, 0] = self._rand(c.reset_ep_max)
                    draws[p, i, 1] = self._rand(c.reset_max_ev)
                    draws[p, i, 2] = self._rand(c.reset_max_a)
        self.front_accel = fa.copy()
        return draws, fa

    def observations(self, x=None):
        x = self.x if x is None else x
        return x[..., : self.obs_width]

    def reset(self, cond=None):
        draws = fa = None
        if self.rng == "host":
            if cond is not None:
                raise ValueError("conditional reset needs rng='device'")
            draws, fa = self._host_reset_draws()
        self._upload_reset(draws, fa, cond)
        self.reset_count += 1
        return self.observations()

    def episode_end(self, ep_reward, M, limit, any_reset=None):
        if self.rng != "device":
            raise ValueError("per-platoon episode ends need rng='device'")
        self.ensure_episode_state()
        st = self.ep_stats
        call("avd_episode_end_f32", ptr(self.d_consts), self.P, self.L, M, ptr(self.x), ptr(self.prev_a), ptr(self.cum_accel),
             ptr(self.done), ptr(self.ep_len), ptr(ep_reward), int(limit), ptr(st["ret_sum"]), ptr(st["len_sum"]),
             ptr(st["count"]), ptr(any_reset), self._mode(), self.seed, self.reset_count, stream_handle())
        self.reset_count += 1

    def ensure_episode_state(self):
        if self.ep_len is None:
            z = lambda dt: torch.zeros(self.P, dtype=dt, device=self.device)
            self.ep_len = z(torch.int32)
            self.ep_stats = dict(ret_sum=z(torch.float32), len_sum=z(torch.float32), count=z(torch.int32))

    def pop_episode_stats(self):
        st = self.ep_stats
        n = int(st["count"].sum())
        ret, ln = float(st["ret_sum"].double().sum()), float(st["len_sum"].double().sum())
        for t in st.values():
            t.zero_()
        return (ret / n if n else float("nan")), (ln / n if n else float("nan")), n

    def step(self, actions, leader_exog):
        self.x, self.x_prev = self.x_prev, self.x
        call("avd_env_step_f32", ptr(self.d_consts), self.P, self.L, ptr(self.x_prev), ptr(self.x), ptr(self.prev_a),
             ptr(self.cum_accel), ptr(actions), ptr(leader_exog), ptr(self.reward), ptr(self.term), ptr(self.done),
             ptr(self.reward_mean), ptr(self.any_done), stream_handle())
        self.step_count += 1
        return self.observations(), self.reward, self.done

    def get_jerk_from(self, x_before, prev_a_before):
        return (x_before[..., 2] - prev_a_before) / self.config.sample_rate


class VecOUNoise:

    def __init__(self, n, config, device=None, rng="host", seed=1, mean=0.0):
        self.n, self.config, self.device = int(n), config, _dev(device)
        self.rng, self.seed, self.calls = rng, int(seed), 0
        self.mean = float(mean)
        self.state = torch.zeros(self.n, dtype=torch.float32, device=self.device)

    def reset(self):
        self.state.zero_()

    def __call__(self, normals=None):
        c = self.config
        d_n = None
        if self.rng == "host":
            if normals is None:
                normals = np.random.normal(0, 1.0, size=self.n)
            d_n = torch.from_numpy(np.asarray(normals, dtype=np.float32).reshape(self.n)).to(self.device)
        call("avd_ou_step_f32", self.n, ptr(self.state), ptr(d_n), c.theta, self.mean, c.ou_dt, c.std_dev, self.seed,
             self.calls, stream_handle())
        self.calls += 1
        return self.state


class VecReplay:

    def __init__(self, n_agents, buffer_capacity, batch_size, num_states, num_actions, device=None, rng="host",
                 seed=1, ring=None):
        self.n, self.cap, self.B = int(n_agents), int(buffer_capacity), int(batch_size)
        self.S, self.A = int(num_states), int(num_actions)
        self.row = 2 * self.S + self.A + 1
        self.device, self.rng, self.seed = _dev(device), rng, int(seed)
        if ring is not None:
            if tuple(ring.shape) != (self.n, self.cap, self.row) or ring.dtype != torch.float32 or not ring.is_contiguous():
                raise _hip.AvdError(f"replay ring must be contiguous float32 {(self.n, self.cap, self.row)}, got {tuple(ring.shape)}")
            self.ring = ring
        else:
            self.ring = torch.zeros(self.n, self.cap, self.row, dtype=torch.float32, device=self.device)
        self.buffer_counter = 0
        self.samples = 0
        f32 = dict(dtype=torch.float32, device=self.device)
        self.idx = torch.zeros(self.n, self.B, dtype=torch.int32, device=self.device)
        self.s = torch.zeros(self.n, self.B, self.S, **f32)
        self.a = torch.zeros(self.n, self.B, self.A, **f32)
        self.r = torch.zeros(self.n, self.B, **f32)
        self.s2 = torch.zeros(self.n, self.B, self.S, **f32)

    def add(self, s_prev, action, reward, s_next, x_stride):
        call("avd_replay_add_f32", self.n, self.cap, self.S, self.A, ptr(self.ring), self.buffer_counter, ptr(s_prev),
             ptr(s_next), x_stride, ptr(action), ptr(reward), stream_handle())
        self.buffer_counter += 1

    def sample_range(self):
        return min(self.buffer_counter, self.cap)

    def draw_indices(self, host_idx=None):
        if self.rng == "host":
            if host_idx is None:
                rr = self.sample_range()
                host_idx = np.stack([np.random.choice(rr, self.B) for _ in range(self.n)])
            self.idx.copy_(torch.from_numpy(np.asarray(host_idx).astype(np.int32)))
        else:
            call("avd_replay_indices", self.n, self.B, self.sample_range(), self.seed, self.samples, ptr(self.idx),
                 stream_handle())
        self.samples += 1
        return self.idx

    def gather(self):
        call("avd_replay_gather_f32", self.n, self.cap, self.S, self.A, self.B, ptr(self.ring), ptr(self.idx),
             ptr(self.s), ptr(self.a), ptr(self.r), ptr(self.s2), stream_handle())
        return self.s, self.a, self.r, self.s2

    def sample(self, host_idx=None):
        if self.rng != "host" and host_idx is None and self.A == 1 and self.S in (3, 4) and self.B % 4 == 0:
            call("avd_replay_sample_f32", self.n, self.cap, self.S, self.A, self.B, ptr(self.ring), self.sample_range(), self.seed,
                 self.samples, ptr(self.idx), ptr(self.s), ptr(self.a), ptr(self.r), ptr(self.s2), stream_handle())
            self.samples += 1
            return self.s, self.a, self.r, self.s2
        self.draw_indices(host_idx)
        return self.gather()


class AgentGroup:

    def __init__(self, n_sets, num_states, num_actions, config, device=None, hidd_mult=1, seed=None, high_bound=None):
        c = config
        self.config, self.device, self.n_sets = c, _dev(device), int(n_sets)
        if (c.critic_layer1_size, c.critic_layer2_size) != (c.actor_layer1_size, c.actor_layer2_size):
            raise _hip.AvdError("actor and critic layer1/layer2 sizes must match (reference defaults do)")
        self.dims = params.Dims(num_states, num_actions, int(c.actor_layer1_size * hidd_mult),
                                int(c.actor_layer2_size * hidd_mult), int(c.critic_act_layer_size * hidd_mult))
        H1p, H2p, Hap = params.padded_widths(self.dims.H1, self.dims.H2, self.dims.Ha)
        self.lay = _hip.make_layout(num_states, num_actions, H1p, H2p, Hap, c.batch_size)
        self.high = float(c.action_high if high_bound is None else high_bound)
        f32 = dict(dtype=torch.float32, device=self.device)
        n, T, S = self.n_sets, self.lay.theta_size, self.lay.stats_size
        self.theta = torch.zeros(n, T, **f32)
        self.stats = torch.zeros(n, S, **f32)
        self.theta_t = torch.zeros(n, T, **f32)
        self.stats_t = torch.zeros(n, S, **f32)
        self.m = torch.zeros(n, T, **f32)
        self.v = torch.zeros(n, T, **f32)
        self.step = torch.zeros(n, dtype=torch.int32, device=self.device)
        self._layp = C.byref(self.lay)
        rs = np.random.RandomState(c.random_seed if seed is None else seed)
        th, st = params.init_weights(self.lay, rs, nominal=(c.actor_layer1_size, c.actor_layer2_size), dims=self.dims)
        self.theta.copy_(torch.from_numpy(th).to(self.device).expand(n, T))
        self.stats.copy_(torch.from_numpy(st).to(self.device).expand(n, S))
        self.theta_t.copy_(self.theta)
        self.stats_t.copy_(self.stats)

    def actor(self, states, set_mod, x_stride=None, out=None, target=False, run_if_nonzero=None):
        n_agents = states.shape[0]
        x_stride = states.shape[-1] if x_stride is None else x_stride
        shape = (n_agents,) if self.lay.A == 1 else (n_agents, self.lay.A)
        out = torch.empty(*shape, dtype=torch.float32, device=self.device) if out is None else out
        th, st = (self.theta_t, self.stats_t) if target else (self.theta, self.stats)
        if run_if_nonzero is not None:
            call("avd_actor_forward_cond_f32", self._layp, n_agents, set_mod, ptr(th), ptr(st), ptr(states), x_stride,
                 self.high, ptr(out), ptr(run_if_nonzero), stream_handle())
        else:
            call("avd_actor_forward_f32", self._layp, n_agents, set_mod, ptr(th), ptr(st), ptr(states), x_stride,
                 self.high, ptr(out), stream_handle())
        return out

    def actor_set(self, states, n_agents, x_stride=None, out=None, run_if_nonzero=None):
        x_stride = states.shape[-1] if x_stride is None else x_stride
        out = torch.empty(n_agents, dtype=torch.float32, device=self.device) if out is None else out
        call("avd_actor_forward_set_f32", self._layp, n_agents, self.n_sets, ptr(self.theta), ptr(self.stats), ptr(states), x_stride,
             self.high, ptr(out), ptr(run_if_nonzero), stream_handle())
        return out

    def critic(self, states, actions, set_mod, x_stride=None, out=None, target=False):
        n_agents = states.shape[0]
        x_stride = states.shape[-1] if x_stride is None else x_stride
        shape = (n_agents,) if self.lay.A == 1 else (n_agents, self.lay.A)
        out = torch.empty(*shape, dtype=torch.float32, device=self.device) if out is None else out
        th, st = (self.theta_t, self.stats_t) if target else (self.theta, self.stats)
        call("avd_critic_forward_f32", self._layp, n_agents, set_mod, ptr(th), ptr(st), ptr(states), x_stride,
             ptr(actions), ptr(out), stream_handle())
        return out

    def learn(self, s, a, r, s2, set_mod, grads=None, losses=None):
        n_agents = s.shape[0]
        if grads is None:
            grads = torch.empty(n_agents, self.lay.theta_size, dtype=torch.float32, device=self.device)
        call("avd_learn_f32", self._layp, n_agents, set_mod, ptr(self.theta), ptr(self.stats), ptr(self.theta_t),
             ptr(self.stats_t), ptr(s), ptr(a), ptr(r), ptr(s2), self.config.gamma, self.high, ptr(grads),
             ptr(losses), stream_handle())
        return grads

    def learn_shared(self, s, a, r, s2, n_agents, grads=None, losses=None, row_weight=None):
        import ctypes
        if grads is None:
            grads = torch.empty(self.n_sets, self.lay.theta_size, dtype=torch.float32, device=self.device)
        need = ctypes.c_size_t(0)
        call("avd_learn_shared_workspace", self._layp, n_agents, self.n_sets, ctypes.byref(need))
        ws = getattr(self, "_wide_ws", None)
        if ws is None or ws.numel() < need.value:
            ws = self._wide_ws = torch.empty(need.value, dtype=torch.uint8, device=self.device)
        call("avd_learn_shared_bf16", self._layp, n_agents, self.n_sets, ptr(self.theta), ptr(self.stats),
             ptr(self.theta_t), ptr(self.stats_t), ptr(s), ptr(a), ptr(r), ptr(s2), ptr(row_weight), self.config.gamma,
             self.high, ptr(grads), ptr(losses), ptr(ws), ws.numel(), stream_handle())
        return grads

    def learn_set_fused(self, s, a, r, s2, n_agents, grads=None, losses=None, agent_weight=None, split=False, phase=None):
        import ctypes
        self._check_agent_major(s, a, r, s2, n_agents, agent_weight)
        if grads is None:
            grads = torch.empty(self.n_sets, self.lay.theta_size, dtype=torch.float32, device=self.device)
        wsf, fn, attr = (("avd_learn_set_split_workspace", "avd_learn_set_split_f16x3", "_fsplit_ws") if split else
                         ("avd_learn_set_fused_workspace", "avd_learn_set_fused_bf16", "_fset_ws"))
        need = ctypes.c_size_t(0)
        call(wsf, self._layp, n_agents, self.n_sets, ctypes.byref(need))
        ws = getattr(self, attr, None)
        if ws is None or ws.numel() < need.value:
            ws = torch.empty(need.value, dtype=torch.uint8, device=self.device)
            setattr(self, attr, ws)
        if phase is not None and not split:
            raise _hip.AvdError("phase= needs split=True (csrc/fsplit.hip)")
        if phase == "actor":
            call("avd_learn_set_split_actor", self._layp, n_agents, self.n_sets, ptr(self.theta), ptr(self.stats), ptr(s), self.high,
                 ptr(grads), ptr(ws), ws.numel(), stream_handle())
            return grads
        if phase not in (None, "critic"):
            raise _hip.AvdError(f"phase={phase!r}")
        call("avd_learn_set_split_critic" if phase == "critic" else fn, self._layp, n_agents, self.n_sets, ptr(self.theta), ptr(self.stats),
             ptr(self.theta_t), ptr(self.stats_t), ptr(s), ptr(a), ptr(r), ptr(s2), ptr(agent_weight), self.config.gamma, self.high,
             ptr(grads), ptr(losses), ptr(ws), ws.numel(), stream_handle())
        return grads

    def learn_set_split(self, s, a, r, s2, n_agents, grads=None, losses=None, agent_weight=None):
        return self.learn_set_fused(s, a, r, s2, n_agents, grads=grads, losses=losses, agent_weight=agent_weight, split=True)

    def _check_agent_major(self, s, a, r, s2, n_agents, agent_weight):
        lay = self.lay
        want = {"s": (n_agents, lay.B, lay.S), "s2": (n_agents, lay.B, lay.S), "r": (n_agents, lay.B)}
        for name, x in (("s", s), ("s2", s2), ("r", r)):
            if tuple(x.shape) != want[name] or x.dtype != torch.float32 or not x.is_contiguous():
                raise _hip.AvdError(f"set learner: {name} must be contiguous float32 {want[name]} (agent-major), got "
                                    f"{tuple(x.shape)} {x.dtype} contiguous={x.is_contiguous()}")
        if a.numel() != n_agents * lay.B * lay.A or a.dtype != torch.float32 or not a.is_contiguous() or a.shape[0] != n_agents:
            raise _hip.AvdError(f"set learner: a must be contiguous float32 [{n_agents}, {lay.B}(, {lay.A})], got {tuple(a.shape)} {a.dtype}")
        if n_agents <= 0 or n_agents % self.n_sets:
            raise _hip.AvdError(f"set learner: n_agents={n_agents} is not a multiple of n_sets={self.n_sets}")
        if agent_weight is not None and (agent_weight.numel() != n_agents or agent_weight.dtype != torch.float32
                                         or not agent_weight.is_contiguous()):
            raise _hip.AvdError(f"set learner: agent_weight must be contiguous float32 [{n_agents}]")

    def actor_shared(self, states_set_major, n_agents, out=None):
        import ctypes
        rows = n_agents // self.n_sets
        if out is None:
            out = torch.empty(self.n_sets, rows, dtype=torch.float32, device=self.device)
        need = ctypes.c_size_t(0)
        call("avd_actor_forward_shared_workspace", self._layp, n_agents, self.n_sets, ctypes.byref(need))
        ws = getattr(self, "_wide_act_ws", None)
        if ws is None or ws.numel() < need.value:
            ws = self._wide_act_ws = torch.empty(need.value, dtype=torch.uint8, device=self.device)
        call("avd_actor_forward_shared_bf16", self._layp, n_agents, self.n_sets, ptr(self.theta), ptr(self.stats),
             ptr(states_set_major), self.high, ptr(out), ptr(ws), ws.numel(), stream_handle())
        return out

    def apply(self, grads, guarded=False):
        c = self.config
        self.step += 1
        if guarded:
            if getattr(self, "nonfinite_skipped", None) is None:
                self.nonfinite_skipped = torch.zeros(1, dtype=torch.int32, device=self.device)
            call("avd_adam_polyak_guarded_f32", self._layp, self.n_sets, ptr(self.theta), ptr(self.stats), ptr(self.theta_t),
                 ptr(self.stats_t), ptr(self.m), ptr(self.v), ptr(grads), ptr(self.step), c.actor_lr, c.critic_lr,
                 float(c.tau), ptr(self.nonfinite_skipped), stream_handle())
            return
        call("avd_adam_polyak_f32", self._layp, self.n_sets, ptr(self.theta), ptr(self.stats), ptr(self.theta_t),
             ptr(self.stats_t), ptr(self.m), ptr(self.v), ptr(grads), ptr(self.step), c.actor_lr, c.critic_lr,
             float(c.tau), stream_handle())

    def apply_intra(self, grads, P, M, weights=None, lead_skip=False, lo=0, hi=None, stream=None, advance=True):
        c = self.config
        hi = P if hi is None else hi
        if self.n_sets != P * M:
            raise _hip.AvdError("apply_intra needs one weight set per agent (P * M sets)")
        if advance:
            if stream is None:
                self.step.view(P, M)[lo:hi, (1 if lead_skip else 0):] += 1
            else:
                with torch.cuda.stream(stream):
                    self.step.view(P, M)[lo:hi, (1 if lead_skip else 0):] += 1
        a, b = lo * M, hi * M
        call("avd_adam_polyak_intra_f32", self._layp, hi - lo, M, 1 if lead_skip else 0, ptr(self.theta[a:b]), ptr(self.stats[a:b]),
             ptr(self.theta_t[a:b]), ptr(self.stats_t[a:b]), ptr(self.m[a:b]), ptr(self.v[a:b]), ptr(grads[a:b]), ptr(self.step[a:b]),
             ptr(None if weights is None else weights.reshape(-1)[a:b]), c.actor_lr, c.critic_lr, float(c.tau),
             stream_handle() if stream is None else _hip.C.c_void_p(stream.cuda_stream))

    def learn_apply_intra(self, s, a, r, s2, grads, P, M, losses=None, chunks=8, weights=None, lead_skip=False, timers=None):
        main = torch.cuda.current_stream()
        if getattr(self, "_side", None) is None:
            self._side = torch.cuda.Stream(device=self.device)
        side = self._side
        c = self.config
        chunks = max(1, min(chunks, P))
        bounds = [(P * i) // chunks for i in range(chunks + 1)]
        T = lambda: torch.cuda.Event(enable_timing=timers is not None)
        self.step.view(P, M)[:, (1 if lead_skip else 0):] += 1
        for i in range(chunks):
            lo, hi = bounds[i] * M, bounds[i + 1] * M
            if hi == lo:
                continue
            t0, t1 = T(), T()
            if timers is not None:
                t0.record(main)
            call("avd_learn_f32", self._layp, hi - lo, 0, ptr(self.theta[lo:hi]), ptr(self.stats[lo:hi]), ptr(self.theta_t[lo:hi]),
                 ptr(self.stats_t[lo:hi]), ptr(s[lo:hi]), ptr(a[lo:hi]), ptr(r[lo:hi]), ptr(s2[lo:hi]), c.gamma, self.high,
                 ptr(grads[lo:hi]), ptr(losses[lo:hi]) if losses is not None else None, _hip.C.c_void_p(main.cuda_stream))
            t1.record(main)
            side.wait_event(t1)
            u0, u1 = T(), T()
            if timers is not None:
                u0.record(side)
            self.apply_intra(grads, P, M, weights=weights, lead_skip=lead_skip, lo=bounds[i], hi=bounds[i + 1], stream=side, advance=False)
            if timers is not None:
                u1.record(side)
                timers.setdefault("learn", []).append((t0, t1))
                timers.setdefault("update", []).append((u0, u1))
        done = torch.cuda.Event()
        done.record(side)
        main.wait_event(done)

    def learn_update(self, s, a, r, s2, grads, losses=None, next_states=None, x_stride=None, next_actions=None):
        n = self.n_sets
        if s.shape[0] != n:
            raise _hip.AvdError("learn_update needs one weight set per agent (set_mod == 0)")
        if getattr(self, "theta_alt", None) is None:
            self.theta_alt = self.theta.clone()
        c = self.config
        self.step += 1
        args = (self._layp, n, ptr(self.theta), ptr(self.stats), ptr(self.theta_alt), ptr(self.theta_t), ptr(self.stats_t),
                ptr(self.m), ptr(self.v), ptr(self.step), ptr(s), ptr(a), ptr(r), ptr(s2), c.gamma, self.high, c.actor_lr,
                c.critic_lr, float(c.tau), ptr(grads), ptr(losses))
        if next_actions is not None:
            if self.lay.A != 1:
                raise _hip.AvdError("next-action epilogue: A == 1 only")
            xs = next_states.shape[-1] if x_stride is None else x_stride
            call("avd_learn_update_act_f32", *args, ptr(next_states), xs, ptr(next_actions), stream_handle())
        else:
            call("avd_learn_update_f32", *args, stream_handle())
        self.theta, self.theta_alt = self.theta_alt, self.theta

    def learn_apply(self, s, a, r, s2, grads, losses=None, chunks=4, timers=None):
        n = self.n_sets
        if s.shape[0] != n:
            raise _hip.AvdError("learn_apply needs one weight set per agent (set_mod == 0)")
        main = torch.cuda.current_stream()
        if getattr(self, "_side", None) is None:
            self._side = torch.cuda.Stream(device=self.device)
        side = self._side
        c = self.config
        self.step += 1
        chunks = max(1, min(chunks, n))
        bounds = [(n * i) // chunks for i in range(chunks + 1)]
        T = lambda: torch.cuda.Event(enable_timing=timers is not None)
        for i in range(chunks):
            lo, hi = bounds[i], bounds[i + 1]
            if hi == lo:
                continue
            t0, t1 = T(), T()
            if timers is not None:
                t0.record(main)
            call("avd_learn_f32", self._layp, hi - lo, 0, ptr(self.theta[lo:hi]), ptr(self.stats[lo:hi]),
                 ptr(self.theta_t[lo:hi]), ptr(self.stats_t[lo:hi]), ptr(s[lo:hi]), ptr(a[lo:hi]), ptr(r[lo:hi]),
                 ptr(s2[lo:hi]), c.gamma, self.high, ptr(grads[lo:hi]), ptr(losses[lo:hi]) if losses is not None else None,
                 _hip.C.c_void_p(main.cuda_stream))
            t1.record(main)
            side.wait_event(t1)
            u0, u1 = T(), T()
            if timers is not None:
                u0.record(side)
            call("avd_adam_polyak_f32", self._layp, hi - lo, ptr(self.theta[lo:hi]), ptr(self.stats[lo:hi]),
                 ptr(self.theta_t[lo:hi]), ptr(self.stats_t[lo:hi]), ptr(self.m[lo:hi]), ptr(self.v[lo:hi]),
                 ptr(grads[lo:hi]), ptr(self.step[lo:hi]), c.actor_lr, c.critic_lr, float(c.tau),
                 _hip.C.c_void_p(side.cuda_stream))
            if timers is not None:
                u1.record(side)
                timers.setdefault("learn", []).append((t0, t1))
                timers.setdefault("update", []).append((u0, u1))
        done = torch.cuda.Event()
        done.record(side)
        main.wait_event(done)

    def get_weights(self, set_idx, which, target=False, trainable_only=False):
        th, st = (self.theta_t, self.stats_t) if target else (self.theta, self.stats)
        return params.unpack(self.lay, th[set_idx].cpu().numpy(), st[set_idx].cpu().numpy(), which, trainable_only,
                             dims=self.dims)

    def set_weights(self, set_idx, which, weights, target=False):
        th, st = (self.theta_t, self.stats_t) if target else (self.theta, self.stats)
        h_th, h_st = th[set_idx].cpu().numpy(), st[set_idx].cpu().numpy()
        params.pack(self.lay, weights, h_th, h_st, which, dims=self.dims)
        th[set_idx].copy_(torch.from_numpy(h_th))
        st[set_idx].copy_(torch.from_numpy(h_st))

    def grads_as_lists(self, grads_row):
        g = grads_row.cpu().numpy()
        dummy = np.zeros(self.lay.stats_size, dtype=np.float32)
        return (params.unpack(self.lay, g, dummy, "critic", trainable_only=True, dims=self.dims),
                params.unpack(self.lay, g, dummy, "actor", trainable_only=True, dims=self.dims))


def fed_mean(grads, P, M, weights=None, group=None, method="interfrl", total=None):
    n = grads.shape[-1]
    if method == "interfrl":
        n_out, n_in, so, si = M, P, 1, M
    elif method == "intrafrl":
        n_out, n_in, so, si = P, M, M, 1
    else:
        raise ValueError(method)
    out = torch.empty(n_out, n, dtype=torch.float32, device=grads.device)
    wsum = torch.empty(n_out, dtype=torch.float32, device=grads.device) if weights is not None else None
    call("avd_fed_sum_f32", n_out, n_in, so, si, n, ptr(grads), ptr(weights), ptr(out), ptr(wsum), stream_handle())
    count = float(n_in)
    if group is not None and method == "interfrl":
        from .dist import exchange_fed_sums
        count = exchange_fed_sums(out, wsum, n_in, group, total=total)
    call("avd_fed_finalize_f32", n_out, n, ptr(out), count, ptr(wsum), stream_handle())
    return out


def fed_scatter(avg, dst, P, M, method="interfrl", i_begin=0):
    n = avg.shape[-1]
    n_out, n_in, so, si = (M, P, 1, M) if method == "interfrl" else (P, M, M, 1)
    call("avd_fed_scatter_f32", n_out, n_in, so, si, i_begin, n, ptr(avg), ptr(dst), stream_handle())
    return dst
```

### include/avddpg_hip.h

```cpp
#ifndef AVDDPG_HIP_H
#define AVDDPG_HIP_H

#include <stddef.h>
#include <stdint.h>

#ifdef __cplusplus
extern "C" {
#pragma GCC visibility push(default)
#endif

#define AVD_MAX_L 16

#define AVD_OK 0
#define AVD_E_INVALID (-1)
#define AVD_E_LAUNCH (-2)
#define AVD_E_UNSUPPORTED (-3)

typedef struct avd_env_consts {
    int32_t L;
    int32_t model_a;
    int32_t can_terminate;
    int32_t uniform_reset;
    float max_ep, max_ev;
    float abs_action_high;
    float two_max_a;
    float T;
    float ca, cb, cc, cd;
    float re_scalar, terminal_reward;
    float stand_still, timegap;
    float reset_ep_max, reset_max_ev, reset_max_a;
    float reset_ep_eval, reset_ev_eval, reset_a_eval;
    float leader_reset_a;
    float A[AVD_MAX_L][16];
    float B[AVD_MAX_L][4];
    float C[AVD_MAX_L][4];
} avd_env_consts;

typedef struct avd_mlp_layout {
    int32_t S, A, H1, H2, Ha, B;
    int32_t aW1, ab1, ag1, abe1, aW2, ab2, ag2, abe2, aW3, ab3;
    int32_t actor_size;
    int32_t cWs, cbs, cgs, cbes, cWa, cba, cga, cbea, cW2, cb2, cg3, cbe3, cW3, cb3;
    int32_t theta_size;
    int32_t amm1, amv1, amm2, amv2, cmms, cmvs, cmma, cmva, cmm3, cmv3;
    int32_t stats_size;
} avd_mlp_layout;

const char* avd_last_error(void);
int avd_version(void);
int avd_diagnostics_enabled(void);

int avd_mlp_layout_init(avd_mlp_layout* out, int S, int A, int H1, int H2, int Ha, int B);

int avd_env_step_f32(const avd_env_consts* d_consts, int P, int L, const float* x_in, float* x_out, float* prev_a,
                     float* cum_accel, const float* u, const float* leader_exog, float* reward, uint8_t* term,
                     uint8_t* done, float* reward_mean, int32_t* any_done, void* stream);

int avd_env_reset_f32(const avd_env_consts* d_consts, int P, int L, float* x, float* prev_a, float* cum_accel,
                      const float* draws, const float* front_accel, int mode, uint64_t seed, uint64_t counter,
                      const int32_t* cond, void* stream);

int avd_episode_end_f32(const avd_env_consts* d_consts, int P, int L, int M, float* x, float* prev_a, float* cum_accel,
                        const uint8_t* done, int32_t* ep_len, float* ep_reward, int limit, float* ret_sum, float* len_sum,
                        int32_t* ep_cnt, int32_t* any_reset, int mode, uint64_t seed, uint64_t counter, void* stream);


int avd_ou_step_f32(int n, float* ou_state, const float* normals, float theta, float mean, float dt, float std_dev,
                    uint64_t seed, uint64_t counter, void* stream);

int avd_policy_f32(int n, const float* actor_out, const float* noise, float lo, float hi, float* action,
                   void* stream);

int avd_normal_f32(int n, float* out, float std_dev, uint64_t seed, uint64_t counter, void* stream);

int avd_uniform_f32(int n, float* out, float half_width, uint64_t seed, uint64_t counter, void* stream);

int avd_replay_add_f32(int n_agents, int cap, int S, int A, float* ring, int64_t counter, const float* s_prev,
                       const float* s_next, int x_stride, const float* action, const float* reward, void* stream);

int avd_replay_indices(int n_agents, int B, int range, uint64_t seed, uint64_t counter, int32_t* idx, void* stream);

int avd_replay_gather_f32(int n_agents, int cap, int S, int A, int B, const float* ring, const int32_t* idx, float* s,
                          float* a, float* r, float* s2, void* stream);


int avd_actor_forward_f32(const avd_mlp_layout* lay, int n_agents, int set_mod, const float* theta, const float* stats,
                          const float* state, int x_stride, float high, float* out, void* stream);

int avd_actor_forward_cond_f32(const avd_mlp_layout* lay, int n_agents, int set_mod, const float* theta,
                               const float* stats, const float* state, int x_stride, float high, float* out,
                               const int32_t* run_if_nonzero, void* stream);

int avd_critic_forward_f32(const avd_mlp_layout* lay, int n_agents, int set_mod, const float* theta,
                           const float* stats, const float* state, int x_stride, const float* action, float* q,
                           void* stream);

int avd_learn_f32(const avd_mlp_layout* lay, int n_agents, int set_mod, const float* theta, const float* stats,
                  const float* theta_t, const float* stats_t, const float* s, const float* a, const float* r,
                  const float* s2, float gamma, float high, float* grads, float* losses, void* stream);

int avd_adam_polyak_f32(const avd_mlp_layout* lay, int n_sets, float* theta, float* stats, float* theta_t,
                        float* stats_t, float* m, float* v, const float* grads, const int32_t* step, float actor_lr,
                        float critic_lr, double tau, void* stream);

int avd_adam_polyak_guarded_f32(const avd_mlp_layout* lay, int n_sets, float* theta, float* stats, float* theta_t, float* stats_t,
                                float* m, float* v, const float* grads, int32_t* step, float actor_lr, float critic_lr, double tau,
                                int32_t* skipped, void* stream);

int avd_learn_update_f32(const avd_mlp_layout* lay, int n_agents, const float* theta, const float* stats,
                         float* theta_out, float* theta_t, float* stats_t, float* m, float* v, const int32_t* step,
                         const float* s, const float* a, const float* r, const float* s2, float gamma, float high,
                         float actor_lr, float critic_lr, double tau, float* grads_scratch, float* losses,
                         void* stream);

int avd_learn_update_plan(const avd_mlp_layout* lay, int n_agents, int* chunk_agents, int* n_chunks, int* update_groups);

int avd_learn_update_act_f32(const avd_mlp_layout* lay, int n_agents, const float* theta, const float* stats,
                             float* theta_out, float* theta_t, float* stats_t, float* m, float* v, const int32_t* step,
                             const float* s, const float* a, const float* r, const float* s2, float gamma, float high,
                             float actor_lr, float critic_lr, double tau, float* grads_scratch, float* losses,
                             const float* next_state, int x_stride, float* next_action, void* stream);

int avd_polyak_f32(int64_t n, const float* w, float* t, double tau, void* stream);

int avd_fed_sum_f32(int n_out, int n_in, int stride_out, int stride_in, int n, const float* g, const float* weights,
                    float* out, float* wsum, void* stream);
int avd_fed_finalize_f32(int n_out, int n, float* out, float count, const float* wsum, void* stream);
int avd_fed_scatter_f32(int n_out, int n_in, int stride_out, int stride_in, int i_begin, int n, const float* src,
                        float* dst, void* stream);

int avd_adam_polyak_intra_f32(const avd_mlp_layout* lay, int P, int M, int lead_skip, float* theta, float* stats, float* theta_t,
                              float* stats_t, float* m, float* v, const float* grads, const int32_t* step, const float* weights,
                              float actor_lr, float critic_lr, double tau, void* stream);

int avd_fed_history_push_f32(int P, int M, int W, float* ep_reward, const uint8_t* done, const int32_t* ep_len, int limit,
                             const int32_t* cond, int force, int zero_after, float* ring, int32_t* hist_cnt, void* stream);
int avd_fed_weights_f32(int P, int M, int W, const float* ring, const int32_t* hist_cnt, int host_enabled, float* w_raw,
                        float* agent_weight, float* wsum, void* stream);

int avd_step_fused_f32(const avd_env_consts* d_consts, int P, int L, int S, const float* x_in, float* x_out, float* prev_a,
                       float* cum_accel, float* reward, uint8_t* term, uint8_t* done, int32_t* any_done, int32_t* any_done_other,
                       const float* actor_out, float* ou_state, float* action, float* leader_exog, float ou_theta, float ou_mean,
                       float ou_dt, float ou_std_dev, float action_low, float action_high, float exog_scale, int exog_uniform,
                       uint64_t seed, uint64_t ou_counter, uint64_t exog_counter, float* ring, int cap, int64_t replay_counter,
                       float* ep_reward, void* stream);

int avd_replay_sample_f32(int n_agents, int cap, int S, int A, int B, const float* ring, int range, uint64_t seed, uint64_t counter,
                          int32_t* idx, float* s, float* a, float* r, float* s2, void* stream);

int avd_actor_forward_set_f32(const avd_mlp_layout* lay, int n_agents, int n_sets, const float* theta, const float* stats,
                              const float* states, int x_stride, float high, float* out, const int32_t* run_if_nonzero, void* stream);

int avd_learn_shared_workspace(const avd_mlp_layout* lay, int n_agents, int n_sets, size_t* bytes);
int avd_learn_shared_bf16(const avd_mlp_layout* lay, int n_agents, int n_sets, const float* theta, const float* stats,
                          const float* theta_t, const float* stats_t, const float* s, const float* a, const float* r,
                          const float* s2, const float* row_weight, float gamma, float high, float* grads, float* losses,
                          void* workspace, size_t workspace_bytes, void* stream);

int avd_learn_set_fused_workspace(const avd_mlp_layout* lay, int n_agents, int n_sets, size_t* bytes);
int avd_learn_set_fused_bf16(const avd_mlp_layout* lay, int n_agents, int n_sets, const float* theta, const float* stats,
                             const float* theta_t, const float* stats_t, const float* s, const float* a, const float* r,
                             const float* s2, const float* agent_weight, float gamma, float high, float* grads, float* losses,
                             void* workspace, size_t workspace_bytes, void* stream);

int avd_learn_set_split_mfma_count(const avd_mlp_layout* lay, int n_agents, int n_sets, unsigned long long* mfma_32x32x16);
int avd_learn_set_split_critic(const avd_mlp_layout* lay, int n_agents, int n_sets, const float* theta, const float* stats,
                               const float* theta_t, const float* stats_t, const float* s, const float* a, const float* r,
                               const float* s2, const float* agent_weight, float gamma, float high, float* grads, float* losses,
                               void* workspace, size_t workspace_bytes, void* stream);
int avd_learn_set_split_actor(const avd_mlp_layout* lay, int n_agents, int n_sets, const float* theta, const float* stats,
                              const float* s, float high, float* grads, void* workspace, size_t workspace_bytes, void* stream);
int avd_learn_set_split_workspace(const avd_mlp_layout* lay, int n_agents, int n_sets, size_t* bytes);
int avd_learn_set_split_f16x3(const avd_mlp_layout* lay, int n_agents, int n_sets, const float* theta, const float* stats,
                               const float* theta_t, const float* stats_t, const float* s, const float* a, const float* r,
                               const float* s2, const float* agent_weight, float gamma, float high, float* grads, float* losses,
                               void* workspace, size_t workspace_bytes, void* stream);

int avd_learn_set_split_bf16x3(const avd_mlp_layout* lay, int n_agents, int n_sets, const float* theta, const float* stats,
                               const float* theta_t, const float* stats_t, const float* s, const float* a, const float* r,
                               const float* s2, const float* agent_weight, float gamma, float high, float* grads, float* losses,
                               void* workspace, size_t workspace_bytes, void* stream);

int avd_actor_forward_shared_workspace(const avd_mlp_layout* lay, int n_agents, int n_sets, size_t* bytes);
int avd_actor_forward_shared_bf16(const avd_mlp_layout* lay, int n_agents, int n_sets, const float* theta,
                                  const float* stats, const float* state, float high, float* out, void* workspace,
                                  size_t workspace_bytes, void* stream);

int avd_gemm_bt_bf16(int M, int Nc, int K, const void* A, long lda, const void* B, long ldb, float* D, long ldd,
                     void* stream);

#ifdef __cplusplus
#pragma GCC visibility pop
}
#endif
#endif
```

Before: 1.989 million.

## Fuse memsets, prep kernels and Adam step increment to cut launch count

```diff
diff --git a/avddpg_amd/_hip.py b/avddpg_amd/_hip.py
--- a/avddpg_amd/_hip.py
+++ b/avddpg_amd/_hip.py
@@ -67,6 +67,7 @@
     "avd_learn_update_plan": [_LP, _i, C.POINTER(C.c_int), C.POINTER(C.c_int), C.POINTER(C.c_int)],
     "avd_adam_polyak_f32": [_LP, _i, _P, _P, _P, _P, _P, _P, _P, _P, _f, _f, _d, _P],
     "avd_adam_polyak_guarded_f32": [_LP, _i, _P, _P, _P, _P, _P, _P, _P, _P, _f, _f, _d, _P, _P],
+    "avd_adam_polyak_guarded_step_f32": [_LP, _i, _P, _P, _P, _P, _P, _P, _P, _P, _P, _f, _f, _d, _P, _P],
     "avd_polyak_f32": [_i64, _P, _P, _d, _P],
     "avd_fed_sum_f32": [_i, _i, _i, _i, _i, _P, _P, _P, _P, _P],
     "avd_fed_finalize_f32": [_i, _i, _P, _f, _P, _P],
diff --git a/avddpg_amd/csrc/fset.hip b/avddpg_amd/csrc/fset.hip
--- a/avddpg_amd/csrc/fset.hip
+++ b/avddpg_amd/csrc/fset.hip
@@ -708,6 +708,19 @@
         for (int o = 1; o < 32; o <<= 1) v += __shfl_xor(v, o);
         return v;
     };
+    __shared__ float db2s[H2];
+    const bool feat_block = a.item_base + blockIdx.z * 16 >= H2;
+    if (feat_block && a.partU[net] == nullptr) {
+        const int KG = critic ? Critic::KG : Actor::KG;
+        for (int n = tid >> 5; n < H2; n += 16) {
+            float S2 = 0.f;
+            for (int j = jl; j < a.J; j += 32) S2 += a.partG[net][(((long)j * a.n_sets + set) * KG + K) * H2 + n];
+            S2 = allsum(S2);
+            if (a.c3[net]) S2 *= a.c3[net][(long)set * VEC + H2 + n];
+            if (jl == 0) db2s[n] = S2;
+        }
+        __syncthreads();
+    }
     if (item < H2) {
         const int n = item;
         const int og2 = critic ? L.cg3 : L.ag2, obe2 = critic ? L.cbe3 : L.abe2, omm2 = critic ? L.cmm3 : L.amm2, omv2 = critic ? L.cmv3 : L.amv2;
@@ -738,7 +751,10 @@
             }
             g[obe2 + n] = w3 * D;
             g[ob2 + n] = S2;
-            if (n == 0) g[ob3] = D;
+            if (n == 0) {
+                g[ob3] = D;
+                for (int k = L.A; k & 3; ++k) g[ob3 + k] = 0.f;
+            }
             if (critic && n == 0 && a.losses) a.losses[2 * set] = Lc * a.inv_n, a.losses[2 * set + 1] = -La * a.inv_n;
         }
         return;
@@ -766,9 +782,9 @@
 #pragma unroll
     for (int k = 0; k < 9; ++k) V[k] = allsum(V[k]);
     if (!have_u) {
-        const int oW2 = critic ? L.cW2 : L.aW2, ob2 = critic ? L.cb2 : L.ab2;
+        const int oW2 = critic ? L.cW2 : L.aW2;
         float u0 = 0.f;
-        for (int n = jl; n < H2; n += 32) u0 = fmaf(th[oW2 + (long)f * H2 + n], g[ob2 + n], u0);
+        for (int n = jl; n < H2; n += 32) u0 = fmaf(th[oW2 + (long)f * H2 + n], db2s[n], u0);
         U0 = allsum(u0);
         int oW, ob, ff = f, ld = H1, sin = a.S;
         if (!critic) oW = L.aW1, ob = L.ab1;
@@ -822,8 +838,10 @@
     if (a.bad && *a.bad) G = __uint_as_float(0x7fc00000u);
     g[oW2 + (long)f * H2 + n] = inv1 * G + sh1 * g[ob2 + n];
 }
-__global__ __launch_bounds__(128) void finalize_t1_kernel(const FinArgs a) {
-    const int set = blockIdx.x, net = a.net_lo + blockIdx.y, n = threadIdx.x;
+constexpr int T1_THREADS = 1024;
+__global__ __launch_bounds__(T1_THREADS) void finalize_t1_kernel(const FinArgs a) {
+    __shared__ __attribute__((aligned(16))) float tl[Critic::K * H2];
+    const int set = blockIdx.x, net = a.net_lo + blockIdx.y, tid = threadIdx.x, n = tid;
     if (!a.t1_from_g[net]) return;
     const bool critic = net;
     const avd_mlp_layout& L = a.L;
@@ -833,17 +851,13 @@
     const int K = critic ? Critic::K : Actor::K;
     const int og2 = critic ? L.cg3 : L.ag2, obe2 = critic ? L.cbe3 : L.abe2, omm2 = critic ? L.cmm3 : L.amm2, omv2 = critic ? L.cmv3 : L.amv2;
     const int oW3 = critic ? L.cW3 : L.aW3, ob3 = critic ? L.cb3 : L.ab3;
-    const float* tp = a.t1p + ((long)net * a.n_sets + set) * Critic::K * H2 + n;
+    const float4* tp = (const float4*)(a.t1p + ((long)net * a.n_sets + set) * Critic::K * H2);
+    for (int i = tid; i < K * H2 / 4; i += T1_THREADS) ((float4*)tl)[i] = tp[i];
+    __syncthreads();
+    if (n >= H2) return;
     float T1 = 0.f;
-    int f = 0;
-    for (; f + 8 <= K; f += 8) {
-        float v[8];
-#pragma unroll
-        for (int u = 0; u < 8; ++u) v[u] = tp[(long)(f + u) * H2];
-#pragma unroll
-        for (int u = 0; u < 8; ++u) T1 += v[u];
-    }
-    for (; f < K; ++f) T1 += tp[(long)f * H2];
+#pragma unroll 16
+    for (int f = 0; f < K; ++f) T1 += tl[f * H2 + n];
     T1 = fmaf(a.c3[net][(long)set * VEC + n], a.s2raw[((long)net * a.n_sets + set) * H2 + n], T1);
     const float D = g[ob3];
     if (a.bad && *a.bad) T1 = __uint_as_float(0x7fc00000u);
@@ -857,17 +871,11 @@
     FinArgs fa = fa0;
     fa.net_lo = net_lo, fa.item_base = 0;
     const int K = (net_lo + n_nets > 1) ? Critic::K : Actor::K;
-    if (fa.partU[net_lo]) {
-        hipLaunchKernelGGL(finalize_small_kernel, dim3(fa.n_sets, n_nets, (H2 + K + 15) / 16), dim3(512), 0, st, fa);
-    } else {
-        hipLaunchKernelGGL(finalize_small_kernel, dim3(fa.n_sets, n_nets, H2 / 16), dim3(512), 0, st, fa);
-        fa.item_base = H2;
-        hipLaunchKernelGGL(finalize_small_kernel, dim3(fa.n_sets, n_nets, (K + 15) / 16), dim3(512), 0, st, fa);
-    }
+    hipLaunchKernelGGL(finalize_small_kernel, dim3(fa.n_sets, n_nets, (H2 + K + 15) / 16), dim3(512), 0, st, fa);
     hipLaunchKernelGGL(finalize_w2_kernel, dim3(K, fa.n_sets, n_nets), dim3(H2), 0, st, fa);
     bool any = false;
     for (int net = net_lo; net < net_lo + n_nets; ++net) any = any || fa.t1_from_g[net];
-    if (any) hipLaunchKernelGGL(finalize_t1_kernel, dim3(fa.n_sets, n_nets), dim3(H2), 0, st, fa);
+    if (any) hipLaunchKernelGGL(finalize_t1_kernel, dim3(fa.n_sets, n_nets), dim3(T1_THREADS), 0, st, fa);
 }
 
 struct Plan {
diff --git a/avddpg_amd/csrc/fsplit.hip b/avddpg_amd/csrc/fsplit.hip
--- a/avddpg_amd/csrc/fsplit.hip
+++ b/avddpg_amd/csrc/fsplit.hip
@@ -161,6 +161,8 @@
     unsigned* wap;
     unsigned* smax;
     int* bad;
+    float4* zero;
+    long n_zero4;
 };
 constexpr int SCALE_SLICES = 16;
 __device__ __forceinline__ float pow2_for(float mx) {
@@ -202,13 +204,59 @@
         __syncthreads();
     }
     if (tid == 0) {
-        unsigned* dst = a.smax + ((long)net * gridDim.y + set) * 2;
-        atomicMax(dst, __float_as_uint(red[0]));
-        atomicMax(dst + 1, __float_as_uint(red2[0]));
-    }
-}
+        unsigned* dst = a.smax + (((long)net * gridDim.y + set) * SCALE_SLICES + slice) * 2;
+        dst[0] = __float_as_uint(red[0]);
+        dst[1] = __float_as_uint(red2[0]);
+    }
+    if (net == 0 && set == 0 && slice == 0 && tid == 0) *a.bad = 0;
+    if (a.zero) {
+        const long nb = (long)gridDim.x * gridDim.y * gridDim.z, b = ((long)slice * gridDim.y + set) * gridDim.x + net;
+        for (long i = b * 256 + tid; i < a.n_zero4; i += nb * 256) a.zero[i] = make_float4(0.f, 0.f, 0.f, 0.f);
+    }
+}
+__device__ __forceinline__ void prep1_tile(const PrepArgs& a, int ft, int net, int set, int lane) {
+    const int r = lane & 31, h = lane >> 5;
+    const bool critic = net & 1, target = net >= 2;
+    const avd_mlp_layout& L = a.L;
+    const float* th = (target ? a.theta_t : a.theta) + (long)set * L.theta_size + (critic ? L.actor_size : 0);
+    const int K = critic ? CriticS::K : ActorS::K;
+    const int f = 32 * ft + r;
+    float w[4] = {0.f, 0.f, 0.f, 0.f}, b = 0.f;
+    if (f == K) {
+        b = 1.f;
+    } else if (f < K) {
+        if (critic && ft >= 8) {
+            w[0] = th[L.cWa + (f - H1)], b = th[L.cba + (f - H1)];
+        } else {
+            const float* W = th + (critic ? L.cWs : L.aW1);
+#pragma unroll
+            for (int k = 0; k < 4; ++k) w[k] = k < a.S ? W[k * H1 + f] : 0.f;
+            b = th[(critic ? L.cbs : L.ab1) + f];
+        }
+        if (not_finite(w[0]) || not_finite(w[1]) || not_finite(w[2]) || not_finite(w[3]) || not_finite(b)) atomicOr(a.bad, 1);
+        if (S1 * fmaxf(fmaxf(fabsf(w[0]), fabsf(w[1])), fmaxf(fmaxf(fabsf(w[2]), fabsf(w[3])), fabsf(b))) >= F16_OVERFLOW) atomicOr(a.bad, 1);
+    }
+    a.wf1h[net][((long)set * NGT_MAX + ft) * 64 + lane] = make_wh(w[0], w[1], w[2], w[3], b, S1, h);
+    if (net == 1 && ft == 0 && lane < 48) {
+        const int hl = lane / 24, hh = (lane / 12) & 1, ks = (lane / 4) % 3, m = lane & 3;
+        unsigned v = 0;
+#pragma unroll
+        for (int e = 0; e < 2; ++e) {
+            const int jj = 2 * m + e, fa = 16 * ks + 8 * (jj >> 2) + 4 * hh + (jj & 3);
+            f16 hi, lo;
+            split1h(S1 * th[L.cWa + fa], hi, lo);
+            v |= (unsigned)__builtin_bit_cast(unsigned short, hl ? lo : hi) << (16 * e);
+        }
+        a.wap[(long)set * 48 + lane] = v;
+    }
+}
+
 __global__ __launch_bounds__(320) void prep_kernel(const PrepArgs a) {
     __shared__ float red[320];
+    if (blockIdx.x >= H2) {
+        if (threadIdx.x < 64) prep1_tile(a, blockIdx.x - H2, blockIdx.y, blockIdx.z, threadIdx.x);
+        return;
+    }
     const int n = blockIdx.x, net = blockIdx.y, set = blockIdx.z, f = threadIdx.x;
     const bool critic = net & 1, target = net >= 2;
     const avd_mlp_layout& L = a.L;
@@ -218,8 +266,11 @@
     const int oW2 = critic ? L.cW2 : L.aW2, ob2 = critic ? L.cb2 : L.ab2, oW3 = critic ? L.cW3 : L.aW3, ob3 = critic ? L.cb3 : L.ab3;
     const int og2 = critic ? L.cg3 : L.ag2, obe2 = critic ? L.cbe3 : L.abe2, omm2 = critic ? L.cmm3 : L.amm2, omv2 = critic ? L.cmv3 : L.amv2;
     const float inv2n = (1.0f / sqrtf(st[omv2 + n] + BN_EPS)) * th[og2 + n], c3n = inv2n * th[oW3 + n];
-    const unsigned* smax = a.smax + ((long)net * gridDim.z + set) * 2;
-    const float SW = pow2_for(__uint_as_float(smax[0])), SWC = pow2_for(__uint_as_float(smax[1]));
+    const unsigned* smax = a.smax + ((long)net * gridDim.z + set) * SCALE_SLICES * 2;
+    unsigned mx = 0, mx2 = 0;
+#pragma unroll
+    for (int i = 0; i < SCALE_SLICES; ++i) mx = max(mx, smax[2 * i]), mx2 = max(mx2, smax[2 * i + 1]);
+    const float SW = pow2_for(__uint_as_float(mx)), SWC = pow2_for(__uint_as_float(mx2));
     float shw = 0.f;
     if (f < KP) {
         float w = 0.f, inv = 0.f;
@@ -280,43 +331,6 @@
         if (f == 0) vec[2 * H2] = th[ob3] + red[0];
     }
 }
-__global__ __launch_bounds__(64) void prep1_kernel(const PrepArgs a) {
-    const int ft = blockIdx.x, net = blockIdx.y, set = blockIdx.z, lane = threadIdx.x, r = lane & 31, h = lane >> 5;
-    const bool critic = net & 1, target = net >= 2;
-    const avd_mlp_layout& L = a.L;
-    const float* th = (target ? a.theta_t : a.theta) + (long)set * L.theta_size + (critic ? L.actor_size : 0);
-    const int K = critic ? CriticS::K : ActorS::K;
-    const int f = 32 * ft + r;
-    float w[4] = {0.f, 0.f, 0.f, 0.f}, b = 0.f;
-    if (f == K) {
-        b = 1.f;
-    } else if (f < K) {
-        if (critic && ft >= 8) {
-            w[0] = th[L.cWa + (f - H1)], b = th[L.cba + (f - H1)];
-        } else {
-            const float* W = th + (critic ? L.cWs : L.aW1);
-#pragma unroll
-            for (int k = 0; k < 4; ++k) w[k] = k < a.S ? W[k * H1 + f] : 0.f;
-            b = th[(critic ? L.cbs : L.ab1) + f];
-        }
-        if (not_finite(w[0]) || not_finite(w[1]) || not_finite(w[2]) || not_finite(w[3]) || not_finite(b)) atomicOr(a.bad, 1);
-        if (S1 * fmaxf(fmaxf(fabsf(w[0]), fabsf(w[1])), fmaxf(fmaxf(fabsf(w[2]), fabsf(w[3])), fabsf(b))) >= F16_OVERFLOW) atomicOr(a.bad, 1);
-    }
-    a.wf1h[net][((long)set * NGT_MAX + ft) * 64 + lane] = make_wh(w[0], w[1], w[2], w[3], b, S1, h);
-    if (net == 1 && ft == 0 && lane < 48) {
-        const int hl = lane / 24, hh = (lane / 12) & 1, ks = (lane / 4) % 3, m = lane & 3;
-        unsigned v = 0;
-#pragma unroll
-        for (int e = 0; e < 2; ++e) {
-            const int jj = 2 * m + e, fa = 16 * ks + 8 * (jj >> 2) + 4 * hh + (jj & 3);
-            f16 hi, lo;
-            split1h(S1 * th[L.cWa + fa], hi, lo);
-            v |= (unsigned)__builtin_bit_cast(unsigned short, hl ? lo : hi) << (16 * e);
-        }
-        a.wap[(long)set * 48 + lane] = v;
-    }
-}
-
 enum HeadMode { OUT_TANH = 0, OUT_TD = 1, HEAD_BOTH = 5, OUT_TANH_SAVE = 6 };
 struct HeadArgs {
     unsigned long long* stamp;
@@ -1215,7 +1229,7 @@
 struct Plan {
     int grid, J;
     size_t Whi[4], Wlo[4], Wchi[2], Wclo[2], wf1h[4], vec[4], wap, a2, y, mu, dmu, g3, sm, sma, tz, t1p, s2raw, xfs, xfs2, partHs[3], partM[2],
-        partV[2], partG[2], bad, total;
+        partV[2], partG[2], bad, smax, total;
 };
 static Plan make_plan(int n_agents, int n_sets) {
     Plan pl;
@@ -1253,7 +1267,8 @@
         pl.partG[i] = take(4 * (size_t)pl.grid * KG * H2);
     }
     for (int i = 0; i < 3; ++i) pl.partHs[i] = take(4 * (size_t)pl.grid * 8 * 2);
-    pl.bad = take(sizeof(int) + sizeof(unsigned) * 4 * (size_t)n_sets * 2);
+    pl.bad = take(sizeof(int));
+    pl.smax = take(sizeof(unsigned) * 4 * (size_t)n_sets * SCALE_SLICES * 2);
     pl.total = o;
     return pl;
 }
@@ -1277,7 +1292,8 @@
                float high, float* grads, float* losses, unsigned char* ws, const Plan& pl, hipStream_t st) {
     PrepArgs pa;
     pa.L = L, pa.S = S, pa.theta = theta, pa.stats = stats, pa.theta_t = theta_t, pa.stats_t = stats_t;
-    pa.wap = (unsigned*)(ws + pl.wap), pa.bad = (int*)(ws + pl.bad), pa.smax = (unsigned*)(ws + pl.bad + sizeof(int));
+    pa.wap = (unsigned*)(ws + pl.wap), pa.bad = (int*)(ws + pl.bad), pa.smax = (unsigned*)(ws + pl.smax);
+    pa.zero = phases == PH_CRITIC ? (float4*)grads : nullptr, pa.n_zero4 = (long)n_sets * L.theta_size / 4;
     NetP net[4];
     for (int i = 0; i < 4; ++i) {
         const bool critic = i & 1, target = i >= 2;
@@ -1329,11 +1345,8 @@
         fa.partG[i] = F(pl.partG[i]), fa.c3[i] = F(pl.vec[i]);
     fa.t1_from_g[0] = fa.t1_from_g[1] = 1, fa.t1p = F(pl.t1p), fa.s2raw = F(pl.s2raw);
     if (phases & PH_CRITIC) {
-        if (hipMemsetAsync(ws + pl.bad, 0, sizeof(int) + sizeof(unsigned) * 4 * (size_t)n_sets * 2, st) != hipSuccess)
-            return check_launch("avd_learn_set_split: memset");
         hipLaunchKernelGGL(scale_kernel, dim3(4, n_sets, SCALE_SLICES), dim3(256), 0, st, pa);
-        hipLaunchKernelGGL(prep_kernel, dim3(H2, 4, n_sets), dim3(320), 0, st, pa);
-        hipLaunchKernelGGL(prep1_kernel, dim3(NGT_MAX, 4, n_sets), dim3(64), 0, st, pa);
+        hipLaunchKernelGGL(prep_kernel, dim3(H2 + NGT_MAX, 4, n_sets), dim3(320), 0, st, pa);
         PackArgs pk;
         pk.x[0] = s, pk.extra[0] = a, pk.outh[0] = xfs, pk.x[1] = s2, pk.extra[1] = r, pk.outh[1] = xfs2, pk.rows = nrows, pk.bad = bad;
         hipLaunchKernelGGL(pack_x_kernel<S>, dim3((unsigned)((2 * nrows + 255) / 256), 2), dim3(256), 0, st, pk);
@@ -1407,8 +1420,6 @@
     AVD_REQUIRE(theta && stats && s && grads && workspace && (!cr || (theta_t && stats_t && a && r && s2)), "%s: null pointer", who);
     const fsplit::Plan pl = fsplit::make_plan(n_agents, n_sets);
     AVD_REQUIRE(workspace_bytes >= pl.total, "%s: workspace %zu B < %zu B", who, workspace_bytes, pl.total);
-    if (cr && hipMemsetAsync(grads, 0, sizeof(float) * (size_t)n_sets * lay->theta_size, (hipStream_t)stream) != hipSuccess)
-        return check_launch("avd_learn_set_split: hipMemsetAsync(grads)");
     if (lay->S == 4)
         return fsplit::run<4>(phases, *lay, n_agents, n_sets, theta, stats, theta_t, stats_t, s, a, r, s2, agent_weight, gamma, high, grads,
                               losses, (unsigned char*)workspace, pl, (hipStream_t)stream);
diff --git a/avddpg_amd/csrc/optim.hip b/avddpg_amd/csrc/optim.hip
--- a/avddpg_amd/csrc/optim.hip
+++ b/avddpg_amd/csrc/optim.hip
@@ -11,6 +11,9 @@
     return a >= 0x7f800000u || c >= 0x7f800000u;
 }
 
+__device__ __forceinline__ void adam_polyak_set(int set, int t, int theta_size, int actor_size, float4* __restrict__ theta,
+                                                float4* __restrict__ theta_t, float4* __restrict__ m, float4* __restrict__ v,
+                                                const float4* __restrict__ grads, float actor_lr, float critic_lr, float tau, float omt);
 template <bool GUARD>
 __global__ __launch_bounds__(256) void adam_polyak_kernel(int theta_size, int actor_size, float4* __restrict__ theta,
                                                           float4* __restrict__ theta_t, float4* __restrict__ m,
@@ -27,6 +30,13 @@
         }
         return;
     }
+    adam_polyak_set(set, t, theta_size, actor_size, theta, theta_t, m, v, grads, actor_lr, critic_lr, tau, omt);
+}
+
+__device__ __forceinline__ void adam_polyak_set(int set, int t, int theta_size, int actor_size, float4* __restrict__ theta,
+                                                float4* __restrict__ theta_t, float4* __restrict__ m, float4* __restrict__ v,
+                                                const float4* __restrict__ grads, float actor_lr, float critic_lr, float tau, float omt) {
+#pragma clang fp contract(off)
     const float b1p = (float)pow((double)ADAM_B1, (double)t);
     const float b2p = (float)pow((double)ADAM_B2, (double)t);
     const float root = sqrtf(1.0f - b2p);
@@ -244,6 +254,36 @@
     const long base = (long)set * stats_size;
     for (int i = blockIdx.x * blockDim.x + threadIdx.x; i < stats_size; i += gridDim.x * blockDim.x)
         t[base + i] = w[base + i] * tau + t[base + i] * omt;
+}
+
+__global__ __launch_bounds__(256) void adam_polyak_step_kernel(int theta_size, int actor_size, int stats_size, float4* __restrict__ theta,
+                                                               float4* __restrict__ theta_t, float4* __restrict__ m,
+                                                               float4* __restrict__ v, const float4* __restrict__ grads,
+                                                               const float* __restrict__ stats, float* __restrict__ stats_t,
+                                                               int32_t* __restrict__ step, int32_t* __restrict__ tick, float actor_lr,
+                                                               float critic_lr, float tau, float omt, int32_t* __restrict__ skipped) {
+#pragma clang fp contract(off)
+    const int set = blockIdx.y;
+    if (slab_is_nan((const float*)grads + (long)set * theta_size, actor_size)) {
+        if (blockIdx.x == 0 && threadIdx.x == 0 && skipped) atomicAdd(skipped, 1);
+        return;
+    }
+    __shared__ int t_sh;
+    if (threadIdx.x == 0) {
+        const int t = step[set] + 1;
+        t_sh = t;
+        __builtin_amdgcn_fence(__ATOMIC_RELEASE, "agent");
+        if (__hip_atomic_fetch_add(tick + set, 1, __ATOMIC_RELAXED, __HIP_MEMORY_SCOPE_AGENT) == (int)gridDim.x - 1) {
+            __builtin_amdgcn_fence(__ATOMIC_ACQUIRE, "agent");
+            tick[set] = 0;
+            step[set] = t;
+        }
+    }
+    __syncthreads();
+    adam_polyak_set(set, t_sh, theta_size, actor_size, theta, theta_t, m, v, grads, actor_lr, critic_lr, tau, omt);
+    const long base = (long)set * stats_size;
+    for (int i = blockIdx.x * blockDim.x + threadIdx.x; i < stats_size; i += gridDim.x * blockDim.x)
+        stats_t[base + i] = stats[base + i] * tau + stats_t[base + i] * omt;
 }
 
 constexpr int FS_COLS = 64, FS_PH = 4, FS_UNR = 8;
@@ -448,6 +488,22 @@
     return check_launch("avd_learn_update_f32(update pass)");
 }
 
+extern "C" int avd_adam_polyak_guarded_step_f32(const avd_mlp_layout* lay, int n_sets, float* theta, float* stats, float* theta_t,
+                                                float* stats_t, float* m, float* v, const float* grads, int32_t* step, int32_t* tick,
+                                                float actor_lr, float critic_lr, double tau, int32_t* skipped, void* stream) {
+    const char* who = "avd_adam_polyak_guarded_step_f32";
+    AVD_REQUIRE(lay && n_sets > 0, "%s: n_sets=%d", who, n_sets);
+    AVD_REQUIRE(theta && stats && theta_t && stats_t && m && v && grads && step && tick, "%s: null pointer", who);
+    AVD_REQUIRE(lay->theta_size % 4 == 0 && lay->actor_size % 4 == 0 && lay->stats_size % 4 == 0, "%s: layout not 4-float aligned", who);
+    const float tauf = (float)tau, omt = (float)(1.0 - tau);
+    int gx = (lay->theta_size / 4 + 255) / 256;
+    if (n_sets >= 256 && gx > 8) gx = 8;
+    hipLaunchKernelGGL(adam_polyak_step_kernel, dim3(gx, n_sets), dim3(256), 0, (hipStream_t)stream, lay->theta_size, lay->actor_size,
+                       lay->stats_size, (float4*)theta, (float4*)theta_t, (float4*)m, (float4*)v, (const float4*)grads, stats, stats_t,
+                       step, tick, actor_lr, critic_lr, tauf, omt, skipped);
+    return check_launch(who);
+}
+
 extern "C" int avd_polyak_f32(int64_t n, const float* w, float* t, double tau, void* stream) {
     AVD_REQUIRE(n > 0 && w && t, "avd_polyak_f32: n=%ld", (long)n);
     long blocks = (n + 255) / 256;
diff --git a/avddpg_amd/vec.py b/avddpg_amd/vec.py
--- a/avddpg_amd/vec.py
+++ b/avddpg_amd/vec.py
@@ -378,14 +378,16 @@
 
     def apply(self, grads, guarded=False):
         c = self.config
-        self.step += 1
         if guarded:
             if getattr(self, "nonfinite_skipped", None) is None:
                 self.nonfinite_skipped = torch.zeros(1, dtype=torch.int32, device=self.device)
-            call("avd_adam_polyak_guarded_f32", self._layp, self.n_sets, ptr(self.theta), ptr(self.stats), ptr(self.theta_t),
-                 ptr(self.stats_t), ptr(self.m), ptr(self.v), ptr(grads), ptr(self.step), c.actor_lr, c.critic_lr,
-                 float(c.tau), ptr(self.nonfinite_skipped), stream_handle())
+            if getattr(self, "_adam_tick", None) is None:
+                self._adam_tick = torch.zeros(self.n_sets, dtype=torch.int32, device=self.device)
+            call("avd_adam_polyak_guarded_step_f32", self._layp, self.n_sets, ptr(self.theta), ptr(self.stats), ptr(self.theta_t),
+                 ptr(self.stats_t), ptr(self.m), ptr(self.v), ptr(grads), ptr(self.step), ptr(self._adam_tick), c.actor_lr,
+                 c.critic_lr, float(c.tau), ptr(self.nonfinite_skipped), stream_handle())
             return
+        self.step += 1
         call("avd_adam_polyak_f32", self._layp, self.n_sets, ptr(self.theta), ptr(self.stats), ptr(self.theta_t),
              ptr(self.stats_t), ptr(self.m), ptr(self.v), ptr(grads), ptr(self.step), c.actor_lr, c.critic_lr,
              float(c.tau), stream_handle())
diff --git a/include/avddpg_hip.h b/include/avddpg_hip.h
--- a/include/avddpg_hip.h
+++ b/include/avddpg_hip.h
@@ -107,6 +107,10 @@
                                 float* m, float* v, const float* grads, int32_t* step, float actor_lr, float critic_lr, double tau,
                                 int32_t* skipped, void* stream);
 
+int avd_adam_polyak_guarded_step_f32(const avd_mlp_layout* lay, int n_sets, float* theta, float* stats, float* theta_t,
+                                     float* stats_t, float* m, float* v, const float* grads, int32_t* step, int32_t* tick,
+                                     float actor_lr, float critic_lr, double tau, int32_t* skipped, void* stream);
+
 int avd_learn_update_f32(const avd_mlp_layout* lay, int n_agents, const float* theta, const float* stats,
                          float* theta_out, float* theta_t, float* stats_t, float* m, float* v, const int32_t* step,
                          const float* s, const float* a, const float* r, const float* s2, float gamma, float high,
```

Result: faster. 2.013 million, median of 6 (+1.2%).
